# damaggu/StableKeypoints

Hardware: AMD Instinct MI355X
Metric: images/sec (token-opt step, 512², N=500 tokens) (higher is better)
Workload: dtype f32

## Files before the change

include/skp.h:

```cpp
#ifndef SKP_H
#define SKP_H

#ifdef __cplusplus
extern "C" {
#endif

#define SKP_OK 0
#define SKP_EBADARG (-1)
#define SKP_ELAUNCH (-2)
#define SKP_MAX_LAYERS 16

const char* skp_last_error(void);
int skp_version(void);

int skp_capture_fwd(const float* z_low, int BH, int s, int N, int R, float* attn, float* stats, void* stream);

int skp_capture_bwd(const float* z_low, int BH, int s, int N, int R, const float* dattn, int group, long long sb,
                    long long sp, long long sn, float gscale, const float* stats, float* dz_low, float* workspace,
                    void* stream);

int skp_capture_maps_fwd(const float* const* z_low, const int* sizes, int L, int B, int H, int N, int R, float* maps,
                         float* const* stats, void* stream);

int skp_capture_maps_bwd(const float* const* z_low, const int* sizes, int L, int B, int H, int N, int R,
                         const float* dmaps, float gscale, const float* const* stats, float* const* dz_low,
                         float* workspace, void* stream);

long long skp_capture_maps_bwd_sel_workspace(const int* sizes, int L, int B, int H, int N, int R, int K);
int skp_capture_maps_bwd_sel(const float* const* z_low, const int* sizes, int L, int B, int H, int N, int R,
                             const long long* sel_tok, int K, const float* gsel, float gscale,
                             const float* const* stats, float* const* dz_low, float* workspace, void* stream);
int skp_sel_bwd_timing(int enable);
int skp_sel_bwd_timing_read(double* ms, int* calls);

int skp_aggregate(const float* const* layers, int L, int BH, int RR, int N, const long long* indices,
                  int n_out, float* out, void* stream);

int skp_resize_bilinear(const float* in, int C, int R, int Ro, float* out, void* stream);
int skp_resize_bilinear_bwd(const float* gout, int C, int R, int Ro, float* gin, void* stream);

int skp_argmax2d(const float* maps, int T, int h, int w, const long long* rows, int n_rows, float* pos,
                 long long* idx, void* stream);

int skp_k_max_pixels(const float* maps, int T, int h, int w, int num, float radius2, float* pos,
                     float* masked, void* stream);

int skp_mask_radius(const float* maps, int T, int h, int w, const float* pos, float radius2, float* out,
                    void* stream);

int skp_weighted_avg(float* maps, int T, int h, int w, float distance, int mutate, float* pos, void* stream);

int skp_gaussian_target(const float* pos, int num, int T, int size, float sigma, float* out, void* stream);

int skp_topk_gaussian(const float* maps, int T, int h, int w, int top_k, float sigma, float epsilon,
                      int num_subjects, long long* out, double* kl, void* workspace, void* stream);

int skp_topk_gaussian_batch(const float* maps, int nb, int T, int h, int w, int top_k, float sigma,
                            float epsilon, int num_subjects, long long* out, double* kl, void* workspace,
                            void* stream);

int skp_topk_keys(const double* keys, int nb, int T, int top_k, long long* out, void* stream);

int skp_entropy_sort(const float* maps, int T, int h, int w, int top_k, long long* out, double* ent,
                     void* workspace, void* stream);

int skp_fps(const float* maps, int T, int h, int w, const long long* cand, int n_cand, int top_k,
            long long* out, int* n_out, void* workspace, void* stream);
int skp_fps_batch(const float* maps, int nb, int T, int h, int w, const long long* cand, int n_cand, int top_k,
                  long long* out, int* n_out, void* workspace, void* stream);
int skp_fps_keys_batch(const double* keys, const float* maps, int nb, int T, int h, int w, int n_cand, int top_k,
                       long long* cand, long long* out, int* n_out, void* workspace, void* stream);

int skp_sharpen_fwd(const float* A, int T, int h, int w, float sigma, int num_subjects, float* pos,
                     double* partial, float* loss, void* stream);
int skp_sharpen_bwd(const float* A, int T, int h, int w, float sigma, int num_subjects, const float* pos,
                     const float* gout, float* dA, void* stream);
int skp_sharpen_fwd_batch(const float* A, int nb, int T, int h, int w, float sigma, int num_subjects, float* pos,
                          double* partial, float* loss, void* stream);
int skp_sharpen_bwd_batch(const float* A, int nb, int T, int h, int w, float sigma, int num_subjects,
                          const float* pos, const float* gout, float* dA, void* stream);

int skp_affine_warp(const float* x, int B, int C, int H, int W, const float* theta, float* out, void* stream);
int skp_affine_warp_bwd(const float* gout, int B, int C, int H, int W, const float* theta, float* gin,
                        void* stream);

int skp_equiv_fwd(const float* A, const float* At, int T, int h, int w, const float* theta_inv,
                  double* partial, float* loss, void* stream);
int skp_equiv_bwd(const float* A, const float* At, int T, int h, int w, const float* theta_inv,
                  const float* gout, float* dA, float* dAt, void* stream);
int skp_equiv_fwd_batch(const float* A, const float* At, int nb, int T, int h, int w, const float* theta_inv,
                        double* partial, float* loss, void* stream);
int skp_equiv_bwd_batch(const float* A, const float* At, int nb, int T, int h, int w, const float* theta_inv,
                        const float* gout, float* dA, float* dAt, void* stream);

int skp_wino_in_transform(const float* x, int B, int C, int H, int W, float* V, void* stream);
int skp_wino_out_transform(const float* M, int B, int K, int H, int W, const float* bias, const float* residual,
                           float* y, void* stream);
int skp_wino_out_transform_kt(const float* M, int B, int K, int H, int W, const float* bias, const float* residual,
                              float* y, float* gn_part, void* stream);

int skp_bgemm_f32(const float* A, long long sAb, long long sAm, long long sAk, const float* B, long long sBb,
                  long long sBk, long long sBn, float* C, long long sCb, long long sCm, long long sCn, int batch,
                  int M, int N, int K, float alpha, int accumulate, void* stream);
int skp_bgemm_f32_2b(const float* A, long long sAo, long long sAb, long long sAm, long long sAk, const float* B,
                     long long sBo, long long sBb, long long sBk, long long sBn, float* C, long long sCo, long long sCb,
                     long long sCm, long long sCn, int batch, int hb, int M, int N, int K, float alpha, int accumulate,
                     void* stream);

int skp_groupnorm_workspace(int B, int C, long long HW, int G);
int skp_groupnorm_fwd(const float* x, const float* gamma, const float* beta, const float* shift, int B, int C,
                      long long HW, int G, float eps, int act, float* y, float* stats, double* partial,
                      void* stream);
int skp_groupnorm_bwd(const float* x, const float* dy, const float* gamma, const float* beta, const float* shift,
                      const float* stats, int B, int C, long long HW, int G, int act, float* dx, double* partial,
                      void* stream);
int skp_groupnorm_fwd_part(const float* x, const float* gamma, const float* beta, const float* shift, const float* part,
                           int nseg, int B, int C, long long HW, int G, float eps, int act, float* y, float* stats,
                           double* partial, void* stream);
int skp_groupnorm_stats(const float* x, const float* shift, int B, int C, long long HW, int G, float eps, float* stats,
                        double* partial, void* stream);
int skp_groupnorm_stats_part(const float* part, int nseg, const float* shift, int B, int C, long long HW, int G,
                             float eps, float* stats, double* partial, void* stream);
int skp_groupnorm_bwd_add(const float* x, const float* dy, const float* gamma, const float* beta, const float* shift,
                          const float* stats, int B, int C, long long HW, int G, int act, const float* dres, float* dx,
                          double* partial, void* stream);
int skp_softmax_bwd(const float* P, float* dP, long long rows, int cols, float alpha, void* stream);
int skp_softmax_fwd(float* S, long long rows, int cols, void* stream);
int skp_attn_dscore(const float* P, const float* dO, const float* V, const float* D, float* out, int BH, int S, int L,
                    int d, float alpha, void* stream);
int skp_attn_bwd_kv(const float* P, const float* dO, const float* Q, const float* V, const float* D, float* dS,
                    float* dV, float* dK, int BH, int S, int L, int d, float alpha, void* stream);
int skp_attn_fwd(const float* Q, const float* K, const float* V, float* O, float* stats, int BH, int S, int L, int d,
                 float scale, void* stream);
int skp_attn_bwd_flash(const float* Q, const float* K, const float* V, const float* dO, const float* stats,
                       const float* D, float* dS, float* dV, float* dK, int BH, int S, int L, int d, float scale,
                       void* stream);
int skp_attn_fwd_bshd(const float* Q, long long q_sb, int q_rs, const float* K, long long k_sb, int k_rs,
                      const float* V, long long v_sb, int v_rs, float* O, long long o_sb, int o_rs, float* stats, int B,
                      int H, int S, int L, int d, float scale, void* stream);
int skp_attn_bwd_flash_bshd(const float* Q, long long q_sb, int q_rs, const float* K, long long k_sb, int k_rs,
                            const float* V, long long v_sb, int v_rs, const float* dO, long long o_sb, int o_rs,
                            const float* stats, const float* D, float* dS, float* dV, long long dv_sb, int dv_rs,
                            float* dK, long long dk_sb, int dk_rs, int B, int H, int S, int L, int d, float scale,
                            void* stream);
int skp_layernorm_fwd(const float* x, const float* gamma, const float* beta, long long rows, int C, float eps, float* y,
                      float* stats, void* stream);
int skp_layernorm_bwd(const float* x, const float* dy, const float* gamma, const float* stats, long long rows, int C,
                      float* dx, void* stream);
int skp_layernorm_bwd_add(const float* x, const float* dy, const float* gamma, const float* stats, long long rows,
                          int C, const float* dres, float* dx, void* stream);
int skp_geglu_fwd(const float* h, long long rows, int I, float* out, void* stream);
int skp_geglu_bwd(const float* h, const float* dout, long long rows, int I, float* dh, void* stream);
int skp_residual_bias_add(const float* a, const float* h, const float* bias, int B, int C, long long HW,
                          float* out, void* stream);
int skp_wino_weights(const float* w, int K, int C, int flip, float* U, void* stream);
int skp_conv3x3_wino(const float* x, const float* U, const float* bias, const float* residual, float* y, int B, int C,
                     int K, int H, int W, int nsplit, float* ws, void* stream);
int skp_wino2_weights(const float* w, int K, int C, int flip, float* U, void* stream);
int skp_conv3x3_wino2(const float* x, const float* U, const float* bias, const float* residual, float* y, int B,
                      int C, int K, int H, int W, int nsplit, float* ws, void* stream);
int skp_conv3x3_wino2_gn(const float* x, const float* U, const float* bias, const float* residual, float* y, int B,
                         int C, int K, int H, int W, int nsplit, float* ws, float* gn_part, void* stream);
int skp_wino2_vtransform(const float* x, float* V, int B, int C, int H, int W, void* stream);
int skp_wino2_vtransform_gn(const float* x, const float* stats, const float* gamma, const float* beta,
                            const float* shift, int G, int act, float* V, int B, int C, int H, int W, void* stream);
int skp_conv3x3_wino2_v(const float* V, const float* U, const float* bias, const float* residual, float* y, int B,
                        int C, int K, int H, int W, int nsplit, float* ws, void* stream);
int skp_conv3x3_wino2_v_gn(const float* V, const float* U, const float* bias, const float* residual, float* y, int B,
                           int C, int K, int H, int W, int nsplit, float* ws, float* gn_part, void* stream);
int skp_wino2s2_weights(const float* w, int K, int C, float* U, void* stream);
int skp_conv3x3s2_f2(const float* x, const float* U, const float* bias, float* y, int B, int C, int K, int H, int W,
                     int nsplit, float* ws, void* stream);

int skp_map_range(const float* maps, int n, int h, int w, float* range, void* stream);
int skp_render_sheet(const float* images, int n, int H, int W, const float* maps, int h, int w, const float* range,
                     const float* lut, float alpha, const float* points, int K, float radius,
                     const unsigned char* colors, int rows, int cols, int f, int pad, unsigned char* out,
                     void* stream);

int skp_tta_reduce_workspace(int B, int n, int S);
int skp_tta_reduce(const float* maps, int B, int C, int n, int S, const float* theta_inv, float* pos, float* avg,
                   void* workspace, void* stream);

int skp_tta_reduce_scored_workspace(int B, int n, int S);
int skp_tta_reduce_scored(const float* maps, int B, int C, int n, int S, const float* theta_inv, float distance,
                          float* pos, float* refined, float* scores, float* avg, void* workspace, void* stream);

#ifdef __cplusplus
}
#endif
#endif
```

stablekeypoints_amd/_lib.py:

```python
import ctypes
import os

import torch

_HERE = os.path.dirname(os.path.abspath(__file__))
LIB_PATH = os.environ.get("SKP_LIB", os.path.join(_HERE, "libskp.so"))

_c_int, _c_float, _c_ll, _p = ctypes.c_int, ctypes.c_float, ctypes.c_longlong, ctypes.c_void_p

_SIGS = {
    "skp_capture_fwd": [_p, _c_int, _c_int, _c_int, _c_int, _p, _p, _p],
    "skp_capture_bwd": [_p, _c_int, _c_int, _c_int, _c_int, _p, _c_int, _c_ll, _c_ll, _c_ll, _c_float, _p, _p, _p,
                        _p],
    "skp_capture_maps_fwd": [ctypes.POINTER(_p), ctypes.POINTER(_c_int), _c_int, _c_int, _c_int, _c_int, _c_int, _p,
                             ctypes.POINTER(_p), _p],
    "skp_capture_maps_bwd": [ctypes.POINTER(_p), ctypes.POINTER(_c_int), _c_int, _c_int, _c_int, _c_int, _c_int, _p,
                             _c_float, ctypes.POINTER(_p), ctypes.POINTER(_p), _p, _p],
    "skp_capture_maps_bwd_sel": [ctypes.POINTER(_p), ctypes.POINTER(_c_int), _c_int, _c_int, _c_int, _c_int, _c_int,
                                 _p, _c_int, _p, _c_float, ctypes.POINTER(_p), ctypes.POINTER(_p), _p, _p],
    "skp_sel_bwd_timing": [_c_int],
    "skp_sel_bwd_timing_read": [_p, _p],
    "skp_capture_maps_bwd_sel_workspace": [ctypes.POINTER(_c_int), _c_int, _c_int, _c_int, _c_int, _c_int, _c_int],
    "skp_aggregate": [ctypes.POINTER(_p), _c_int, _c_int, _c_int, _c_int, _p, _c_int, _p, _p],
    "skp_resize_bilinear": [_p, _c_int, _c_int, _c_int, _p, _p],
    "skp_resize_bilinear_bwd": [_p, _c_int, _c_int, _c_int, _p, _p],
    "skp_argmax2d": [_p, _c_int, _c_int, _c_int, _p, _c_int, _p, _p, _p],
    "skp_k_max_pixels": [_p, _c_int, _c_int, _c_int, _c_int, _c_float, _p, _p, _p],
    "skp_mask_radius": [_p, _c_int, _c_int, _c_int, _p, _c_float, _p, _p],
    "skp_weighted_avg": [_p, _c_int, _c_int, _c_int, _c_float, _c_int, _p, _p],
    "skp_gaussian_target": [_p, _c_int, _c_int, _c_int, _c_float, _p, _p],
    "skp_topk_gaussian": [_p, _c_int, _c_int, _c_int, _c_int, _c_float, _c_float, _c_int, _p, _p, _p, _p],
    "skp_topk_gaussian_batch": [_p, _c_int, _c_int, _c_int, _c_int, _c_int, _c_float, _c_float, _c_int, _p, _p, _p,
                                _p],
    "skp_topk_keys": [_p, _c_int, _c_int, _c_int, _p, _p],
    "skp_entropy_sort": [_p, _c_int, _c_int, _c_int, _c_int, _p, _p, _p, _p],
    "skp_fps": [_p, _c_int, _c_int, _c_int, _p, _c_int, _c_int, _p, _p, _p, _p],
    "skp_fps_batch": [_p, _c_int, _c_int, _c_int, _c_int, _p, _c_int, _c_int, _p, _p, _p, _p],
    "skp_fps_keys_batch": [_p, _p, _c_int, _c_int, _c_int, _c_int, _c_int, _c_int, _p, _p, _p, _p, _p],
    "skp_sharpen_fwd": [_p, _c_int, _c_int, _c_int, _c_float, _c_int, _p, _p, _p, _p],
    "skp_sharpen_bwd": [_p, _c_int, _c_int, _c_int, _c_float, _c_int, _p, _p, _p, _p],
    "skp_wino_in_transform": [_p, _c_int, _c_int, _c_int, _c_int, _p, _p],
    "skp_wino_out_transform": [_p, _c_int, _c_int, _c_int, _c_int, _p, _p, _p, _p],
    "skp_wino_out_transform_kt": [_p, _c_int, _c_int, _c_int, _c_int, _p, _p, _p, _p, _p],
    "skp_sharpen_fwd_batch": [_p, _c_int, _c_int, _c_int, _c_int, _c_float, _c_int, _p, _p, _p, _p],
    "skp_sharpen_bwd_batch": [_p, _c_int, _c_int, _c_int, _c_int, _c_float, _c_int, _p, _p, _p, _p],
    "skp_affine_warp": [_p, _c_int, _c_int, _c_int, _c_int, _p, _p, _p],
    "skp_affine_warp_bwd": [_p, _c_int, _c_int, _c_int, _c_int, _p, _p, _p],
    "skp_equiv_fwd": [_p, _p, _c_int, _c_int, _c_int, _p, _p, _p, _p],
    "skp_equiv_bwd": [_p, _p, _c_int, _c_int, _c_int, _p, _p, _p, _p, _p],
    "skp_equiv_fwd_batch": [_p, _p, _c_int, _c_int, _c_int, _c_int, _p, _p, _p, _p],
    "skp_equiv_bwd_batch": [_p, _p, _c_int, _c_int, _c_int, _c_int, _p, _p, _p, _p, _p],
    "skp_bgemm_f32": [_p, _c_ll, _c_ll, _c_ll, _p, _c_ll, _c_ll, _c_ll, _p, _c_ll, _c_ll, _c_ll, _c_int, _c_int,
                      _c_int, _c_int, _c_float, _c_int, _p],
    "skp_bgemm_f32_2b": [_p, _c_ll, _c_ll, _c_ll, _c_ll, _p, _c_ll, _c_ll, _c_ll, _c_ll, _p, _c_ll, _c_ll, _c_ll,
                         _c_ll, _c_int, _c_int, _c_int, _c_int, _c_int, _c_float, _c_int, _p],
    "skp_groupnorm_workspace": [_c_int, _c_int, _c_ll, _c_int],
    "skp_groupnorm_fwd": [_p, _p, _p, _p, _c_int, _c_int, _c_ll, _c_int, _c_float, _c_int, _p, _p, _p, _p],
    "skp_groupnorm_bwd": [_p, _p, _p, _p, _p, _p, _c_int, _c_int, _c_ll, _c_int, _c_int, _p, _p, _p],
    "skp_groupnorm_bwd_add": [_p, _p, _p, _p, _p, _p, _c_int, _c_int, _c_ll, _c_int, _c_int, _p, _p, _p, _p],
    "skp_residual_bias_add": [_p, _p, _p, _c_int, _c_int, _c_ll, _p, _p],
    "skp_softmax_bwd": [_p, _p, _c_ll, _c_int, _c_float, _p],
    "skp_softmax_fwd": [_p, _c_ll, _c_int, _p],
    "skp_attn_dscore": [_p, _p, _p, _p, _p, _c_int, _c_int, _c_int, _c_int, _c_float, _p],
    "skp_attn_bwd_kv": [_p, _p, _p, _p, _p, _p, _p, _p, _c_int, _c_int, _c_int, _c_int, _c_float, _p],
    "skp_attn_fwd": [_p, _p, _p, _p, _p, _c_int, _c_int, _c_int, _c_int, _c_float, _p],
    "skp_attn_bwd_flash": [_p, _p, _p, _p, _p, _p, _p, _p, _p, _c_int, _c_int, _c_int, _c_int, _c_float, _p],
    "skp_attn_fwd_bshd": [_p, _c_ll, _c_int, _p, _c_ll, _c_int, _p, _c_ll, _c_int, _p, _c_ll, _c_int, _p, _c_int, _c_int,
                          _c_int, _c_int, _c_int, _c_float, _p],
    "skp_attn_bwd_flash_bshd": [_p, _c_ll, _c_int, _p, _c_ll, _c_int, _p, _c_ll, _c_int, _p, _c_ll, _c_int, _p, _p, _p,
                                _p, _c_ll, _c_int, _p, _c_ll, _c_int, _c_int, _c_int, _c_int, _c_int, _c_int, _c_float,
                                _p],
    "skp_layernorm_fwd": [_p, _p, _p, _c_ll, _c_int, _c_float, _p, _p, _p],
    "skp_layernorm_bwd": [_p, _p, _p, _p, _c_ll, _c_int, _p, _p],
    "skp_layernorm_bwd_add": [_p, _p, _p, _p, _c_ll, _c_int, _p, _p, _p],
    "skp_geglu_fwd": [_p, _c_ll, _c_int, _p, _p],
    "skp_geglu_bwd": [_p, _p, _c_ll, _c_int, _p, _p],
    "skp_wino_weights": [_p, _c_int, _c_int, _c_int, _p, _p],
    "skp_conv3x3_wino": [_p, _p, _p, _p, _p, _c_int, _c_int, _c_int, _c_int, _c_int, _c_int, _p, _p],
    "skp_wino2_weights": [_p, _c_int, _c_int, _c_int, _p, _p],
    "skp_conv3x3_wino2": [_p, _p, _p, _p, _p, _c_int, _c_int, _c_int, _c_int, _c_int, _c_int, _p, _p],
    "skp_conv3x3_wino2_gn": [_p, _p, _p, _p, _p, _c_int, _c_int, _c_int, _c_int, _c_int, _c_int, _p, _p, _p],
    "skp_groupnorm_fwd_part": [_p, _p, _p, _p, _p, _c_int, _c_int, _c_int, _c_ll, _c_int, _c_float, _c_int, _p, _p, _p,
                               _p],
    "skp_groupnorm_stats": [_p, _p, _c_int, _c_int, _c_ll, _c_int, _c_float, _p, _p, _p],
    "skp_groupnorm_stats_part": [_p, _c_int, _p, _c_int, _c_int, _c_ll, _c_int, _c_float, _p, _p, _p],
    "skp_wino2_vtransform": [_p, _p, _c_int, _c_int, _c_int, _c_int, _p],
    "skp_wino2_vtransform_gn": [_p, _p, _p, _p, _p, _c_int, _c_int, _p, _c_int, _c_int, _c_int, _c_int, _p],
    "skp_conv3x3_wino2_v": [_p, _p, _p, _p, _p, _c_int, _c_int, _c_int, _c_int, _c_int, _c_int, _p, _p],
    "skp_conv3x3_wino2_v_gn": [_p, _p, _p, _p, _p, _c_int, _c_int, _c_int, _c_int, _c_int, _c_int, _p, _p, _p],
    "skp_wino2s2_weights": [_p, _c_int, _c_int, _p, _p],
    "skp_conv3x3s2_f2":   [_p, _p, _p, _p, _c_int, _c_int, _c_int, _c_int, _c_int, _c_int, _p, _p],
    "skp_map_range": [_p, _c_int, _c_int, _c_int, _p, _p],
    "skp_render_sheet": [_p, _c_int, _c_int, _c_int, _p, _c_int, _c_int, _p, _p, _c_float, _p, _c_int, _c_float, _p,
                         _c_int, _c_int, _c_int, _c_int, _p, _p],
    "skp_tta_reduce_workspace": [_c_int, _c_int, _c_int],
    "skp_tta_reduce": [_p, _c_int, _c_int, _c_int, _c_int, _p, _p, _p, _p, _p],
    "skp_tta_reduce_scored_workspace": [_c_int, _c_int, _c_int],
    "skp_tta_reduce_scored": [_p, _c_int, _c_int, _c_int, _c_int, _p, _c_float, _p, _p, _p, _p, _p, _p],
    "skp_version": [],
}


_RESTYPE = {"skp_capture_maps_bwd_sel_workspace": _c_ll}
_MEASUREMENT_ONLY = {"skp_sel_bwd_timing", "skp_sel_bwd_timing_read"}


class SkpLibraryError(RuntimeError):
    pass


_lib = None


def lib():
    global _lib
    if _lib is None:
        if not os.path.exists(LIB_PATH):
            raise SkpLibraryError(f"libskp.so not found at {LIB_PATH}: build it with "
                                  "`python -c 'import __graft_entry__ as g; g.build()'` or `make -C stablekeypoints_amd/csrc`")
        try:
            L = ctypes.CDLL(LIB_PATH)
        except OSError as e:
            raise SkpLibraryError(f"cannot load {LIB_PATH}: {e}") from e
        for name, args in _SIGS.items():
            if name in _MEASUREMENT_ONLY and not hasattr(L, name):
                continue
            f = getattr(L, name)
            f.argtypes = args
            f.restype = _RESTYPE.get(name, _c_int)
        L.skp_last_error.argtypes = []
        L.skp_last_error.restype = ctypes.c_char_p
        _lib = L
    return _lib


def exported_symbols():
    return list(_SIGS) + ["skp_last_error"]


def call(name, *args):
    rc = getattr(lib(), name)(*args)
    if rc != 0:
        msg = lib().skp_last_error().decode(errors="replace")
        raise RuntimeError(f"{name} failed (rc={rc}): {msg}")


def ptr(t):
    return None if t is None else ctypes.c_void_p(t.data_ptr())


def stream(device=None):
    return ctypes.c_void_p(torch.cuda.current_stream(device).cuda_stream)


def require_device(*tensors):
    for t in tensors:
        if t is not None and not t.is_cuda:
            raise ValueError("stablekeypoints_amd ops run on the HIP device only; got a CPU tensor "
                             "(there is no CPU fallback: the CPU oracle lives under oracle/ and is test-only)")
```

stablekeypoints_amd/csrc/skp_groupnorm.hip:

```cpp
#include <algorithm>

#include "skp_common.h"
#include "skp_gn.h"

using namespace skp;

namespace {

constexpr int kThreads = 256;
constexpr int kChunk = 16384;

__device__ __forceinline__ float silu_grad(float z) {
  const float s = sigmoid_of(z);
  return s * (1.0f + z * (1.0f - s));
}

struct GNShape {
  int B, C, G, cpg, nsplit;
  long long HW, len;
};

__device__ __forceinline__ int chan_of(long long e, const GNShape& sh) {
#if SKP_GN_FAST
  return (int)((unsigned)e / (unsigned)sh.HW);
#else
  return (int)(e / sh.HW);
#endif
}

#ifndef SKP_GN_BATCH
#define SKP_GN_BATCH 4
#endif
template <typename Ld, typename Use>
__device__ __forceinline__ void for_f4(long long lo, long long hi, Ld ld, Use use) {
  constexpr int U = SKP_GN_BATCH;
  constexpr long long S = 4 * kThreads;
  long long e = lo + 4 * threadIdx.x;
  for (; e + (U - 1) * S < hi; e += U * S) {
    decltype(ld(e)) v[U];
#pragma unroll
    for (int u = 0; u < U; ++u) v[u] = ld(e + u * S);
#pragma unroll
    for (int u = 0; u < U; ++u) use(e + u * S, v[u]);
  }
  for (; e < hi; e += S) use(e, ld(e));
}

__device__ __forceinline__ float add_rn(float a, float b) {
#pragma clang fp contract(off)
  return a + b;
}

struct Pair4 {
  float4 a, b, r;
};
__device__ __forceinline__ Pair4 make_pair4(float4 a, float4 b) { return Pair4{a, b, make_float4(0.f, 0.f, 0.f, 0.f)}; }

__device__ __forceinline__ float shift_of(const float* __restrict__ shift, const GNShape& sh, int grp, int c) {
  return shift ? shift[(grp / sh.G) * sh.C + c] : 0.0f;
}

__device__ __forceinline__ void block_sum2(double& a, double& b, double* sd) {
  a = wave_sum(a);
  b = wave_sum(b);
  const int lane = threadIdx.x & 63, wid = threadIdx.x >> 6;
  if (lane == 0) { sd[2 * wid] = a; sd[2 * wid + 1] = b; }
  __syncthreads();
  if (threadIdx.x == 0) {
    double x = 0.0, y = 0.0;
    for (int w = 0; w < kThreads / 64; ++w) { x += sd[2 * w]; y += sd[2 * w + 1]; }
    sd[0] = x;
    sd[1] = y;
  }
  __syncthreads();
  a = sd[0];
  b = sd[1];
}

template <bool VEC>
__global__ __launch_bounds__(kThreads) void gn_stats_kernel(const float* __restrict__ x,
                                                            const float* __restrict__ shift, GNShape sh,
                                                            double* __restrict__ partial) {
  __shared__ double sd[2 * kThreads / 64];
  const int grp = blockIdx.x / sh.nsplit, sp = blockIdx.x % sh.nsplit;
  const int g = grp % sh.G;
  const float* base = x + (size_t)grp * sh.len;
  const long long lo = (long long)sp * kChunk, hi = min(sh.len, lo + kChunk);
  double s1 = 0.0, s2 = 0.0;
  if (VEC) {
    for_f4(lo, hi, [&](long long e) { return *reinterpret_cast<const float4*>(base + e); },
           [&](long long e, float4 v) {
             const float t = shift_of(shift, sh, grp, g * sh.cpg + chan_of(e, sh));
             v.x += t; v.y += t; v.z += t; v.w += t;
             s1 += (double)v.x + (double)v.y + (double)v.z + (double)v.w;
             s2 += (double)v.x * v.x + (double)v.y * v.y + (double)v.z * v.z + (double)v.w * v.w;
           });
  } else {
    for (long long e = lo + threadIdx.x; e < hi; e += kThreads) {
      const double v = base[e] + shift_of(shift, sh, grp, g * sh.cpg + chan_of(e, sh));
      s1 += v;
      s2 += v * v;
    }
  }
  block_sum2(s1, s2, sd);
  if (threadIdx.x == 0) {
    partial[2 * blockIdx.x] = s1;
    partial[2 * blockIdx.x + 1] = s2;
  }
}

__global__ __launch_bounds__(kThreads) void gn_part_combine_kernel(const float2* __restrict__ part, int nseg,
                                                                   const float* __restrict__ shift, GNShape sh,
                                                                   double* __restrict__ partial) {
  __shared__ double sd[2 * kThreads / 64];
  const int grp = blockIdx.x;
  const int b = grp / sh.G, g = grp - b * sh.G;
  const float2* pg = part + ((size_t)b * sh.C + (size_t)g * sh.cpg) * nseg;
  const double n = (double)(sh.HW / nseg);
  double s1 = 0.0, s2 = 0.0;
  for (int e = threadIdx.x; e < sh.cpg * nseg; e += kThreads) {
    const float2 v = pg[e];
    const double t = shift ? (double)shift[(size_t)b * sh.C + g * sh.cpg + e / nseg] : 0.0;
    const double mt = (double)v.x + t;
    s1 += n * mt;
    s2 += (double)v.y + n * mt * mt;
  }
  block_sum2(s1, s2, sd);
  if (threadIdx.x < sh.nsplit) {
    partial[2 * ((size_t)grp * sh.nsplit + threadIdx.x)] = threadIdx.x == 0 ? s1 : 0.0;
    partial[2 * ((size_t)grp * sh.nsplit + threadIdx.x) + 1] = threadIdx.x == 0 ? s2 : 0.0;
  }
  for (int k = kThreads + threadIdx.x; k < sh.nsplit; k += kThreads) {
    partial[2 * ((size_t)grp * sh.nsplit + k)] = 0.0;
    partial[2 * ((size_t)grp * sh.nsplit + k) + 1] = 0.0;
  }
}

__device__ __forceinline__ void group_moments(const double* __restrict__ partial, int grp, const GNShape& sh, float eps,
                                              float& mean, float& rstd) {
  double s1 = 0.0, s2 = 0.0;
  for (int k = 0; k < sh.nsplit; ++k) {
    s1 += partial[2 * (grp * sh.nsplit + k)];
    s2 += partial[2 * (grp * sh.nsplit + k) + 1];
  }
  const double n = (double)sh.len;
  const double m = s1 / n;
  double var = s2 / n - m * m;
  var = var < 0.0 ? 0.0 : var;
  mean = (float)m;
  rstd = (float)(1.0 / sqrt(var + (double)eps));
}

template <bool VEC, bool ACT>
__global__ __launch_bounds__(kThreads) void gn_apply_kernel(const float* __restrict__ x, const float* __restrict__ gamma,
                                                            const float* __restrict__ beta,
                                                            const float* __restrict__ shift, GNShape sh, float eps,
                                                            const double* __restrict__ partial, float* __restrict__ y,
                                                            float* __restrict__ stats) {
  __shared__ float sm[2];
  const int grp = blockIdx.x / sh.nsplit, sp = blockIdx.x % sh.nsplit;
  if (threadIdx.x == 0) {
    float mean, rstd;
    group_moments(partial, grp, sh, eps, mean, rstd);
    sm[0] = mean;
    sm[1] = rstd;
    if (sp == 0 && stats) { stats[2 * grp] = mean; stats[2 * grp + 1] = rstd; }
  }
  __syncthreads();
  const float mean = sm[0], rstd = sm[1];
  const int g = grp % sh.G;
  const float* base = x + (size_t)grp * sh.len;
  float* out = y + (size_t)grp * sh.len;
  const long long lo = (long long)sp * kChunk, hi = min(sh.len, lo + kChunk);
  if (VEC) {
    for_f4(lo, hi, [&](long long e) { return *reinterpret_cast<const float4*>(base + e); },
           [&](long long e, float4 v) {
             const int c = g * sh.cpg + chan_of(e, sh);
             const GNCoef k = gn_coef(gamma[c], beta[c], mean, rstd);
             const float t = shift_of(shift, sh, grp, c);
             v.x = gn_elem<ACT>(v.x, t, k); v.y = gn_elem<ACT>(v.y, t, k);
             v.z = gn_elem<ACT>(v.z, t, k); v.w = gn_elem<ACT>(v.w, t, k);
             *reinterpret_cast<float4*>(out + e) = v;
           });
  } else {
    for (long long e = lo + threadIdx.x; e < hi; e += kThreads) {
      const int c = g * sh.cpg + chan_of(e, sh);
      float v = ((base[e] + shift_of(shift, sh, grp, c)) - mean) * rstd * gamma[c] + beta[c];
      out[e] = ACT ? silu(v) : v;
    }
  }
}

template <bool VEC, bool ACT>
__global__ __launch_bounds__(kThreads) void gn_bwd_stats_kernel(const float* __restrict__ x,
                                                                const float* __restrict__ dy,
                                                                const float* __restrict__ gamma,
                                                                const float* __restrict__ beta,
                                                                const float* __restrict__ shift, GNShape sh,
                                                                const float* __restrict__ stats,
                                                                double* __restrict__ partial) {
  __shared__ double sd[2 * kThreads / 64];
  const int grp = blockIdx.x / sh.nsplit, sp = blockIdx.x % sh.nsplit;
  const int g = grp % sh.G;
  const float mean = stats[2 * grp], rstd = stats[2 * grp + 1];
  const float* xb = x + (size_t)grp * sh.len;
  const float* db = dy + (size_t)grp * sh.len;
  const long long lo = (long long)sp * kChunk, hi = min(sh.len, lo + kChunk);
  double s1 = 0.0, s2 = 0.0;
  auto body = [&](long long e0, const float* xv, const float* dv, int n) {
    const int c = g * sh.cpg + chan_of(e0, sh);
    const float ga = gamma[c], be = beta[c], t = shift_of(shift, sh, grp, c);
#pragma unroll
    for (int k = 0; k < 4; ++k) {
      if (k >= n) break;
      const float xh = ((xv[k] + t) - mean) * rstd;
      float gz = dv[k];
      if (ACT) gz *= silu_grad(xh * ga + be);
      const float gg = gz * ga;
      s1 += (double)gg;
      s2 += (double)gg * (double)xh;
    }
  };
  if (VEC) {
    for_f4(lo, hi,
           [&](long long e) {
             return make_pair4(*reinterpret_cast<const float4*>(xb + e), *reinterpret_cast<const float4*>(db + e));
           },
           [&](long long e, const Pair4& v) {
             const float xv[4] = {v.a.x, v.a.y, v.a.z, v.a.w}, dv[4] = {v.b.x, v.b.y, v.b.z, v.b.w};
             body(e, xv, dv, 4);
           });
  } else {
    for (long long e0 = lo + threadIdx.x; e0 < hi; e0 += kThreads) body(e0, xb + e0, db + e0, 1);
  }
  block_sum2(s1, s2, sd);
  if (threadIdx.x == 0) {
    partial[2 * blockIdx.x] = s1;
    partial[2 * blockIdx.x + 1] = s2;
  }
}

template <bool VEC, bool ACT>
__global__ __launch_bounds__(kThreads) void gn_bwd_apply_kernel(const float* __restrict__ x,
                                                                const float* __restrict__ dy,
                                                                const float* __restrict__ gamma,
                                                                const float* __restrict__ beta,
                                                                const float* __restrict__ shift, GNShape sh,
                                                                const float* __restrict__ stats,
                                                                const double* __restrict__ partial,
                                                                const float* __restrict__ dres,
                                                                float* __restrict__ dx) {
  __shared__ float sm[2];
  const int grp = blockIdx.x / sh.nsplit, sp = blockIdx.x % sh.nsplit;
  if (threadIdx.x == 0) {
    double s1 = 0.0, s2 = 0.0;
    for (int k = 0; k < sh.nsplit; ++k) {
      s1 += partial[2 * (grp * sh.nsplit + k)];
      s2 += partial[2 * (grp * sh.nsplit + k) + 1];
    }
    sm[0] = (float)(s1 / (double)sh.len);
    sm[1] = (float)(s2 / (double)sh.len);
  }
  __syncthreads();
  const float ma = sm[0], mb = sm[1];
  const int g = grp % sh.G;
  const float mean = stats[2 * grp], rstd = stats[2 * grp + 1];
  const float* xb = x + (size_t)grp * sh.len;
  const float* db = dy + (size_t)grp * sh.len;
  float* ob = dx + (size_t)grp * sh.len;
  const float* rb = dres ? dres + (size_t)grp * sh.len : nullptr;
  const long long lo = (long long)sp * kChunk, hi = min(sh.len, lo + kChunk);
  auto body = [&](long long e0, const float* xv, const float* dv, const float* av, float* r, int n) {
    const int c = g * sh.cpg + chan_of(e0, sh);
    const float ga = gamma[c], be = beta[c], t = shift_of(shift, sh, grp, c);
#pragma unroll
    for (int k = 0; k < 4; ++k) {
      if (k >= n) break;
      const float xh = ((xv[k] + t) - mean) * rstd;
      float gz = dv[k];
      if (ACT) gz *= silu_grad(xh * ga + be);
      r[k] = rstd * (gz * ga - ma - xh * mb);
      if (rb) r[k] = add_rn(r[k], av[k]);
    }
  };
  if (VEC) {
    for_f4(lo, hi,
           [&](long long e) {
             Pair4 v = make_pair4(*reinterpret_cast<const float4*>(xb + e), *reinterpret_cast<const float4*>(db + e));
             v.r = rb ? *reinterpret_cast<const float4*>(rb + e) : make_float4(0.f, 0.f, 0.f, 0.f);
             return v;
           },
           [&](long long e, const Pair4& v) {
             const float xv[4] = {v.a.x, v.a.y, v.a.z, v.a.w}, dv[4] = {v.b.x, v.b.y, v.b.z, v.b.w};
             const float av[4] = {v.r.x, v.r.y, v.r.z, v.r.w};
             float r[4];
             body(e, xv, dv, av, r, 4);
             *reinterpret_cast<float4*>(ob + e) = make_float4(r[0], r[1], r[2], r[3]);
           });
  } else {
    for (long long e0 = lo + threadIdx.x; e0 < hi; e0 += kThreads) {
      const float av = rb ? rb[e0] : 0.0f;
      float r;
      body(e0, xb + e0, db + e0, &av, &r, 1);
      ob[e0] = r;
    }
  }
}

template <bool VEC>
__global__ __launch_bounds__(kThreads) void residual_bias_kernel(const float* __restrict__ a,
                                                                 const float* __restrict__ h,
                                                                 const float* __restrict__ bias, int C, long long HW,
                                                                 long long total, float* __restrict__ out) {
  const long long step = (long long)gridDim.x * kThreads * (VEC ? 4 : 1);
  for (long long e = ((long long)blockIdx.x * kThreads + threadIdx.x) * (VEC ? 4 : 1); e < total; e += step) {
    const float b = bias[(e / HW) % C];
    if (VEC) {
      const float4 x = *reinterpret_cast<const float4*>(a + e), y = *reinterpret_cast<const float4*>(h + e);
      *reinterpret_cast<float4*>(out + e) = make_float4(x.x + (y.x + b), x.y + (y.y + b), x.z + (y.z + b),
                                                        x.w + (y.w + b));
    } else {
      out[e] = a[e] + (h[e] + b);
    }
  }
}

bool make_shape(int B, int C, long long HW, int G, GNShape& sh) {
  if (B <= 0 || C <= 0 || HW <= 0 || G <= 0 || C % G != 0) return false;
  sh.B = B; sh.C = C; sh.G = G; sh.cpg = C / G; sh.HW = HW;
  sh.len = (long long)sh.cpg * HW;
  sh.nsplit = (int)((sh.len + kChunk - 1) / kChunk);
  return sh.len < (1LL << 32);
}

}

extern "C" int skp_groupnorm_workspace(int B, int C, long long HW, int G) {
  GNShape sh;
  if (!make_shape(B, C, HW, G, sh)) return -1;
  return B * G * sh.nsplit * 2;
}

extern "C" int skp_groupnorm_fwd(const float* x, const float* gamma, const float* beta, const float* shift, int B,
                                 int C, long long HW, int G, float eps, int act, float* y, float* stats,
                                 double* partial, void* stream) {
  SKP_CHECK_ARG(x && gamma && beta && y && partial, "null pointer");
  GNShape sh;
  SKP_CHECK_ARG(make_shape(B, C, HW, G, sh), "bad shape (C must be divisible by G)");
  const bool vec = (HW % 4 == 0) && ((reinterpret_cast<uintptr_t>(x) & 15) == 0) &&
                   ((reinterpret_cast<uintptr_t>(y) & 15) == 0);
  hipStream_t st = as_stream(stream);
  const dim3 grid(B * G * sh.nsplit);
  if (vec) hipLaunchKernelGGL(gn_stats_kernel<true>, grid, dim3(kThreads), 0, st, x, shift, sh, partial);
  else hipLaunchKernelGGL(gn_stats_kernel<false>, grid, dim3(kThreads), 0, st, x, shift, sh, partial);
  SKP_LAUNCH_CHECK();
#define SKP_GN_APPLY(V, A) \
  hipLaunchKernelGGL((gn_apply_kernel<V, A>), grid, dim3(kThreads), 0, st, x, gamma, beta, shift, sh, eps, partial, y, \
                     stats)
  if (vec) { if (act) SKP_GN_APPLY(true, true); else SKP_GN_APPLY(true, false); }
  else { if (act) SKP_GN_APPLY(false, true); else SKP_GN_APPLY(false, false); }
#undef SKP_GN_APPLY
  SKP_LAUNCH_CHECK();
  return SKP_OK;
}

extern "C" int skp_groupnorm_fwd_part(const float* x, const float* gamma, const float* beta, const float* shift,
                                      const float* part, int nseg, int B, int C, long long HW, int G, float eps,
                                      int act, float* y, float* stats, double* partial, void* stream) {
  SKP_CHECK_ARG(x && gamma && beta && y && partial && part, "null pointer");
  SKP_CHECK_ARG(nseg > 0 && HW % nseg == 0, "nseg must divide H·W");
  GNShape sh;
  SKP_CHECK_ARG(make_shape(B, C, HW, G, sh), "bad shape (C must be divisible by G)");
  SKP_CHECK_ARG((reinterpret_cast<uintptr_t>(part) & 7) == 0, "part must be 8-byte aligned");
  const bool vec = (HW % 4 == 0) && ((reinterpret_cast<uintptr_t>(x) & 15) == 0) &&
                   ((reinterpret_cast<uintptr_t>(y) & 15) == 0);
  hipStream_t st = as_stream(stream);
  hipLaunchKernelGGL(gn_part_combine_kernel, dim3(B * G), dim3(kThreads), 0, st, reinterpret_cast<const float2*>(part),
                     nseg, shift, sh, partial);
  SKP_LAUNCH_CHECK();
  const dim3 grid(B * G * sh.nsplit);
#define SKP_GN_APPLY(V, A) \
  hipLaunchKernelGGL((gn_apply_kernel<V, A>), grid, dim3(kThreads), 0, st, x, gamma, beta, shift, sh, eps, partial, y, \
                     stats)
  if (vec) { if (act) SKP_GN_APPLY(true, true); else SKP_GN_APPLY(true, false); }
  else { if (act) SKP_GN_APPLY(false, true); else SKP_GN_APPLY(false, false); }
#undef SKP_GN_APPLY
  SKP_LAUNCH_CHECK();
  return SKP_OK;
}

namespace {
__global__ __launch_bounds__(kThreads) void gn_moments_kernel(const double* __restrict__ partial, GNShape sh, float eps,
                                                              float* __restrict__ stats) {
  const int grp = blockIdx.x * kThreads + threadIdx.x;
  if (grp >= sh.B * sh.G) return;
  float mean, rstd;
  group_moments(partial, grp, sh, eps, mean, rstd);
  stats[2 * grp] = mean;
  stats[2 * grp + 1] = rstd;
}
}

extern "C" int skp_groupnorm_stats(const float* x, const float* shift, int B, int C, long long HW, int G, float eps,
                                   float* stats, double* partial, void* stream) {
  SKP_CHECK_ARG(x && stats && partial, "null pointer");
  GNShape sh;
  SKP_CHECK_ARG(make_shape(B, C, HW, G, sh), "bad shape (C must be divisible by G)");
  const bool vec = (HW % 4 == 0) && ((reinterpret_cast<uintptr_t>(x) & 15) == 0);
  hipStream_t st = as_stream(stream);
  const dim3 grid(B * G * sh.nsplit);
  if (vec) hipLaunchKernelGGL(gn_stats_kernel<true>, grid, dim3(kThreads), 0, st, x, shift, sh, partial);
  else hipLaunchKernelGGL(gn_stats_kernel<false>, grid, dim3(kThreads), 0, st, x, shift, sh, partial);
  SKP_LAUNCH_CHECK();
  hipLaunchKernelGGL(gn_moments_kernel, dim3((B * G + kThreads - 1) / kThreads), dim3(kThreads), 0, st, partial, sh, eps,
                     stats);
  SKP_LAUNCH_CHECK();
  return SKP_OK;
}

extern "C" int skp_groupnorm_stats_part(const float* part, int nseg, const float* shift, int B, int C, long long HW,
                                        int G, float eps, float* stats, double* partial, void* stream) {
  SKP_CHECK_ARG(part && stats && partial, "null pointer");
  SKP_CHECK_ARG(nseg > 0 && HW % nseg == 0, "nseg must divide H·W");
  GNShape sh;
  SKP_CHECK_ARG(make_shape(B, C, HW, G, sh), "bad shape (C must be divisible by G)");
  SKP_CHECK_ARG((reinterpret_cast<uintptr_t>(part) & 7) == 0, "part must be 8-byte aligned");
  hipStream_t st = as_stream(stream);
  hipLaunchKernelGGL(gn_part_combine_kernel, dim3(B * G), dim3(kThreads), 0, st, reinterpret_cast<const float2*>(part),
                     nseg, shift, sh, partial);
  SKP_LAUNCH_CHECK();
  hipLaunchKernelGGL(gn_moments_kernel, dim3((B * G + kThreads - 1) / kThreads), dim3(kThreads), 0, st, partial, sh, eps,
                     stats);
  SKP_LAUNCH_CHECK();
  return SKP_OK;
}

extern "C" int skp_groupnorm_bwd_add(const float* x, const float* dy, const float* gamma, const float* beta,
                                     const float* shift, const float* stats, int B, int C, long long HW, int G, int act,
                                     const float* dres, float* dx, double* partial, void* stream) {
  SKP_CHECK_ARG(x && dy && gamma && beta && stats && dx && partial, "null pointer");
  GNShape sh;
  SKP_CHECK_ARG(make_shape(B, C, HW, G, sh), "bad shape (C must be divisible by G)");
  const bool vec = (HW % 4 == 0) && ((reinterpret_cast<uintptr_t>(x) & 15) == 0) &&
                   ((reinterpret_cast<uintptr_t>(dy) & 15) == 0) && ((reinterpret_cast<uintptr_t>(dx) & 15) == 0) &&
                   ((reinterpret_cast<uintptr_t>(dres) & 15) == 0);
  hipStream_t st = as_stream(stream);
  const dim3 grid(B * G * sh.nsplit);
#define SKP_GN_B(K, V, A, ...) hipLaunchKernelGGL((K<V, A>), grid, dim3(kThreads), 0, st, __VA_ARGS__)
  if (vec) {
    if (act) SKP_GN_B(gn_bwd_stats_kernel, true, true, x, dy, gamma, beta, shift, sh, stats, partial);
    else SKP_GN_B(gn_bwd_stats_kernel, true, false, x, dy, gamma, beta, shift, sh, stats, partial);
  } else {
    if (act) SKP_GN_B(gn_bwd_stats_kernel, false, true, x, dy, gamma, beta, shift, sh, stats, partial);
    else SKP_GN_B(gn_bwd_stats_kernel, false, false, x, dy, gamma, beta, shift, sh, stats, partial);
  }
  SKP_LAUNCH_CHECK();
  if (vec) {
    if (act) SKP_GN_B(gn_bwd_apply_kernel, true, true, x, dy, gamma, beta, shift, sh, stats, partial, dres, dx);
    else SKP_GN_B(gn_bwd_apply_kernel, true, false, x, dy, gamma, beta, shift, sh, stats, partial, dres, dx);
  } else {
    if (act) SKP_GN_B(gn_bwd_apply_kernel, false, true, x, dy, gamma, beta, shift, sh, stats, partial, dres, dx);
    else SKP_GN_B(gn_bwd_apply_kernel, false, false, x, dy, gamma, beta, shift, sh, stats, partial, dres, dx);
  }
#undef SKP_GN_B
  SKP_LAUNCH_CHECK();
  return SKP_OK;
}

extern "C" int skp_groupnorm_bwd(const float* x, const float* dy, const float* gamma, const float* beta,
                                 const float* shift, const float* stats, int B, int C, long long HW, int G, int act,
                                 float* dx, double* partial, void* stream) {
  return skp_groupnorm_bwd_add(x, dy, gamma, beta, shift, stats, B, C, HW, G, act, nullptr, dx, partial, stream);
}

extern "C" int skp_residual_bias_add(const float* a, const float* h, const float* bias, int B, int C, long long HW,
                                     float* out, void* stream) {
  SKP_CHECK_ARG(a && h && bias && out, "null pointer");
  SKP_CHECK_ARG(B > 0 && C > 0 && HW > 0, "non-positive shape");
  const long long total = (long long)B * C * HW;
  const bool vec = (HW % 4 == 0) && ((reinterpret_cast<uintptr_t>(a) & 15) == 0) &&
                   ((reinterpret_cast<uintptr_t>(h) & 15) == 0) && ((reinterpret_cast<uintptr_t>(out) & 15) == 0);
  const long long units = vec ? total / 4 : total;
  const int blocks = (int)std::min<long long>((units + kThreads - 1) / kThreads, 256LL * 16);
  hipStream_t st = as_stream(stream);
  if (vec) hipLaunchKernelGGL(residual_bias_kernel<true>, dim3(blocks), dim3(kThreads), 0, st, a, h, bias, C, HW, total, out);
  else hipLaunchKernelGGL(residual_bias_kernel<false>, dim3(blocks), dim3(kThreads), 0, st, a, h, bias, C, HW, total, out);
  SKP_LAUNCH_CHECK();
  return SKP_OK;
}
```

stablekeypoints_amd/csrc/skp_softmax.hip:

```cpp
#include "skp_common.h"

using namespace skp;

namespace {

template <int TPR, int EPT, bool VEC>
__global__ __launch_bounds__(TPR) void softmax_bwd_kernel(const float* __restrict__ P, float* __restrict__ G,
                                                          long long rows, int cols, float alpha) {
  __shared__ float sred[TPR / WAVE];
  const long long row = blockIdx.x;
  if (row >= rows) return;
  const float* p = P + row * cols;
  float* g = G + row * cols;
  static_assert(!VEC || EPT % 4 == 0, "float4 path needs EPT % 4 == 0");
  float pv[EPT], gv[EPT];
  float dot = 0.0f;
  if (VEC) {
#pragma unroll
    for (int q = 0; q < EPT / 4; ++q) {
      const int e = 4 * (threadIdx.x + q * TPR);
      float4 a = make_float4(0.f, 0.f, 0.f, 0.f), b = a;
      if (e < cols) {
        a = *reinterpret_cast<const float4*>(p + e);
        b = *reinterpret_cast<const float4*>(g + e);
// ... 233 lines not shown
template <int KS, int DB>
__global__ __launch_bounds__(256) void attn_fwd_kernel(const float* __restrict__ Q, const float* __restrict__ K,
                                                       const float* __restrict__ V, float* __restrict__ O,
                                                       float2* __restrict__ ST, int S, int L, float scale, int H,
                                                       AttnLay lq, AttnLay lk, AttnLay lv, AttnLay lo) {
  constexpr int d = 4 * KS, dp = d + 1;
  __shared__ float sK[64 * dp], sV[64 * 16 * DB];
  const int b = blockIdx.y;
  const int r0 = blockIdx.x * 64;
  const int t = threadIdx.x, lane = t & 63, w = t >> 6;
  const int row = r0 + 16 * w + (lane & 15);
  const float* Qb = lq.at(Q, b, H, d);
  const float* Kb = lk.at(K, b, H, d);
  const float* Vb = lv.at(V, b, H, d);
  float qv[KS];
  {
    const float* q = Qb + (size_t)row * lq.rs + (lane >> 4);
#pragma unroll
    for (int ks = 0; ks < KS; ++ks) qv[ks] = q[4 * ks] * scale;
  }
  f32x4a o[DB];
#pragma unroll
  for (int db = 0; db < DB; ++db) o[db] = f32x4a{0.f, 0.f, 0.f, 0.f};
  float m = -INFINITY, l = 0.0f;
  for (int k0 = 0; k0 < L; k0 += 64) {
    __syncthreads();
    {
      for (int e = t; e < 64 * KS; e += 256) {
        const int key = e / KS, c = 4 * (e - key * KS);
        float4 kk = make_float4(0.f, 0.f, 0.f, 0.f), vv = kk;
        if (k0 + key < L) {
          kk = *reinterpret_cast<const float4*>(Kb + (size_t)(k0 + key) * lk.rs + c);
          vv = *reinterpret_cast<const float4*>(Vb + (size_t)(k0 + key) * lv.rs + c);
        }
        float* pk = sK + key * dp + c;
        pk[0] = kk.x; pk[1] = kk.y; pk[2] = kk.z; pk[3] = kk.w;
        *reinterpret_cast<float4*>(sV + key * 16 * DB + c) = vv;
      }
      if constexpr (16 * DB > d)
        for (int e = t; e < 64 * (16 * DB - d); e += 256) {
          const int key = e / (16 * DB - d), c = d + (e - key * (16 * DB - d));
          sV[key * 16 * DB + c] = 0.0f;
        }
    }
    __syncthreads();
    f32x4a s4[4];
#pragma unroll
    for (int c = 0; c < 4; ++c) {
      s4[c] = f32x4a{0.f, 0.f, 0.f, 0.f};
      const float* kr = sK + (16 * c + (lane & 15)) * dp + (lane >> 4);
#pragma unroll
      for (int ks = 0; ks < KS; ++ks) s4[c] = __builtin_amdgcn_mfma_f32_16x16x4f32(kr[4 * ks], qv[ks], s4[c], 0, 0, 0);
    }
    if (k0 + 64 > L) {
#pragma unroll
      for (int c = 0; c < 4; ++c)
#pragma unroll
        for (int r = 0; r < 4; ++r)
          if (k0 + 16 * c + 4 * (lane >> 4) + r >= L) s4[c][r] = -INFINITY;
    }
    float bm = -INFINITY;
#pragma unroll
    for (int c = 0; c < 4; ++c) bm = fmaxf(bm, fmaxf(fmaxf(s4[c][0], s4[c][1]), fmaxf(s4[c][2], s4[c][3])));
    bm = fmaxf(bm, __shfl_xor(bm, 16, 64));
    bm = fmaxf(bm, __shfl_xor(bm, 32, 64));
    const float mn = fmaxf(m, bm);
    const float corr = __expf(m - mn);
    float bs = 0.0f;
#pragma unroll
    for (int c = 0; c < 4; ++c)
#pragma unroll
      for (int r = 0; r < 4; ++r) {
        s4[c][r] = __expf(s4[c][r] - mn);
        bs += s4[c][r];
      }
    bs += __shfl_xor(bs, 16, 64);
    bs += __shfl_xor(bs, 32, 64);
    l = l * corr + bs;
    m = mn;
#pragma unroll
    for (int db = 0; db < DB; ++db) o[db] *= corr;
#pragma unroll
    for (int c = 0; c < 4; ++c)
#pragma unroll
      for (int r = 0; r < 4; ++r) {
        const float* vr = sV + (16 * c + 4 * (lane >> 4) + r) * 16 * DB + (lane & 15);
#pragma unroll
        for (int db = 0; db < DB; ++db)
          o[db] = __builtin_amdgcn_mfma_f32_16x16x4f32(vr[16 * db], s4[c][r], o[db], 0, 0, 0);
      }
  }
  const float inv = 1.0f / l;
  float* orow = lo.at(O, b, H, d) + (size_t)row * lo.rs;
#pragma unroll
  for (int db = 0; db < DB; ++db) {
    const int dd = 16 * db + 4 * (lane >> 4);
    if (dd < d) *reinterpret_cast<float4*>(orow + dd) = make_float4(o[db][0] * inv, o[db][1] * inv, o[db][2] * inv, o[db][3] * inv);
  }
  if (ST != nullptr && lane < 16) ST[(size_t)b * S + row] = make_float2(m, inv);
}

}

namespace {
int attn_fwd_launch(const float* Q, AttnLay lq, const float* K, AttnLay lk, const float* V, AttnLay lv, float* O,
                    AttnLay lo, float* stats, int BH, int H, int S, int L, int d, float scale, void* stream) {
  SKP_CHECK_ARG(Q && K && V && O, "null pointer");
  SKP_CHECK_ARG(BH > 0 && H > 0 && BH % H == 0 && S > 0 && L > 0, "non-positive shape");
  SKP_CHECK_ARG(S % 64 == 0, "S must be a multiple of 64");
  SKP_CHECK_ARG(BH <= 65535, "grid too large");
  SKP_CHECK_ARG(((reinterpret_cast<uintptr_t>(K) | reinterpret_cast<uintptr_t>(V) | reinterpret_cast<uintptr_t>(O)) &
                 15) == 0,
                "tensors must be 16-byte aligned");
  SKP_CHECK_ARG(((lk.rs | lv.rs | lo.rs | lk.sb | lv.sb | lo.sb) & 3) == 0, "K, V, O strides must be multiples of 4");
  SKP_CHECK_ARG((reinterpret_cast<uintptr_t>(stats) & 7) == 0, "stats must be 8-byte aligned");
  const dim3 grid((unsigned)(S / 64), (unsigned)BH);
  hipStream_t st = as_stream(stream);
  float2* ST = reinterpret_cast<float2*>(stats);
#define SKP_AF(KS_, DB_)                                                                                        \
  hipLaunchKernelGGL((attn_fwd_kernel<KS_, DB_>), grid, dim3(256), 0, st, Q, K, V, O, ST, S, L, scale, H, lq, lk, lv, \
                     lo)
  switch (d) {
    case 40: SKP_AF(10, 3); break;
    case 64: SKP_AF(16, 4); break;
    case 80: SKP_AF(20, 5); break;
    default: SKP_CHECK_ARG(false, "head dim must be 40, 64 or 80");
  }
#undef SKP_AF
  SKP_LAUNCH_CHECK();
  return SKP_OK;
}
AttnLay contig(int rows, int d) { return AttnLay{(long long)rows * d, d}; }
}

extern "C" int skp_attn_fwd(const float* Q, const float* K, const float* V, float* O, float* stats, int BH, int S,
                            int L, int d, float scale, void* stream) {
  return attn_fwd_launch(Q, contig(S, d), K, contig(L, d), V, contig(L, d), O, contig(S, d), stats, BH, 1, S, L, d,
                         scale, stream);
}

extern "C" int skp_attn_fwd_bshd(const float* Q, long long q_sb, int q_rs, const float* K, long long k_sb, int k_rs,
                                 const float* V, long long v_sb, int v_rs, float* O, long long o_sb, int o_rs,
                                 float* stats, int B, int H, int S, int L, int d, float scale, void* stream) {
  SKP_CHECK_ARG(B > 0 && H > 0 && (long long)B * H <= 65535, "bad B, H");
  return attn_fwd_launch(Q, AttnLay{q_sb, q_rs}, K, AttnLay{k_sb, k_rs}, V, AttnLay{v_sb, v_rs}, O, AttnLay{o_sb, o_rs},
                         stats, B * H, H, S, L, d, scale, stream);
}

namespace {

template <int KS, int DB, int WPE, bool RC>
__global__ __launch_bounds__(256) __attribute__((amdgpu_waves_per_eu(WPE, WPE))) void attn_bwd_kv_kernel(
    const float* __restrict__ P, const float* __restrict__ dO, const float* __restrict__ Q, const float* __restrict__ V,
    const float* __restrict__ D, float* __restrict__ dS, float* __restrict__ dV, float* __restrict__ dK, int S, int L,
    float alpha, const float* __restrict__ Kt, const float2* __restrict__ ST, float scale, int H, AttnLay lo, AttnLay lq,
    AttnLay lk, AttnLay lv, AttnLay ldv, AttnLay ldk) {
  constexpr int d = 4 * KS, dp = d + 1, dq = 16 * DB + 1;
  __shared__ float sV[64 * dp];
  __shared__ float sK[RC ? 64 * dp : 1];
  __shared__ float2 sST[2][RC ? 64 : 1];
  __shared__ float sO[2][64 * dq], sQ[2][64 * dq];
  __shared__ float sD[2][64];
  const int b = blockIdx.y, k0 = blockIdx.x * 64;
  const int t = threadIdx.x, lane = t & 63, w = t >> 6;
  const float* Vb = lv.at(V, b, H, d);
  const float* dOb = lo.at(dO, b, H, d);
  const float* Qb = lq.at(Q, b, H, d);
  {
    for (int e = t; e < 64 * KS; e += 256) {
      const int key = e / KS, c = 4 * (e - key * KS);
      const bool in = k0 + key < L;
      const float4 v = in ? *reinterpret_cast<const float4*>(Vb + (size_t)(k0 + key) * lv.rs + c)
                          : make_float4(0.f, 0.f, 0.f, 0.f);
      float* p = sV + key * dp + c;
      p[0] = v.x; p[1] = v.y; p[2] = v.z; p[3] = v.w;
      if constexpr (RC) {
        const float4 kk = in ? *reinterpret_cast<const float4*>(lk.at(Kt, b, H, d) + (size_t)(k0 + key) * lk.rs + c)
                             : make_float4(0.f, 0.f, 0.f, 0.f);
        float* pk = sK + key * dp + c;
        pk[0] = kk.x; pk[1] = kk.y; pk[2] = kk.z; pk[3] = kk.w;
      }
    }
    for (int e = t; e < 64 * (dq - d); e += 256) {
      const int row = e / (dq - d), c = d + (e - row * (dq - d));
      sO[0][row * dq + c] = 0.0f; sO[1][row * dq + c] = 0.0f;
      sQ[0][row * dq + c] = 0.0f; sQ[1][row * dq + c] = 0.0f;
    }
  }
  constexpr int NPF = (64 * KS + 255) / 256;
  float4 fo[NPF], fq[NPF];
  float fd = 0.0f;
  float2 fst = make_float2(0.0f, 0.0f);
  const int rl = 16 * w + 4 * (lane >> 4);
  auto fetch = [&](int r0) {
#pragma unroll
    for (int j = 0; j < NPF; ++j) {
      const int e = t + 256 * j;
      if (e < 64 * KS) {
        const int row = e / KS, c = 4 * (e - row * KS);
        fo[j] = *reinterpret_cast<const float4*>(dOb + (size_t)(r0 + row) * lo.rs + c);
        fq[j] = *reinterpret_cast<const float4*>(Qb + (size_t)(r0 + row) * lq.rs + c);
      }
    }
    if (t < 64) {
      fd = D[(size_t)b * S + r0 + t];
      if constexpr (RC) fst = ST[(size_t)b * S + r0 + t];
    }
  };
  auto stash = [&](int buf) {
#pragma unroll
    for (int j = 0; j < NPF; ++j) {
      const int e = t + 256 * j;
      if (e < 64 * KS) {
        const int row = e / KS, c = 4 * (e - row * KS);
        float* po = sO[buf] + row * dq + c;
        float* pq = sQ[buf] + row * dq + c;
        po[0] = fo[j].x; po[1] = fo[j].y; po[2] = fo[j].z; po[3] = fo[j].w;
        pq[0] = fq[j].x; pq[1] = fq[j].y; pq[2] = fq[j].z; pq[3] = fq[j].w;
      }
    }
    if (t < 64) {
      sD[buf][t] = fd;
      if constexpr (RC) sST[buf][t] = fst;
    }
  };
  const float* Pl = P + ((size_t)b * S + rl) * L + k0 + (lane & 15);
  float* dSl = dS + ((size_t)b * S + rl) * L + k0 + (lane & 15);
  f32x4a pc[4];
  if constexpr (!RC) {
#pragma unroll
    for (int bj = 0; bj < 4; ++bj)
#pragma unroll
      for (int r = 0; r < 4; ++r) pc[bj][r] = Pl[(size_t)r * L + 16 * bj];
  }
  fetch(0);
  stash(0);
  f32x4a dv[DB][4], dk[DB][4];
#pragma unroll
  for (int db = 0; db < DB; ++db)
#pragma unroll
    for (int bj = 0; bj < 4; ++bj) {
      dv[db][bj] = f32x4a{0.f, 0.f, 0.f, 0.f};
      dk[db][bj] = f32x4a{0.f, 0.f, 0.f, 0.f};
    }
  for (int r0 = 0, buf = 0; r0 < S; r0 += 64, buf ^= 1) {
    __syncthreads();
    const bool more = r0 + 64 < S;
    f32x4a pn[4];
    if (more) {
      fetch(r0 + 64);
      if constexpr (!RC) {
        const float* Pn = Pl + (size_t)(r0 + 64) * L;
#pragma unroll
        for (int bj = 0; bj < 4; ++bj)
#pragma unroll
          for (int r = 0; r < 4; ++r) pn[bj][r] = Pn[(size_t)r * L + 16 * bj];
      }
    }
    const float* tO = sO[buf];
    const float* tQ = sQ[buf];
    f32x4a dp4[4];
    {
      const float* oa = tO + (16 * w + (lane & 15)) * dq + (lane >> 4);
      const float* vb = sV + (lane & 15) * dp + (lane >> 4);
#pragma unroll
      for (int bj = 0; bj < 4; ++bj) dp4[bj] = f32x4a{0.f, 0.f, 0.f, 0.f};
#pragma unroll
      for (int ks = 0; ks < KS; ++ks) {
        const float a = oa[4 * ks];
#pragma unroll
        for (int bj = 0; bj < 4; ++bj)
          dp4[bj] = __builtin_amdgcn_mfma_f32_16x16x4f32(a, vb[16 * bj * dp + 4 * ks], dp4[bj], 0, 0, 0);
      }
    }
    if constexpr (RC) {
      f32x4a sc[4];
      const float* qa = tQ + (16 * w + (lane & 15)) * dq + (lane >> 4);
      const float* kb = sK + (lane & 15) * dp + (lane >> 4);
#pragma unroll
      for (int bj = 0; bj < 4; ++bj) sc[bj] = f32x4a{0.f, 0.f, 0.f, 0.f};
#pragma unroll
      for (int ks = 0; ks < KS; ++ks) {
        const float a = qa[4 * ks];
#pragma unroll
        for (int bj = 0; bj < 4; ++bj)
          sc[bj] = __builtin_amdgcn_mfma_f32_16x16x4f32(a, kb[16 * bj * dp + 4 * ks], sc[bj], 0, 0, 0);
      }
#pragma unroll
      for (int r = 0; r < 4; ++r) {
        const float2 st = sST[buf][rl + r];
#pragma unroll
        for (int bj = 0; bj < 4; ++bj)
          pc[bj][r] = k0 + 16 * bj + (lane & 15) < L ? __expf(sc[bj][r] * scale - st.x) * st.y : 0.0f;
      }
    }
    f32x4a s4[4];
    float* dSr = dSl + (size_t)r0 * L;
#pragma unroll
    for (int r = 0; r < 4; ++r) {
      const float Dr = sD[buf][rl + r];
#pragma unroll
      for (int bj = 0; bj < 4; ++bj) {
        const float sv = alpha * (pc[bj][r] * (dp4[bj][r] - Dr));
        if (!RC || k0 + 16 * bj + (lane & 15) < L) dSr[(size_t)r * L + 16 * bj] = sv;
        s4[bj][r] = sv;
      }
    }
#pragma unroll
    for (int r = 0; r < 4; ++r) {
      const float* orow = tO + (rl + r) * dq + (lane & 15);
      const float* qrow = tQ + (rl + r) * dq + (lane & 15);
#pragma unroll
      for (int db = 0; db < DB; ++db) {
        const float ao = orow[16 * db], aq = qrow[16 * db];
#pragma unroll
        for (int bj = 0; bj < 4; ++bj) {
          dv[db][bj] = __builtin_amdgcn_mfma_f32_16x16x4f32(ao, pc[bj][r], dv[db][bj], 0, 0, 0);
          dk[db][bj] = __builtin_amdgcn_mfma_f32_16x16x4f32(aq, s4[bj][r], dk[db][bj], 0, 0, 0);
        }
      }
    }
    if (more) {
      stash(buf ^ 1);
      if constexpr (!RC) {
#pragma unroll
        for (int bj = 0; bj < 4; ++bj) pc[bj] = pn[bj];
      }
    }
  }
  __syncthreads();
  float* red = sO[0];
  for (int m = 0; m < 2; ++m) {
#pragma unroll
    for (int db = 0; db < DB; ++db)
#pragma unroll
      for (int bj = 0; bj < 4; ++bj) {
        const f32x4a val = m == 0 ? dv[db][bj] : dk[db][bj];
        *reinterpret_cast<float4*>(red + (w * 64 + lane) * 4) = make_float4(val[0], val[1], val[2], val[3]);
        __syncthreads();
        if (w == 0) {
          float4 acc = *reinterpret_cast<const float4*>(red + lane * 4);
#pragma unroll
          for (int ww = 1; ww < 4; ++ww) {
            const float4 x = *reinterpret_cast<const float4*>(red + (ww * 64 + lane) * 4);
            acc.x += x.x; acc.y += x.y; acc.z += x.z; acc.w += x.w;
          }
          const int dd = 16 * db + 4 * (lane >> 4);
          const int key = k0 + 16 * bj + (lane & 15);
          if (dd < d && key < L) {
            float* dst = m == 0 ? ldv.at(dV, b, H, d) + (size_t)key * ldv.rs : ldk.at(dK, b, H, d) + (size_t)key * ldk.rs;
            *reinterpret_cast<float4*>(dst + dd) = acc;
          }
        }
        __syncthreads();
      }
  }
}

}

extern "C" int skp_attn_bwd_kv(const float* P, const float* dO, const float* Q, const float* V, const float* D,
                               float* dS, float* dV, float* dK, int BH, int S, int L, int d, float alpha,
                               void* stream) {
  SKP_CHECK_ARG(P && dO && Q && V && D && dS && dV && dK, "null pointer");
  SKP_CHECK_ARG(BH > 0 && S > 0 && L > 0, "non-positive shape");
  SKP_CHECK_ARG(S % 64 == 0 && L % 64 == 0, "S and L must be multiples of 64");
  SKP_CHECK_ARG(BH <= 65535, "grid too large");
  SKP_CHECK_ARG(((reinterpret_cast<uintptr_t>(dO) | reinterpret_cast<uintptr_t>(Q) | reinterpret_cast<uintptr_t>(V) |
                  reinterpret_cast<uintptr_t>(dV) | reinterpret_cast<uintptr_t>(dK)) & 15) == 0,
                "tensors must be 16-byte aligned");
  const dim3 grid((unsigned)(L / 64), (unsigned)BH);
  hipStream_t st = as_stream(stream);
  const AttnLay ls = contig(S, d), ll = contig(L, d);
  switch (d) {
#define SKP_BKV(KS_, DB_, W_) \
  hipLaunchKernelGGL((attn_bwd_kv_kernel<KS_, DB_, W_, false>), grid, dim3(256), 0, st, P, dO, Q, V, D, dS, dV, dK, S, L, \
                     alpha, nullptr, nullptr, 0.0f, 1, ls, ls, ll, ll, ll, ll)
    case 40: SKP_BKV(10, 3, 2); break;
    case 64: SKP_BKV(16, 4, 1); break;
    case 80: SKP_BKV(20, 5, 1); break;
#undef SKP_BKV
    default: SKP_CHECK_ARG(false, "head dim must be 40, 64 or 80");
  }
  SKP_LAUNCH_CHECK();
  return SKP_OK;
}

namespace {
int attn_bwd_flash_launch(const float* Q, AttnLay lq, const float* K, AttnLay lk, const float* V, AttnLay lv,
                          const float* dO, AttnLay lo, const float* stats, const float* D, float* dS, float* dV,
                          AttnLay ldv, float* dK, AttnLay ldk, int BH, int H, int S, int L, int d, float scale,
                          void* stream) {
  SKP_CHECK_ARG(Q && K && V && dO && stats && D && dS && dV && dK, "null pointer");
  SKP_CHECK_ARG(BH > 0 && H > 0 && BH % H == 0 && S > 0 && L > 0, "non-positive shape");
  SKP_CHECK_ARG(S % 64 == 0, "S must be a multiple of 64");
  SKP_CHECK_ARG(BH <= 65535, "grid too large");
  SKP_CHECK_ARG(((reinterpret_cast<uintptr_t>(dO) | reinterpret_cast<uintptr_t>(Q) | reinterpret_cast<uintptr_t>(K) |
                  reinterpret_cast<uintptr_t>(V) | reinterpret_cast<uintptr_t>(dV) | reinterpret_cast<uintptr_t>(dK)) &
                 15) == 0 && (reinterpret_cast<uintptr_t>(stats) & 7) == 0,
                "tensors must be 16-byte aligned (stats 8-byte)");
  SKP_CHECK_ARG(((lq.rs | lk.rs | lv.rs | lo.rs | ldv.rs | ldk.rs | lq.sb | lk.sb | lv.sb | lo.sb | ldv.sb | ldk.sb) & 3) == 0,
                "strides must be multiples of 4");
  const dim3 grid((unsigned)((L + 63) / 64), (unsigned)BH);
  hipStream_t st = as_stream(stream);
  const float2* ST = reinterpret_cast<const float2*>(stats);
  switch (d) {
#define SKP_BFL(KS_, DB_, W_) \
  hipLaunchKernelGGL((attn_bwd_kv_kernel<KS_, DB_, W_, true>), grid, dim3(256), 0, st, nullptr, dO, Q, V, D, dS, dV, dK, \
                     S, L, scale, K, ST, scale, H, lo, lq, lk, lv, ldv, ldk)
    case 40: SKP_BFL(10, 3, 2); break;
    case 64: SKP_BFL(16, 4, 1); break;
    case 80: SKP_BFL(20, 5, 1); break;
#undef SKP_BFL
    default: SKP_CHECK_ARG(false, "head dim must be 40, 64 or 80");
  }
  SKP_LAUNCH_CHECK();
  return SKP_OK;
}
}

extern "C" int skp_attn_bwd_flash(const float* Q, const float* K, const float* V, const float* dO, const float* stats,
                                  const float* D, float* dS, float* dV, float* dK, int BH, int S, int L, int d, float scale,
                                  void* stream) {
  const AttnLay ls = contig(S, d), ll = contig(L, d);
  return attn_bwd_flash_launch(Q, ls, K, ll, V, ll, dO, ls, stats, D, dS, dV, ll, dK, ll, BH, 1, S, L, d, scale, stream);
}

extern "C" int skp_attn_bwd_flash_bshd(const float* Q, long long q_sb, int q_rs, const float* K, long long k_sb,
                                       int k_rs, const float* V, long long v_sb, int v_rs, const float* dO,
                                       long long o_sb, int o_rs, const float* stats, const float* D, float* dS,
                                       float* dV, long long dv_sb, int dv_rs, float* dK, long long dk_sb, int dk_rs,
                                       int B, int H, int S, int L, int d, float scale, void* stream) {
  SKP_CHECK_ARG(B > 0 && H > 0 && (long long)B * H <= 65535, "bad B, H");
  return attn_bwd_flash_launch(Q, AttnLay{q_sb, q_rs}, K, AttnLay{k_sb, k_rs}, V, AttnLay{v_sb, v_rs}, dO,
                               AttnLay{o_sb, o_rs}, stats, D, dS, dV, AttnLay{dv_sb, dv_rs}, dK, AttnLay{dk_sb, dk_rs},
                               B * H, H, S, L, d, scale, stream);
}
```

stablekeypoints_amd/csrc/skp_wino_gemm.hip:

```cpp
#include "skp_common.h"

using namespace skp;

namespace {

__device__ constexpr float kBt[6][6] = {{1.f, -1.5f, -2.f, 1.5f, 1.f, 0.f},  {0.f, -1.f, 0.5f, 2.5f, 1.f, 0.f},
                                        {0.f, 1.f, -2.5f, 0.5f, 1.f, 0.f},  {0.f, -2.f, -1.f, 2.f, 1.f, 0.f},
                                        {0.f, 0.5f, -1.f, -0.5f, 1.f, 0.f}, {0.f, 1.f, -1.5f, -2.f, 1.5f, 1.f}};
__device__ constexpr float kAt[4][6] = {{1.f, 1.f, 1.f, 1.f, 1.f, 0.f},
                                        {0.f, 1.f, -1.f, 0.5f, -2.f, 0.f},
                                        {0.f, 1.f, 1.f, 0.25f, 4.f, 0.f},
                                        {0.f, 1.f, -1.f, 0.125f, -8.f, 1.f}};

__global__ __launch_bounds__(256) void wino_in_kernel(const float* __restrict__ x, int B, int C, int H, int W,
                                                      float* __restrict__ V) {
  const int tw = W >> 2, th = H >> 2, T = B * th * tw;
  const int t = blockIdx.x * blockDim.x + threadIdx.x;
  const int c = blockIdx.y;
  if (t >= T) return;
  const int b = t / (th * tw), r = t - b * th * tw;
  const int ty = r / tw, tx = r - ty * tw;
  const float* xc = x + ((size_t)b * C + c) * H * W;
  float d[6][6];
#pragma unroll
  for (int a = 0; a < 6; ++a) {
    const int yy = 4 * ty - 1 + a;
#pragma unroll
    for (int e = 0; e < 6; ++e) {
      const int xx = 4 * tx - 1 + e;
      d[a][e] = (yy >= 0 && yy < H && xx >= 0 && xx < W) ? xc[(size_t)yy * W + xx] : 0.0f;
    }
  }
  float tmp[6][6];
#pragma unroll
  for (int i = 0; i < 6; ++i)
#pragma unroll
    for (int e = 0; e < 6; ++e) {
      float s = 0.0f;
#pragma unroll
      for (int a = 0; a < 6; ++a)
        if (kBt[i][a] != 0.0f) s = fmaf(kBt[i][a], d[a][e], s);
      tmp[i][e] = s;
    }
  const size_t ps = (size_t)C * T;
  float* out = V + (size_t)c * T + t;
#pragma unroll
  for (int i = 0; i < 6; ++i)
#pragma unroll
    for (int j = 0; j < 6; ++j) {
      float s = 0.0f;
#pragma unroll
      for (int e = 0; e < 6; ++e)
        if (kBt[j][e] != 0.0f) s = fmaf(tmp[i][e], kBt[j][e], s);
      out[(size_t)(6 * i + j) * ps] = s;
    }
}

__global__ __launch_bounds__(256) void wino_out_kernel(const float* __restrict__ M, int B, int K, int H, int W,
                                                       const float* __restrict__ bias, const float* __restrict__ res,
                                                       float* __restrict__ y) {
  const int tw = W >> 2, th = H >> 2, T = B * th * tw;
  const int k = blockIdx.x * blockDim.x + threadIdx.x;
  const int t = blockIdx.y;
  if (k >= K) return;
  const int b = t / (th * tw), r = t - b * th * tw;
  const int ty = r / tw, tx = r - ty * tw;
  const size_t ps = (size_t)T * K;
  const float* m = M + (size_t)t * K + k;
  float mv[6][6];
#pragma unroll
  for (int i = 0; i < 6; ++i)
#pragma unroll
    for (int j = 0; j < 6; ++j) mv[i][j] = m[(size_t)(6 * i + j) * ps];
  float tmp[4][6];
#pragma unroll
  for (int q = 0; q < 4; ++q)
#pragma unroll
    for (int j = 0; j < 6; ++j) {
      float s = 0.0f;
#pragma unroll
      for (int i = 0; i < 6; ++i)
        if (kAt[q][i] != 0.0f) s = fmaf(kAt[q][i], mv[i][j], s);
      tmp[q][j] = s;
    }
  const float bk = bias ? bias[k] : 0.0f;
  const size_t base = ((size_t)b * K + k) * H * W + (size_t)(4 * ty) * W + 4 * tx;
#pragma unroll
  for (int q = 0; q < 4; ++q) {
    float o[4];
#pragma unroll
    for (int s2 = 0; s2 < 4; ++s2) {
      float s = 0.0f;
#pragma unroll
      for (int j = 0; j < 6; ++j)
        if (kAt[s2][j] != 0.0f) s = fmaf(tmp[q][j], kAt[s2][j], s);
      o[s2] = s;
    }
    const size_t off = base + (size_t)q * W;
    float4 v = make_float4(o[0], o[1], o[2], o[3]);
    if (bias) {
      v.x += bk; v.y += bk; v.z += bk; v.w += bk;
    }
    if (res) {
      const float4 rv = *reinterpret_cast<const float4*>(res + off);
      v.x += rv.x; v.y += rv.y; v.z += rv.z; v.w += rv.w;
    }
    *reinterpret_cast<float4*>(y + off) = v;
  }
}

__global__ __launch_bounds__(256) void wino_out_kt_kernel(const float* __restrict__ M, int B, int K, int H, int W,
                                                          const float* __restrict__ bias,
                                                          const float* __restrict__ res, float* __restrict__ y,
                                                          float2* __restrict__ gnp) {
  const int tw = W >> 2, th = H >> 2, P = th * tw, T = B * P;
  const long long e = (long long)blockIdx.x * blockDim.x + threadIdx.x;
  const bool live = e < (long long)K * T;
  const long long ee = live ? e : (long long)K * T - 1;
  const int k = (int)(ee / T);
  const int tt = (int)(ee - (long long)k * T);
  const int b = tt / P, r = tt - b * P;
  const int ty = r / tw, tx = r - ty * tw;
  const size_t ps = (size_t)K * T;
  const float* m = M + (size_t)k * T + tt;
  float mv[6][6];
#pragma unroll
  for (int i = 0; i < 6; ++i)
#pragma unroll
    for (int j = 0; j < 6; ++j) mv[i][j] = m[(size_t)(6 * i + j) * ps];
  float tmp[4][6];
#pragma unroll
  for (int q = 0; q < 4; ++q)
#pragma unroll
    for (int j = 0; j < 6; ++j) {
      float s = 0.0f;
#pragma unroll
      for (int i = 0; i < 6; ++i)
        if (kAt[q][i] != 0.0f) s = fmaf(kAt[q][i], mv[i][j], s);
      tmp[q][j] = s;
    }
  const float bk = bias ? bias[k] : 0.0f;
  const size_t base = ((size_t)b * K + k) * H * W + (size_t)(4 * ty) * W + 4 * tx;
  const int seg = P < 64 ? P : 64;
  float s1 = 0.0f, s2 = 0.0f, piv = 0.0f;
#pragma unroll
  for (int q = 0; q < 4; ++q) {
    float o[4];
#pragma unroll
    for (int s2i = 0; s2i < 4; ++s2i) {
      float s = 0.0f;
#pragma unroll
      for (int j = 0; j < 6; ++j)
        if (kAt[s2i][j] != 0.0f) s = fmaf(tmp[q][j], kAt[s2i][j], s);
      o[s2i] = s;
    }
    const size_t off = base + (size_t)q * W;
    float4 v = make_float4(o[0], o[1], o[2], o[3]);
    if (bias) {
      v.x += bk; v.y += bk; v.z += bk; v.w += bk;
    }
    if (res) {
      const float4 rv = *reinterpret_cast<const float4*>(res + off);
      v.x += rv.x; v.y += rv.y; v.z += rv.z; v.w += rv.w;
    }
    if (live) *reinterpret_cast<float4*>(y + off) = v;
    if (gnp) {
      if (q == 0) piv = __shfl(v.x, (int)(threadIdx.x & 63) & ~(seg - 1), 64);
      const float dx = v.x - piv, dy = v.y - piv, dz = v.z - piv, dw = v.w - piv;
      s1 += (dx + dy) + (dz + dw);
      s2 += (dx * dx + dy * dy) + (dz * dz + dw * dw);
    }
  }
  if (gnp) {
    if (!live) s1 = s2 = 0.0f;
    s1 += dpp_read<0xB1>(s1); s2 += dpp_read<0xB1>(s2);
    s1 += dpp_read<0x4E>(s1); s2 += dpp_read<0x4E>(s2);
    s1 += dpp_read<0x141>(s1); s2 += dpp_read<0x141>(s2);
    s1 += dpp_read<0x140>(s1); s2 += dpp_read<0x140>(s2);
    if (seg >= 32) { s1 += __shfl_xor(s1, 16, 64); s2 += __shfl_xor(s2, 16, 64); }
    if (seg >= 64) { s1 += __shfl_xor(s1, 32, 64); s2 += __shfl_xor(s2, 32, 64); }
    if (live && (threadIdx.x & (seg - 1)) == 0) {
      const int nseg = P / seg;
      const float inv_n = 1.0f / (float)(16 * seg);
      gnp[((size_t)b * K + k) * nseg + r / seg] = make_float2(piv + s1 * inv_n, fmaxf(s2 - s1 * (s1 * inv_n), 0.0f));
    }
  }
}

}

extern "C" int skp_wino_in_transform(const float* x, int B, int C, int H, int W, float* V, void* stream) {
  SKP_CHECK_ARG(x && V, "null pointer");
  SKP_CHECK_ARG(B > 0 && C > 0 && H > 0 && W > 0, "non-positive shape");
  SKP_CHECK_ARG(H % 4 == 0 && W % 4 == 0, "H and W must be multiples of 4");
  SKP_CHECK_ARG(C <= 65535, "C > 65535");
  const long long T = (long long)B * (H / 4) * (W / 4);
  SKP_CHECK_ARG(T * C * 36 < (1LL << 40), "too large");
  hipLaunchKernelGGL(wino_in_kernel, dim3((unsigned)((T + 255) / 256), C), dim3(256), 0, as_stream(stream), x, B, C, H, W,
                     V);
  SKP_LAUNCH_CHECK();
  return SKP_OK;
}

extern "C" int skp_wino_out_transform(const float* M, int B, int K, int H, int W, const float* bias,
                                      const float* residual, float* y, void* stream) {
  SKP_CHECK_ARG(M && y, "null pointer");
  SKP_CHECK_ARG(B > 0 && K > 0 && H > 0 && W > 0, "non-positive shape");
  SKP_CHECK_ARG(H % 4 == 0 && W % 4 == 0, "H and W must be multiples of 4");
  SKP_CHECK_ARG((reinterpret_cast<uintptr_t>(y) & 15) == 0 &&
                    (!residual || (reinterpret_cast<uintptr_t>(residual) & 15) == 0),
                "y and residual must be 16-B aligned");
  const long long T = (long long)B * (H / 4) * (W / 4);
  SKP_CHECK_ARG(T <= 65535, "more than 65535 tiles (grid y)");
  hipLaunchKernelGGL(wino_out_kernel, dim3((K + 255) / 256, (unsigned)T), dim3(256), 0, as_stream(stream), M, B, K, H,
                     W, bias, residual, y);
  SKP_LAUNCH_CHECK();
  return SKP_OK;
}

extern "C" int skp_wino_out_transform_kt(const float* M, int B, int K, int H, int W, const float* bias,
                                         const float* residual, float* y, float* gn_part, void* stream) {
  SKP_CHECK_ARG(M && y, "null pointer");
  SKP_CHECK_ARG(B > 0 && K > 0 && H > 0 && W > 0, "non-positive shape");
  SKP_CHECK_ARG(H % 4 == 0 && W % 4 == 0, "H and W must be multiples of 4");
  SKP_CHECK_ARG(K <= 65535, "more than 65535 output channels (grid y)");
  SKP_CHECK_ARG((reinterpret_cast<uintptr_t>(y) & 15) == 0 &&
                    (!residual || (reinterpret_cast<uintptr_t>(residual) & 15) == 0),
                "y and residual must be 16-B aligned");
  const long long P = (long long)(H / 4) * (W / 4), T = B * P;
  SKP_CHECK_ARG(T < (1LL << 31), "too many tiles");
  SKP_CHECK_ARG(!gn_part || ((P == 16 || P == 32 || P % 64 == 0) && (reinterpret_cast<uintptr_t>(gn_part) & 7) == 0),
                "gn_part: tiles per plane must be 16, 32 or a multiple of 64; 8-B aligned");
  SKP_CHECK_ARG(T * K < (1LL << 40), "too large");
  hipLaunchKernelGGL(wino_out_kt_kernel, dim3((unsigned)((T * K + 255) / 256)), dim3(256), 0, as_stream(stream), M, B,
                     K, H, W, bias, residual, y, reinterpret_cast<float2*>(gn_part));
  SKP_LAUNCH_CHECK();
  return SKP_OK;
}
```

stablekeypoints_amd/ops.py:

```python
import ctypes
import os

import torch

from . import _lib
from ._lib import call, ptr, stream

F32 = torch.float32

_TIMER = None


def set_kernel_timer(timer):
    global _TIMER
    _TIMER = timer


class _NoTimer:
    def __enter__(self):
        return self

    def __exit__(self, *a):
        return False

# ... 541 lines not shown
    call("skp_gaussian_target", ptr(pos), num, T, int(size), float(sigma), ptr(out), stream(pos.device))
    return out


def find_top_k_gaussian(maps, top_k, sigma=3, epsilon=1e-5, num_subjects=1, return_kl=False):
    _lib.require_device(maps)
    maps = _c(maps)
    T, h, w = maps.shape
    top_k = min(int(top_k), T)
    out = torch.empty(top_k, device=maps.device, dtype=torch.int64)
    kl = torch.empty(T, device=maps.device, dtype=torch.float64)
    call("skp_topk_gaussian", ptr(maps), T, h, w, int(top_k), float(sigma), float(epsilon), int(num_subjects),
         ptr(out), ptr(kl), ptr(kl), stream(maps.device))
    return (out, kl) if return_kl else out


def find_top_k_gaussian_batch(maps, top_k, sigma=3, epsilon=1e-5, num_subjects=1):
    _lib.require_device(maps)
    maps = _c(maps)
    nb, T, h, w = maps.shape
    top_k = min(int(top_k), T)
    out = torch.empty(nb, top_k, device=maps.device, dtype=torch.int64)
    kl = torch.empty(nb, T, device=maps.device, dtype=torch.float64)
    with _timed("skp_topk_gaussian_batch", maps.numel() * 4 + nb * T * 8):
        call("skp_topk_gaussian_batch", ptr(maps), nb, T, h, w, int(top_k), float(sigma), float(epsilon),
             int(num_subjects), ptr(out), ptr(kl), ptr(kl), stream(maps.device))
    return out


def furthest_point_sampling_batch(maps, top_k, candidates):
    _lib.require_device(maps)
    maps = _c(maps)
    nb, T, h, w = maps.shape
    cand = candidates.to(device=maps.device, dtype=torch.int64).contiguous()
    if cand.dim() != 2 or cand.shape[0] != nb:
        raise ValueError(f"candidates {tuple(cand.shape)} for {nb} images")
    out = torch.empty(nb, top_k, device=maps.device, dtype=torch.int64)
    n_out = torch.empty(nb, device=maps.device, dtype=torch.int32)
    ws = torch.empty(2 * cand.numel() + 2, device=maps.device, dtype=F32)
    call("skp_fps_batch", ptr(maps), nb, T, h, w, ptr(cand), cand.shape[1], int(top_k), ptr(out), ptr(n_out),
         ptr(ws), stream(maps.device))
    return out, n_out


def fps_from_keys_batch(keys, maps, n_cand, top_k):
    _lib.require_device(maps)
    maps = _c(maps)
    nb, T, h, w = maps.shape
    keys = keys.to(device=maps.device, dtype=torch.float64).contiguous()
    if tuple(keys.shape) != (nb, T):
        raise ValueError(f"keys {tuple(keys.shape)} for maps {tuple(maps.shape)}")
    n_cand = min(int(n_cand), T)
    dev = maps.device
    cand = torch.empty(nb, n_cand, device=dev, dtype=torch.int64)
    out = torch.empty(nb, top_k, device=dev, dtype=torch.int64)
    n_out = torch.empty(nb, device=dev, dtype=torch.int32)
    ws = torch.empty(2 * nb * n_cand + 2, device=dev, dtype=F32)
    call("skp_fps_keys_batch", ptr(keys), ptr(maps), nb, T, h, w, n_cand, int(top_k), ptr(cand), ptr(out), ptr(n_out),
         ptr(ws), stream(dev))
    return out, n_out, cand


def gaussian_fps_batch(maps, maps_t, n_cand, top_k, sigma=3, epsilon=1e-5, num_subjects=1):
    _lib.require_device(maps)
    maps = _c(maps)
    nb, T, h, w = maps.shape
    if tuple(maps_t.shape) != (nb, T, h, w):
        raise ValueError(f"maps_t {tuple(maps_t.shape)} for maps {tuple(maps.shape)}")
    kl = torch.empty(nb, T, device=maps.device, dtype=torch.float64)
    with _timed("skp_selection", maps.numel() * 4 + nb * T * 8 + nb * min(int(n_cand), T) * h * w * 4):
        with _timed("skp_topk_gaussian_batch", maps.numel() * 4 + nb * T * 8):
            call("skp_topk_gaussian_batch", ptr(maps), nb, T, h, w, 0, float(sigma), float(epsilon),
                 int(num_subjects), ptr(kl), ptr(kl), ptr(kl), stream(maps.device))
        return fps_from_keys_batch(kl, maps_t, n_cand, top_k)


def entropy_keys_batch(maps):
    _lib.require_device(maps)
    maps = _c(maps)
    nb, T, h, w = maps.shape
    ent = torch.empty(nb, T, device=maps.device, dtype=torch.float64)
    call("skp_entropy_sort", ptr(maps), nb * T, h, w, 0, ptr(ent), ptr(ent), ptr(ent), stream(maps.device))
    return ent


def entropy_sort_batch(maps, top_k):
    _lib.require_device(maps)
    maps = _c(maps)
    nb, T, h, w = maps.shape
    top_k = min(int(top_k), T)
    out = torch.empty(nb, top_k, device=maps.device, dtype=torch.int64)
    ent = torch.empty(nb, T, device=maps.device, dtype=torch.float64)
    call("skp_entropy_sort", ptr(maps), nb * T, h, w, 0, ptr(out), ptr(ent), ptr(ent), stream(maps.device))
    if top_k > 0:
        call("skp_topk_keys", ptr(ent), nb, T, int(top_k), ptr(out), stream(maps.device))
    return out


def entropy_sort(maps, top_k, return_entropy=False):
    _lib.require_device(maps)
    maps = _c(maps)
    T, h, w = maps.shape
    top_k = min(int(top_k), T)
    out = torch.empty(top_k, device=maps.device, dtype=torch.int64)
    ent = torch.empty(T, device=maps.device, dtype=torch.float64)
    call("skp_entropy_sort", ptr(maps), T, h, w, int(top_k), ptr(out), ptr(ent), ptr(ent), stream(maps.device))
    return (out, ent) if return_entropy else out


def furthest_point_sampling(maps, top_k, candidates):
    _lib.require_device(maps)
    maps = _c(maps)
    T, h, w = maps.shape
    cand = candidates.to(device=maps.device, dtype=torch.int64).contiguous()
    out = torch.empty(top_k, device=maps.device, dtype=torch.int64)
    n_out = torch.empty(1, device=maps.device, dtype=torch.int32)
    ws = torch.empty(2 * cand.numel() + 2, device=maps.device, dtype=F32)
    call("skp_fps", ptr(maps), T, h, w, ptr(cand), cand.numel(), int(top_k), ptr(out), ptr(n_out), ptr(ws),
         stream(maps.device))
    return out, n_out


class SharpeningLoss(torch.autograd.Function):
    @staticmethod
    def forward(ctx, A, sigma, num_subjects):
        A = _c(A)
        T, h, w = A.shape
        pos = torch.empty(num_subjects, T, 2, device=A.device, dtype=F32)
        part = torch.empty(T, device=A.device, dtype=torch.float64)
        loss = torch.empty((), device=A.device, dtype=F32)
        call("skp_sharpen_fwd", ptr(A), T, h, w, float(sigma), int(num_subjects), ptr(pos), ptr(part), ptr(loss),
             stream(A.device))
        ctx.save_for_backward(A, pos)
        ctx.sigma, ctx.num = sigma, num_subjects
        return loss

    @staticmethod
    def backward(ctx, g):
        A, pos = ctx.saved_tensors
        T, h, w = A.shape
        dA = torch.empty_like(A)
        call("skp_sharpen_bwd", ptr(A), T, h, w, float(ctx.sigma), int(ctx.num), ptr(pos), ptr(_c(g.reshape(1))),
             ptr(dA), stream(A.device))
        return dA, None, None


def sharpening_loss(A, sigma=1.0, num_subjects=1):
    _lib.require_device(A)
    return SharpeningLoss.apply(A, float(sigma), int(num_subjects))


class SharpeningLossBatch(torch.autograd.Function):

    @staticmethod
    def forward(ctx, A, nb, sigma, num_subjects):
        A = _c(A)
        R, h, w = A.shape
        T = R // nb
        pos = torch.empty(num_subjects, R, 2, device=A.device, dtype=F32)
        part = torch.empty(R, device=A.device, dtype=torch.float64)
        loss = torch.empty(nb, device=A.device, dtype=F32)
        call("skp_sharpen_fwd_batch", ptr(A), nb, T, h, w, float(sigma), int(num_subjects), ptr(pos), ptr(part),
             ptr(loss), stream(A.device))
        ctx.save_for_backward(A, pos)
        ctx.meta = (nb, T, sigma, num_subjects)
        return loss

    @staticmethod
    def backward(ctx, g):
        A, pos = ctx.saved_tensors
        nb, T, sigma, num = ctx.meta
        _, h, w = A.shape
        dA = torch.empty_like(A)
        call("skp_sharpen_bwd_batch", ptr(A), nb, T, h, w, float(sigma), int(num), ptr(pos), ptr(_c(g.reshape(nb))),
             ptr(dA), stream(A.device))
        return dA, None, None, None


def sharpening_loss_batch(A, nb, sigma=1.0, num_subjects=1):
    _lib.require_device(A)
    if A.shape[0] % nb:
        raise ValueError(f"{A.shape[0]} rows for {nb} images")
    return SharpeningLossBatch.apply(A, int(nb), float(sigma), int(num_subjects))


class AffineWarp(torch.autograd.Function):
    @staticmethod
    def forward(ctx, x, theta):
        x = _c(x)
        B, C, H, W = x.shape
        th = _c(theta.to(x.device))
        out = torch.empty_like(x)
        call("skp_affine_warp", ptr(x), B, C, H, W, ptr(th), ptr(out), stream(x.device))
        ctx.save_for_backward(th)
        ctx.shape = (B, C, H, W)
        return out

    @staticmethod
    def backward(ctx, g):
        (th,) = ctx.saved_tensors
        B, C, H, W = ctx.shape
        gin = torch.empty(B, C, H, W, device=g.device, dtype=F32)
        call("skp_affine_warp_bwd", ptr(_c(g)), B, C, H, W, ptr(th), ptr(gin), stream(g.device))
        return gin, None


def affine_warp(x, theta):
    _lib.require_device(x)
    return AffineWarp.apply(x, theta)


class EquivarianceLoss(torch.autograd.Function):
    @staticmethod
    def forward(ctx, A, At, theta_inv):
        A, At = _c(A), _c(At)
        T, h, w = A.shape
        th = _c(theta_inv.to(A.device)).reshape(6)
        part = torch.empty(T, device=A.device, dtype=torch.float64)
        loss = torch.empty((), device=A.device, dtype=F32)
        call("skp_equiv_fwd", ptr(A), ptr(At), T, h, w, ptr(th), ptr(part), ptr(loss), stream(A.device))
        ctx.save_for_backward(A, At, th)
        return loss

    @staticmethod
    def backward(ctx, g):
        A, At, th = ctx.saved_tensors
        T, h, w = A.shape
        dA = torch.empty_like(A) if ctx.needs_input_grad[0] else None
        dAt = torch.empty_like(At)
        call("skp_equiv_bwd", ptr(A), ptr(At), T, h, w, ptr(th), ptr(_c(g.reshape(1))), ptr(dA), ptr(dAt),
             stream(A.device))
        return dA, (dAt if ctx.needs_input_grad[1] else None), None


def equivariance_loss_single(A, At, theta_inv):
    _lib.require_device(A, At)
    return EquivarianceLoss.apply(A, At, theta_inv)


class EquivarianceLossBatch(torch.autograd.Function):

    @staticmethod
    def forward(ctx, A, At, theta_inv, nb):
        A, At = _c(A), _c(At)
        R, h, w = A.shape
        T = R // nb
        th = _c(theta_inv.to(A.device)).reshape(nb * 6)
        part = torch.empty(R, device=A.device, dtype=torch.float64)
        loss = torch.empty(nb, device=A.device, dtype=F32)
        call("skp_equiv_fwd_batch", ptr(A), ptr(At), nb, T, h, w, ptr(th), ptr(part), ptr(loss), stream(A.device))
        ctx.save_for_backward(A, At, th)
        ctx.meta = (nb, T)
        return loss

    @staticmethod
    def backward(ctx, g):
        A, At, th = ctx.saved_tensors
        nb, T = ctx.meta
        _, h, w = A.shape
        dA = torch.empty_like(A) if ctx.needs_input_grad[0] else None
        dAt = torch.empty_like(At)
        call("skp_equiv_bwd_batch", ptr(A), ptr(At), nb, T, h, w, ptr(th), ptr(_c(g.reshape(nb))), ptr(dA), ptr(dAt),
             stream(A.device))
        return dA, (dAt if ctx.needs_input_grad[1] else None), None, None


def equivariance_loss_batch(A, At, theta_inv, nb):
    _lib.require_device(A, At)
    if A.shape[0] % nb or theta_inv.numel() != 6 * nb:
        raise ValueError(f"{A.shape[0]} rows / theta_inv {tuple(theta_inv.shape)} for {nb} images")
    return EquivarianceLossBatch.apply(A, At, theta_inv, int(nb))


GN_EPI = True


def _gn_parts_of(x):
    ent = getattr(x, "_skp_gn", None)
    if ent is None or ent[0] != x._version:
        return None
    return ent[1], ent[2]


def _gn_fwd(x, gamma, beta, shift, groups, eps, act):
    B, C = x.shape[:2]
    HW = x[0, 0].numel()
    nws = _lib.lib().skp_groupnorm_workspace(B, C, HW, groups)
    if nws < 0:
        raise ValueError(f"groupnorm: bad shape {tuple(x.shape)} groups={groups}")
    part = torch.empty(nws, device=x.device, dtype=torch.float64)
    stats = torch.empty(B * groups * 2, device=x.device, dtype=F32)
    y = torch.empty_like(x)
    g, b = _c(gamma.detach()), _c(beta.detach())
    pre = _gn_parts_of(x) if GN_EPI else None
    if pre is not None:
        call("skp_groupnorm_fwd_part", ptr(x), ptr(g), ptr(b), ptr(shift), ptr(pre[0]), pre[1], B, C, HW,
             int(groups), float(eps), int(act), ptr(y), ptr(stats), ptr(part), stream(x.device))
    else:
        call("skp_groupnorm_fwd", ptr(x), ptr(g), ptr(b), ptr(shift), B, C, HW, int(groups), float(eps), int(act),
             ptr(y), ptr(stats), ptr(part), stream(x.device))
    return y, stats, g, b, nws


class GroupNormAct(torch.autograd.Function):

    @staticmethod
    def forward(ctx, x, gamma, beta, groups, eps, act, shift):
        x = _c(x)
        B, C = x.shape[:2]
        HW = x[0, 0].numel()
        if shift is not None:
            shift = _c(shift.detach().expand(B, C))
        y, stats, g, b, nws = _gn_fwd(x, gamma, beta, shift, groups, eps, act)
        ctx.save_for_backward(x, g, b, stats, shift)
        ctx.meta = (B, C, HW, int(groups), int(act), nws)
        return y

    @staticmethod
    def backward(ctx, dy):
        x, g, b, stats, shift = ctx.saved_tensors
        B, C, HW, G, act, nws = ctx.meta
        dy = _c(dy)
        dx = torch.empty_like(x)
        part = torch.empty(nws, device=x.device, dtype=torch.float64)
        call("skp_groupnorm_bwd", ptr(x), ptr(dy), ptr(g), ptr(b), ptr(shift), ptr(stats), B, C, HW, G, act, ptr(dx),
             ptr(part), stream(x.device))
        return dx, None, None, None, None, None, None


class GroupNormActRes(torch.autograd.Function):

    @staticmethod
    def forward(ctx, x, gamma, beta, groups, eps, act, shift):
        xc = _c(x)
        B, C = xc.shape[:2]
        HW = xc[0, 0].numel()
        if shift is not None:
            shift = _c(shift.detach().expand(B, C))
        y, stats, g, b, nws = _gn_fwd(xc, gamma, beta, shift, groups, eps, act)
        ctx.save_for_backward(xc, g, b, stats, shift)
        ctx.meta = (B, C, HW, int(groups), int(act), nws)
        return y, x.view_as(x)

    @staticmethod
    def backward(ctx, dy, dpass):
        x, g, b, stats, shift = ctx.saved_tensors
        B, C, HW, G, act, nws = ctx.meta
        dy = _c(dy)
        dres = None if dpass is None else _c16(dpass)
        dx = torch.empty_like(x)
        part = torch.empty(nws, device=x.device, dtype=torch.float64)
        call("skp_groupnorm_bwd_add", ptr(x), ptr(dy), ptr(g), ptr(b), ptr(shift), ptr(stats), B, C, HW, G, act,
             ptr(dres), ptr(dx), ptr(part), stream(x.device))
        return dx, None, None, None, None, None, None


def group_norm_act_res(x, gamma, beta, groups, eps, act):
    _lib.require_device(x)
    return GroupNormActRes.apply(x, gamma, beta, int(groups), float(eps), bool(act), None)


def group_norm_act(x, gamma, beta, groups, eps, act, shift=None):
    _lib.require_device(x)
    if shift is not None:
        shift = shift.reshape(-1, x.shape[1]).to(x.device, F32)
    return GroupNormAct.apply(x, gamma, beta, int(groups), float(eps), bool(act), shift)


class ResidualBiasAdd(torch.autograd.Function):

    @staticmethod
    def forward(ctx, a, h, bias):
        a, h = _c(a), _c(h)
        B, C = a.shape[:2]
        out = torch.empty_like(a)
        call("skp_residual_bias_add", ptr(a), ptr(h), ptr(_c(bias.detach())), B, C, a[0, 0].numel(), ptr(out),
             stream(a.device))
        return out

    @staticmethod
    def backward(ctx, g):
        return g, g, None


def residual_bias_add(a, h, bias):
    _lib.require_device(a, h)
    if a.shape != h.shape:
        raise ValueError(f"residual_bias_add: shapes {tuple(a.shape)} and {tuple(h.shape)} differ")
    return ResidualBiasAdd.apply(a, h, bias)


def softmax_(s):
    if s.dtype != F32 or not s.is_contiguous() or s.shape[-1] % 4 or s.shape[-1] > 16384 or \
            s.data_ptr() % 16:
        return s.copy_(s.softmax(dim=-1))
    call("skp_softmax_fwd", ptr(s), s.numel() // s.shape[-1], s.shape[-1], stream(s.device))
    return s


def attention_probs(q, k, scale):
    sim = torch.baddbmm(torch.empty(q.shape[0], q.shape[1], k.shape[1], dtype=q.dtype, device=q.device),
                        q, k.transpose(1, 2), beta=0, alpha=scale)
    return softmax_(sim)


def attention_nograd(q, k, v, scale):
    BH, S, d = q.shape
    L = k.shape[1]
    if (q.dtype == F32 and S % 64 == 0 and d in (40, 64, 80) and q.is_contiguous()
            and k.is_contiguous() and v.is_contiguous()):
        out = torch.empty_like(q)
        call("skp_attn_fwd", ptr(q), ptr(k), ptr(v), ptr(out), None, BH, S, L, d, float(scale), stream(q.device))
        return out
    return torch.bmm(attention_probs(q, k, scale), v)


ATTN_FUSED_KV = (40,)


class MathAttention(torch.autograd.Function):

    @staticmethod
    def forward(ctx, q, k, v, scale):
        p = attention_probs(q, k, scale)
        out = torch.bmm(p, v)
        ctx.save_for_backward(q, k, v, p, out)
        ctx.scale = scale
        return out

    @staticmethod
    def backward(ctx, dout):
        q, k, v, p, out = ctx.saved_tensors
        dout = dout.contiguous()
        BH, S, L = p.shape
        d = q.shape[2]
        if (d in ATTN_FUSED_KV and S % 64 == 0 and L % 64 == 0 and ctx.needs_input_grad[1]
                and all(t.is_contiguous() and t.data_ptr() % 16 == 0 for t in (q, v, dout))):
            D = (dout * out).sum(-1)
            ds, dv, dk = torch.empty_like(p), torch.empty_like(v), torch.empty_like(k)
            call("skp_attn_bwd_kv", ptr(p), ptr(dout), ptr(q), ptr(v), ptr(D), ptr(ds), ptr(dv), ptr(dk),
                 BH, S, L, d, float(ctx.scale), stream(p.device))
            dq = torch.bmm(ds, k) if ctx.needs_input_grad[0] else None
            return dq, dk, dv if ctx.needs_input_grad[2] else None, None
        dv = torch.bmm(p.transpose(1, 2), dout) if ctx.needs_input_grad[2] else None
        dq = dk = None
        if ctx.needs_input_grad[0] or ctx.needs_input_grad[1]:
            if S % 64 == 0 and L % 64 == 0 and d in (40, 64, 80, 160) and v.is_contiguous():
                D = (dout * out).sum(-1)
                ds = torch.empty_like(p)
                call("skp_attn_dscore", ptr(p), ptr(dout), ptr(v), ptr(D), ptr(ds), BH, S, L, d,
                     float(ctx.scale), stream(p.device))
            else:
                ds = torch.bmm(dout, v.transpose(1, 2))
                call("skp_softmax_bwd", ptr(p), ptr(ds), p.shape[0] * p.shape[1], p.shape[2], float(ctx.scale),
                     stream(p.device))
            dq = torch.bmm(ds, k) if ctx.needs_input_grad[0] else None
            dk = torch.bmm(ds.transpose(1, 2), q) if ctx.needs_input_grad[1] else None
        return dq, dk, dv, None


class LayerNormFn(torch.autograd.Function):

    @staticmethod
    def forward(ctx, x, weight, bias, eps):
        x = _c(x)
        C = x.shape[-1]
        rows = x.numel() // C
        y = torch.empty_like(x)
        stats = torch.empty(rows, 2, device=x.device, dtype=F32)
        w, b = _c(weight.detach()), _c(bias.detach())
        call("skp_layernorm_fwd", ptr(x), ptr(w), ptr(b), rows, C, float(eps), ptr(y), ptr(stats), stream(x.device))
        ctx.save_for_backward(x, w, stats)
        return y

    @staticmethod
    def backward(ctx, dy):
        x, w, stats = ctx.saved_tensors
        dy = _c(dy)
        C = x.shape[-1]
        dx = torch.empty_like(x)
        call("skp_layernorm_bwd", ptr(x), ptr(dy), ptr(w), ptr(stats), x.numel() // C, C, ptr(dx), stream(x.device))
        return dx, None, None, None


class LayerNormRes(torch.autograd.Function):

    @staticmethod
    def forward(ctx, x, weight, bias, eps):
        xc = _c(x)
        C = xc.shape[-1]
        rows = xc.numel() // C
        y = torch.empty_like(xc)
        stats = torch.empty(rows, 2, device=xc.device, dtype=F32)
        w, b = _c(weight.detach()), _c(bias.detach())
        call("skp_layernorm_fwd", ptr(xc), ptr(w), ptr(b), rows, C, float(eps), ptr(y), ptr(stats), stream(xc.device))
        ctx.save_for_backward(xc, w, stats)
        return y, x.view_as(x)

    @staticmethod
    def backward(ctx, dy, dpass):
        x, w, stats = ctx.saved_tensors
        dy = _c(dy)
        dres = None if dpass is None else _c16(dpass)
        C = x.shape[-1]
        dx = torch.empty_like(x)
        call("skp_layernorm_bwd_add", ptr(x), ptr(dy), ptr(w), ptr(stats), x.numel() // C, C, ptr(dres), ptr(dx),
             stream(x.device))
        return dx, None, None, None


def layer_norm_res(x, weight, bias, eps):
    _lib.require_device(x)
    C = x.shape[-1]
    if (x.dtype != F32 or C % 4 or C > 2048 or weight is None or bias is None or weight.requires_grad
            or bias.requires_grad or x.numel() == 0 or x.numel() // C < LN_MIN_ROWS):
        return torch.nn.functional.layer_norm(x, (C,), weight, bias, eps), x
    return LayerNormRes.apply(x, weight, bias, float(eps))


LN_MIN_ROWS = 2048


def layer_norm(x, weight, bias, eps):
    _lib.require_device(x)
    C = x.shape[-1]
    if (x.dtype != F32 or C % 4 or C > 2048 or weight is None or bias is None or weight.requires_grad
            or bias.requires_grad or x.numel() == 0 or x.numel() // C < LN_MIN_ROWS):
        return torch.nn.functional.layer_norm(x, (C,), weight, bias, eps)
    return LayerNormFn.apply(x, weight, bias, float(eps))


class Geglu(torch.autograd.Function):

    @staticmethod
    def forward(ctx, h):
        h = _c(h)
        I = h.shape[-1] // 2
        out = torch.empty(*h.shape[:-1], I, device=h.device, dtype=F32)
        call("skp_geglu_fwd", ptr(h), h.numel() // h.shape[-1], I, ptr(out), stream(h.device))
        ctx.save_for_backward(h)
        return out

    @staticmethod
    def backward(ctx, dout):
        (h,) = ctx.saved_tensors
        dout = _c(dout)
        dh = torch.empty_like(h)
        call("skp_geglu_bwd", ptr(h), ptr(dout), h.numel() // h.shape[-1], h.shape[-1] // 2, ptr(dh),
             stream(h.device))
        return dh


def geglu(h):
    _lib.require_device(h)
    if h.dtype != F32 or h.shape[-1] % 8:
        x, gate = h.chunk(2, dim=-1)
        return x * torch.nn.functional.gelu(gate)
    return Geglu.apply(h)


ATTN_FLASH = (40, 64)


class FlashAttention(torch.autograd.Function):

    @staticmethod
    def forward(ctx, q, k, v, scale):
        BH, S, d = q.shape
        L = k.shape[1]
        out = torch.empty_like(q)
        stats = torch.empty(BH, S, 2, device=q.device, dtype=F32)
        call("skp_attn_fwd", ptr(q), ptr(k), ptr(v), ptr(out), ptr(stats), BH, S, L, d, float(scale),
             stream(q.device))
        ctx.save_for_backward(q, k, v, out, stats)
        ctx.scale = scale
        return out

    @staticmethod
    def backward(ctx, dout):
        q, k, v, out, stats = ctx.saved_tensors
        dout = dout.contiguous()
        BH, S, d = q.shape
        L = k.shape[1]
        D = (dout * out).sum(-1)
        ds = torch.empty(BH, S, L, device=q.device, dtype=F32)
        dv, dk = torch.empty_like(v), torch.empty_like(k)
        call("skp_attn_bwd_flash", ptr(q), ptr(k), ptr(v), ptr(dout), ptr(stats), ptr(D), ptr(ds), ptr(dv), ptr(dk),
             BH, S, L, d, float(ctx.scale), stream(q.device))
        dq = torch.bmm(ds, k) if ctx.needs_input_grad[0] else None
        return dq, dk if ctx.needs_input_grad[1] else None, dv if ctx.needs_input_grad[2] else None, None


def math_attention(q, k, v, scale):
    _lib.require_device(q, k, v)
    BH, S, d = q.shape
    L = k.shape[1]
    if (d in ATTN_FLASH and S % 64 == 0 and q.dtype == F32
            and all(t.dtype == F32 and t.is_contiguous() and t.data_ptr() % 16 == 0 for t in (q, k, v))):
        return FlashAttention.apply(q, k, v, float(scale))
    return MathAttention.apply(q, k, v, float(scale))


ATTN_BSHD = True


def _lay(t):
    return int(t.stride(0)), int(t.stride(1))


def _bshd_ok(q, k, v, H):
    B, S, C = q.shape
    if not ATTN_BSHD or C % H or S % 64 or k.shape[-1] != C or v.shape[-1] != C:
        return False
    return all(t.is_cuda and t.dtype == F32 and t.dim() == 3 and t.stride(2) == 1 and t.stride(1) % 4 == 0
               and t.stride(0) % 4 == 0 and t.data_ptr() % 16 == 0 for t in (q, k, v))


class FlashAttentionBSHD(torch.autograd.Function):

    @staticmethod
    def forward(ctx, q, k, v, H, scale):
        B, S, C = q.shape
        L = k.shape[1]
        d = C // H
        out = torch.empty(B, S, C, device=q.device, dtype=F32)
        stats = torch.empty(B * H, S, 2, device=q.device, dtype=F32)
        call("skp_attn_fwd_bshd", ptr(q), *_lay(q), ptr(k), *_lay(k), ptr(v), *_lay(v), ptr(out), S * C, C, ptr(stats),
             B, H, S, L, d, float(scale), stream(q.device))
        ctx.save_for_backward(q, k, v, out, stats)
        ctx.H, ctx.scale = H, scale
        return out

    @staticmethod
    def backward(ctx, dout):
        q, k, v, out, stats = ctx.saved_tensors
        H, scale = ctx.H, ctx.scale
        dout = _c16(dout)
        B, S, C = q.shape
        L = k.shape[1]
        d = C // H
        D = (dout.view(B, S, H, d) * out.view(B, S, H, d)).sum(-1).transpose(1, 2).contiguous()
        ds = torch.empty(B * H, S, L, device=q.device, dtype=F32)
        dv = torch.empty(B, L, C, device=q.device, dtype=F32)
        dk = torch.empty(B, L, C, device=q.device, dtype=F32)
        call("skp_attn_bwd_flash_bshd", ptr(q), *_lay(q), ptr(k), *_lay(k), ptr(v), *_lay(v), ptr(dout), S * C, C,
             ptr(stats), ptr(D), ptr(ds), ptr(dv), L * C, C, ptr(dk), L * C, C, B, H, S, L, d, float(scale),
             stream(q.device))
        dq = None
        if ctx.needs_input_grad[0]:
            k4 = k.view(k.shape[0], L, H, d).transpose(1, 2).expand(B, H, L, d)
            dq = torch.matmul(ds.view(B, H, S, L), k4).transpose(1, 2).reshape(B, S, C)
        return (dq, dk if ctx.needs_input_grad[1] else None, dv if ctx.needs_input_grad[2] else None, None, None)


def attention_heads(q, k, v, H, scale):
    if not _bshd_ok(q, k, v, H):
        return None
    B, S, C = q.shape
    d = C // H
    if torch.is_grad_enabled() and (q.requires_grad or k.requires_grad or v.requires_grad):
        if d not in ATTN_FLASH or k.stride(0) != 0:
            return None
        return FlashAttentionBSHD.apply(q, k, v, int(H), float(scale))
    if d not in (40, 64, 80):
        return None
    out = torch.empty(B, S, C, device=q.device, dtype=F32)
    call("skp_attn_fwd_bshd", ptr(q), *_lay(q), ptr(k), *_lay(k), ptr(v), *_lay(v), ptr(out), S * C, C, None,
         B, H, S, k.shape[1], d, float(scale), stream(q.device))
    return out


_QKV_W = {}


def _qkv_weight(*ws):
    key = tuple(id(w) for w in ws)
    sig = tuple((w._version, w.data_ptr()) for w in ws)
    ent = _QKV_W.get(key)
    if ent is not None and ent[0] == sig and all(r() is w for r, w in zip(ent[1], ws)):
        return ent[2]
    w3 = torch.cat([w.detach() for w in ws], 0).contiguous()
    drop = lambda _r, key=key: _QKV_W.pop(key, None)
    _QKV_W[key] = (sig, tuple(_weakref.ref(w, drop) for w in ws), w3)
    return w3


class QKVProjection(torch.autograd.Function):

    @staticmethod
    def forward(ctx, x, w3, C):
        out = torch.matmul(x, w3.t())
        ctx.save_for_backward(w3)
        ctx.C = C
        ctx.x_shape = x.shape
        ctx.set_materialize_grads(False)
        return tuple(out[..., i * C:(i + 1) * C] for i in range(w3.shape[0] // C))

    @staticmethod
    def backward(ctx, *grads):
        (w3,) = ctx.saved_tensors
        C = ctx.C
        dx = None
        for i, g in enumerate(grads):
            if g is None:
                continue
            g2 = g.reshape(-1, C)
            wi = w3[i * C:(i + 1) * C]
            if dx is None:
                dx = torch.mm(g2, wi)
            else:
                dx.addmm_(g2, wi)
        if dx is None:
            return None, None, None
        return dx.view(ctx.x_shape), None, None


QKV_FUSED = True


def qkv_projection(x, *ws):
    _lib.require_device(x)
    return QKVProjection.apply(x, _qkv_weight(*ws), int(ws[0].shape[0]))


class TokensProjIn(torch.autograd.Function):

    @staticmethod
    def forward(ctx, x, w, bias):
        B, C, HW = x.shape
        h = torch.bmm(x.transpose(1, 2), w.t().expand(B, C, w.shape[0]))
        if bias is not None:
            h.add_(bias)
        ctx.save_for_backward(w)
        return h

    @staticmethod
    def backward(ctx, dh):
        (w,) = ctx.saved_tensors
        B = dh.shape[0]
        dx = torch.bmm(w.t().expand(B, w.shape[1], w.shape[0]), dh.transpose(1, 2))
        return dx, None, None


class TokensProjOut(torch.autograd.Function):

    @staticmethod
    def forward(ctx, h, w):
        B = h.shape[0]
        ctx.save_for_backward(w)
        return torch.bmm(w.expand(B, *w.shape), h.transpose(1, 2))

    @staticmethod
    def backward(ctx, dy):
        (w,) = ctx.saved_tensors
        B = dy.shape[0]
        return torch.bmm(dy.transpose(1, 2), w.expand(B, *w.shape)), None


def tokens_proj_in(x, weight, bias):
    B, C = x.shape[:2]
    return TokensProjIn.apply(x.reshape(B, C, -1), weight.detach().reshape(weight.shape[0], C),
                              None if bias is None else bias.detach())


def tokens_proj_out(h, weight, bias, residual):
    B, C = residual.shape[:2]
    y = TokensProjOut.apply(h, weight.detach().reshape(C, h.shape[-1]))
    return residual_bias_add(residual, y.view(residual.shape), bias)


import weakref as _weakref

_WINO_U = {}
WINO_MIN_WORKGROUPS = 128
WINO_KERNEL = "auto"
WINO_SPLIT = True
WINO_NSPLIT_FORCE = 0


def _wino_v2(H, W, B=None):
    if WINO_KERNEL == "v1":
        return False
    return (H % 32 == 0 and W % 32 == 0) or (H == 16 and W == 16 and B is not None and B % 4 == 0)


def _wino_u_cached(weight, flip, form, build):
    key = id(weight)
    ent = _WINO_U.get(key)
    if ent is None or ent[0]() is not weight:
        ent = _WINO_U[key] = (_weakref.ref(weight, lambda _r: _WINO_U.pop(key, None)), {})
    hit = ent[1].get((flip, form))
    if hit is None or hit[0] != weight._version:
        hit = ent[1][(flip, form)] = (weight._version, build())
    return hit[1]


def _wino_u(weight, flip, v2=False):
    def build():
        w = _c(weight.detach())
        K, C = (w.shape[0], w.shape[1]) if not flip else (w.shape[1], w.shape[0])
        if v2 == "s2":
            U = torch.empty(K * C * 28, device=w.device, dtype=F32)
            call("skp_wino2s2_weights", ptr(w), K, C, ptr(U), stream(w.device))
        else:
            U = torch.empty(K * C * (40 if v2 else 36), device=w.device, dtype=F32)
            call("skp_wino2_weights" if v2 else "skp_wino_weights", ptr(w), K, C, int(flip), ptr(U), stream(w.device))
        return U
    return _wino_u_cached(weight, flip, v2, build)


def _batch_chunks(B, per_img_bytes):
    bmax = max(1, (2 ** 31 - 1) // per_img_bytes)
    for b0 in range(0, B, bmax):
        yield b0, min(B, b0 + bmax)


def _wino_plan_uncached(B, C, K, H, W, force):
    v2 = _wino_v2(H, W, B)
    if v2:
        wgs = (B // 4 if H == 16 else B * (H // 32) * (W // 32)) * (K // 32)
    elif B * (H // 4) * (W // 4) <= 32 and K % 64 == 0:
        wgs = K // 64
    else:
        wgs = -(-(B * (H // 4) * (W // 4)) // 64) * (K // 32)
    out_bytes = B * K * H * W * 4

    def cost(s):
        if v2:
            k = -(-2 * wgs * s // 256)
            st = C // s // 4
            return (k // 2) * st * 1.72e-6 + (k % 2) * st * 1.48e-6 + (s > 1) * (s + 1) * out_bytes / 2e12
        rounds = -(-wgs * s // 256)
        return rounds * ((C // s // 4) * 2.4e-6 + 5e-6) + (s > 1) * (s + 1) * out_bytes / 5e12

    nsplit = 1
    if WINO_SPLIT:
        cands = [s for s in range(1, 33) if C % (4 * s) == 0 and (s == 1 or C // s >= 32)]
        nsplit = min(cands, key=cost)
        if force and C % (4 * force) == 0:
            nsplit = force
    return v2, nsplit, wgs * nsplit


_WINO_PLANS = {}


def _wino_plan(B, C, K, H, W):
    force = int(WINO_NSPLIT_FORCE)
    key = (B, C, K, H, W, force, WINO_KERNEL, WINO_SPLIT)
    plan = _WINO_PLANS.get(key)
    if plan is None:
        plan = _WINO_PLANS[key] = _wino_plan_uncached(B, C, K, H, W, force)
    return plan


def wino_eligible(B, C, K, H, W, min_workgroups=None):
    if C % 4 or K % 32 or H % 4 or W % 4:
        return False
    wgs = _wino_plan(B, C, K, H, W)[2]
    return wgs >= (WINO_MIN_WORKGROUPS if min_workgroups is None else min_workgroups)


WINO_GEMM_MAX_HW = 1024
WINO_GEMM_MIN_CH = 256
_WINO_G = ((1.0, 0.0, 0.0), (1 / 3, 1 / 3, 1 / 3), (-1 / 3, 1 / 3, -1 / 3), (-16 / 15, -8 / 15, -4 / 15),
           (1 / 15, -2 / 15, 4 / 15), (0.0, 0.0, 1.0))


def _wino_gemm_ok(B, C, K, H, W):
    return (0 < H * W <= WINO_GEMM_MAX_HW and C >= WINO_GEMM_MIN_CH and K >= WINO_GEMM_MIN_CH
            and H % 4 == 0 and W % 4 == 0 and B * (H // 4) * (W // 4) <= 65535)


def _wino_u_gemm(weight, flip):
    def build():
        w = weight.detach().double()
        g = w.flip(2, 3).transpose(0, 1) if flip else w
        G = torch.tensor(_WINO_G, dtype=torch.float64, device=w.device)
        return torch.einsum("iu,kcuv,jv->ijck", G, g, G).reshape(36, g.shape[1], g.shape[0]).float().contiguous()
    return _wino_u_cached(weight, flip, "gemm", build)


def _wino_gemm_conv(x, weight, flip, bias, residual, K, gn=False):
    B, C, H, W = x.shape
    T = B * (H // 4) * (W // 4)
    U = _wino_u_gemm(weight, flip)
    V = torch.empty(36, C, T, device=x.device, dtype=F32)
    call("skp_wino_in_transform", ptr(x), B, C, H, W, ptr(V), stream(x.device))
    y = torch.empty(B, K, H, W, device=x.device, dtype=F32)
    bp, rp = ptr(bias) if bias is not None else None, ptr(residual) if residual is not None else None
    M = torch.bmm(U.transpose(1, 2), V)
    P = (H // 4) * (W // 4)
    gnp = None
    if gn and GN_EPI and (P in (16, 32) or P % 64 == 0):
        nseg = P // min(P, 64)
        gnp = torch.empty(B, K, nseg, 2, device=x.device, dtype=F32)
    call("skp_wino_out_transform_kt", ptr(M), B, K, H, W, bp, rp, ptr(y), ptr(gnp), stream(x.device))
    if gnp is not None:
        y._skp_gn = (y._version, gnp, gnp.shape[2])
    return y


def _wino_conv(x, weight, flip, bias, residual, K, gn=False):
    B, C, H, W = x.shape
    if _wino_gemm_ok(B, C, K, H, W):
        return _wino_gemm_conv(x, weight, flip, bias, residual, K, gn)
    y = torch.empty(B, K, H, W, device=x.device, dtype=F32)
    chunks = list(_batch_chunks(B, C * H * W * 4))
    gnp = None
    if gn and GN_EPI and H % 32 == 0 and W % 32 == 0 and all(
            _wino_plan(b1 - b0, C, K, H, W)[:2] == (True, 1) for b0, b1 in chunks):
        nseg = (H // 16) * (W // 32)
        gnp = torch.empty(B, K, nseg, 2, device=x.device, dtype=F32)
    for b0, b1 in chunks:
        _wino_launch(x[b0:b1], weight, flip, bias, None if residual is None else residual[b0:b1], y[b0:b1], K,
                     None if gnp is None else gnp[b0:b1])
    if gnp is not None:
        y._skp_gn = (y._version, gnp, gnp.shape[2])
    return y


def _wino_launch(x, weight, flip, bias, residual, y, K, gnp=None):
    B, C, H, W = x.shape
    v2, nsplit, _ = _wino_plan(B, C, K, H, W)
    U = _wino_u(weight, flip, v2)
    ws = torch.empty(nsplit, B, K, H, W, device=x.device, dtype=F32) if nsplit > 1 else None
    name = "skp_conv3x3_wino2" if v2 else "skp_conv3x3_wino"
    args = (ptr(x), ptr(U), ptr(bias) if bias is not None else None,
            ptr(residual) if residual is not None else None, ptr(y), B, C, K, H, W, nsplit,
            ptr(ws) if ws is not None else None)
    with _timed(name, 0):
        if gnp is not None:
            call("skp_conv3x3_wino2_gn", *args, ptr(gnp), stream(x.device))
        else:
            call(name, *args, stream(x.device))


class Conv3x3(torch.autograd.Function):

    @staticmethod
    def forward(ctx, x, weight, bias, residual):
        x = _c(x)
        K = weight.shape[0]
        y = _wino_conv(x, weight, False, None if bias is None else _c(bias.detach()),
                       None if residual is None else _c(residual), K, gn=True)
        ctx.weight = weight
        ctx.xshape = x.shape
        ctx.has_res = residual is not None
        return y

    @staticmethod
    def backward(ctx, dy):
        w = ctx.weight
        B, C, H, W = ctx.xshape
        K = w.shape[0]
        dx = None
        if ctx.needs_input_grad[0]:
            dy = _c(dy)
            if wino_eligible(B, K, C, H, W):
                dx = _wino_conv(dy, w, True, None, None, C)
            else:
                dx = torch.nn.grad.conv2d_input(ctx.xshape, w.detach(), dy, padding=1)
        return dx, None, None, (dy if ctx.has_res else None)


class Conv1x1(torch.autograd.Function):

    @staticmethod
    def forward(ctx, x, w):
        B, C, H, W = x.shape
        K = w.shape[0]
        y = torch.bmm(w.expand(B, K, C), x.reshape(B, C, H * W))
        ctx.save_for_backward(w)
        ctx.shape = (B, C, H, W)
        return y.view(B, K, H, W)

    @staticmethod
    def backward(ctx, dy):
        (w,) = ctx.saved_tensors
        B, C, H, W = ctx.shape
        K = w.shape[0]
        dx = torch.bmm(w.t().expand(B, C, K), dy.reshape(B, K, H * W)) if ctx.needs_input_grad[0] else None
        return (None if dx is None else dx.view(B, C, H, W)), None


CONV1X1_GEMM = False


def conv1x1(x, weight):
    _lib.require_device(x)
    if weight.requires_grad:
        raise ValueError("conv1x1: the weight must be frozen (requires_grad=False)")
    if not CONV1X1_GEMM or x.dtype != F32:
        return torch.nn.functional.conv2d(x, weight)
    return Conv1x1.apply(_c(x), weight.detach().reshape(weight.shape[0], weight.shape[1]))


WINO_S2 = True
WINO_S2_MIN_PIXELS = 128 * 128


def conv3x3_s2_eligible(x, weight):
    B, C, H, W = x.shape
    K = weight.shape[0]
    return (WINO_S2 and x.is_cuda and x.dtype == F32 and tuple(weight.shape[1:]) == (C, 3, 3) and C % 4 == 0
            and K % 32 == 0 and H % 32 == 0 and W % 32 == 0 and H * W >= WINO_S2_MIN_PIXELS
            and not weight.requires_grad and not (torch.is_grad_enabled() and x.requires_grad))


def conv3x3_s2(x, weight, bias=None):
    _lib.require_device(x)
    if not conv3x3_s2_eligible(x, weight):
        raise ValueError(f"conv3x3_s2: unsupported x {tuple(x.shape)} / weight {tuple(weight.shape)}")
    x = _c16(x)
    B, C, H, W = x.shape
    K = weight.shape[0]
    y = torch.empty(B, K, H // 2, W // 2, device=x.device, dtype=F32)
    U = _wino_u(weight, False, "s2")
    b = None if bias is None else _c(bias.detach())
    for b0, b1 in _batch_chunks(B, C * H * W * 4):
        _, nsplit, _ = _wino_plan(b1 - b0, C, K, H, W)
        ws = torch.empty(nsplit, b1 - b0, K, H // 2, W // 2, device=x.device, dtype=F32) if nsplit > 1 else None
        with _timed("skp_conv3x3s2_f2", 0):
            call("skp_conv3x3s2_f2", ptr(x[b0:b1]), ptr(U), ptr(b), ptr(y[b0:b1]), b1 - b0, C, K, H, W, nsplit,
                 ptr(ws), stream(x.device))
    return y


def conv3x3(x, weight, bias=None, residual=None):
    _lib.require_device(x)
    if weight.requires_grad:
        raise ValueError("conv3x3: the weight must be frozen (requires_grad=False)")
    B, C, H, W = x.shape
    K = weight.shape[0]
    if tuple(weight.shape[1:]) != (C, 3, 3):
        raise ValueError(f"conv3x3: weight {tuple(weight.shape)} does not fit input {tuple(x.shape)}")
    if residual is not None and tuple(residual.shape) != (B, K, H, W):
        raise ValueError(f"conv3x3: residual {tuple(residual.shape)} is not ({B}, {K}, {H}, {W})")
    if C % 4 and C < 16 and x.dtype == F32 and wino_eligible(B, C + 4 - C % 4, K, H, W):
        pad = 4 - C % 4
        xp = torch.nn.functional.pad(x, (0, 0, 0, 0, 0, pad))
        wp = torch.nn.functional.pad(weight.detach(), (0, 0, 0, 0, 0, pad))
        return Conv3x3.apply(xp, wp, bias, residual)
    if x.dtype != F32 or not wino_eligible(B, C, K, H, W):
        y = torch.nn.functional.conv2d(x, weight, bias, 1, 1)
        return y if residual is None else residual + y
    return Conv3x3.apply(x, weight, bias, residual)


WINO_V_SHAPES = {(512, 512, 64, 64), (256, 512, 128, 128), (512, 512, 128, 128), (128, 256, 256, 256),
                 (256, 256, 256, 256)}
WINO_V_MIN_BATCH = 4


def gn_conv3x3_wins(B, C, K, H, W):
    return ((C, K, H, W) in WINO_V_SHAPES and B >= WINO_V_MIN_BATCH and C % 4 == 0 and K % 32 == 0
            and H % 32 == 0 and W % 32 == 0 and WINO_KERNEL == "auto" and not _wino_gemm_ok(B, C, K, H, W))


def gn_conv3x3(x, gamma, beta, groups, eps, act, shift, weight, bias=None, residual=None):
    _lib.require_device(x)
    if torch.is_grad_enabled() and (x.requires_grad or (residual is not None and residual.requires_grad)):
        raise ValueError("gn_conv3x3: forward only (no gradient reaches the normalised activation)")
    if weight.requires_grad or gamma.requires_grad or beta.requires_grad:
        raise ValueError("gn_conv3x3: the parameters must be frozen")
    pre = _gn_parts_of(x) if GN_EPI else None
    x = _c16(x.detach())
    B, C, H, W = x.shape
    K = weight.shape[0]
    if tuple(weight.shape[1:]) != (C, 3, 3):
        raise ValueError(f"gn_conv3x3: weight {tuple(weight.shape)} does not fit input {tuple(x.shape)}")
    if residual is not None:
        if tuple(residual.shape) != (B, K, H, W):
            raise ValueError(f"gn_conv3x3: residual {tuple(residual.shape)} is not ({B}, {K}, {H}, {W})")
        residual = _c16(residual.detach())
    if shift is not None:
        shift = _c(shift.detach().reshape(-1, C).to(x.device, F32).expand(B, C))
    dev = x.device
    nws = _lib.lib().skp_groupnorm_workspace(B, C, H * W, int(groups))
    if nws < 0:
        raise ValueError(f"gn_conv3x3: bad shape {tuple(x.shape)} groups={groups}")
    part = torch.empty(nws, device=dev, dtype=torch.float64)
    stats = torch.empty(B * groups * 2, device=dev, dtype=F32)
    g, b = _c(gamma.detach()), _c(beta.detach())
    if pre is not None:
        call("skp_groupnorm_stats_part", ptr(pre[0]), pre[1], ptr(shift), B, C, H * W, int(groups), float(eps),
             ptr(stats), ptr(part), stream(dev))
    else:
        call("skp_groupnorm_stats", ptr(x), ptr(shift), B, C, H * W, int(groups), float(eps), ptr(stats), ptr(part),
             stream(dev))
    V = torch.empty(B * C * (H // 4) * (W // 4) * 36, device=dev, dtype=F32)
    with _timed("skp_wino2_vtransform_gn", 0):
        call("skp_wino2_vtransform_gn", ptr(x), ptr(stats), ptr(g), ptr(b), ptr(shift), int(groups), int(bool(act)),
             ptr(V), B, C, H, W, stream(dev))
    _, nsplit, _ = _wino_plan(B, C, K, H, W)
    U = _wino_u(weight, False, True)
    y = torch.empty(B, K, H, W, device=dev, dtype=F32)
    ws = torch.empty(nsplit, B, K, H, W, device=dev, dtype=F32) if nsplit > 1 else None
    gnp = torch.empty(B, K, (H // 16) * (W // 32), 2, device=dev, dtype=F32) if GN_EPI and nsplit == 1 else None
    bias = None if bias is None else _c(bias.detach())
    with _timed("skp_conv3x3_wino2_v", 0):
        call("skp_conv3x3_wino2_v_gn", ptr(V), ptr(U), ptr(bias), ptr(residual), ptr(y), B, C, K, H, W, nsplit,
             ptr(ws), ptr(gnp), stream(dev))
    if gnp is not None:
        y._skp_gn = (y._version, gnp, gnp.shape[2])
    return y


TAB10 = ((31, 119, 180), (255, 127, 14), (44, 160, 44), (214, 39, 40), (148, 103, 189), (140, 86, 75),
         (227, 119, 194), (127, 127, 127), (188, 189, 34), (23, 190, 207))
_VIRIDIS_ANCHORS = ((0, (0.267004, 0.004874, 0.329415)), (32, (0.278826, 0.175490, 0.483397)),
                    (64, (0.229739, 0.322361, 0.545706)), (96, (0.172719, 0.448791, 0.557885)),
                    (128, (0.127568, 0.566949, 0.550556)), (160, (0.157851, 0.683765, 0.501686)),
                    (192, (0.369214, 0.788888, 0.382914)), (224, (0.678489, 0.863742, 0.189503)),
                    (255, (0.993248, 0.906157, 0.143936)))
_LUT_CACHE = {}


def default_colors(K):
    if K <= 10:
        rows = TAB10[:K]
    else:
        import colorsys
        rows = [tuple(int(round(255 * c)) for c in colorsys.hsv_to_rgb(j / K, 0.9, 1.0)) for j in range(K)]
    return torch.tensor(rows, dtype=torch.uint8).reshape(K, 3)


def fallback_lut():
    lut = torch.empty(256, 3, dtype=F32)
    for (i0, c0), (i1, c1) in zip(_VIRIDIS_ANCHORS[:-1], _VIRIDIS_ANCHORS[1:]):
        t = torch.arange(i0, i1 + 1, dtype=torch.float64).sub(i0).div(i1 - i0)[:, None]
        lut[i0:i1 + 1] = (torch.tensor(c0, dtype=torch.float64) * (1 - t) + torch.tensor(c1, dtype=torch.float64) * t).float()
    return lut.clamp_(0.0, 1.0)


def default_lut():
    try:
        import matplotlib
        import numpy as np
        cm = matplotlib.colormaps["viridis"]
        return torch.tensor(np.asarray(cm(np.linspace(0.0, 1.0, 256)))[:, :3], dtype=F32).contiguous()
    except ImportError:
        return fallback_lut()


def map_range(maps):
    _lib.require_device(maps)
    maps = _c(maps)
    n, h, w = maps.shape
    out = torch.empty(n, 2, device=maps.device, dtype=F32)
    call("skp_map_range", ptr(maps), n, h, w, ptr(out), stream(maps.device))
    return out


def sheet_shape(H, W, rows, cols, downscale=1, pad=2):
    return rows * (H // downscale + pad) + pad, cols * (W // downscale + pad) + pad


def render_sheet(images, maps=None, points=None, *, rows, cols, downscale=1, pad=2, alpha=0.7, radius=None,
                 colors=None, lut=None, overlay=None):
    _lib.require_device(images, maps, points)
    images = _c(images)
    n, C, H, W = images.shape
    if C != 3:
        raise ValueError(f"render_sheet: images must be (n, 3, H, W), got {tuple(images.shape)}")
    dev = images.device
    f = int(downscale)
    h = w = 0
    rng = None
    if maps is not None:
        maps = _c(maps)
        if maps.dim() != 3 or maps.shape[0] != n:
            raise ValueError(f"render_sheet: maps must be ({n}, h, w), got {tuple(maps.shape)}")
        h, w = maps.shape[1:]
        rng = map_range(maps)
        if overlay is not None:
            keep = torch.as_tensor(overlay, dtype=torch.bool).to(dev)
            if keep.shape != (n,):
                raise ValueError(f"render_sheet: overlay must be ({n},), got {tuple(keep.shape)}")
            rng[~keep] = float("nan")
        if lut is None:
            if dev not in _LUT_CACHE:
                _LUT_CACHE[dev] = default_lut().to(dev)
            lut = _LUT_CACHE[dev]
        lut = _c(lut.to(dev))
        if tuple(lut.shape) != (256, 3):
            raise ValueError(f"render_sheet: lut must be (256, 3), got {tuple(lut.shape)}")
    K = 0
    if points is not None:
        points = _c(points)
        if points.dim() != 3 or points.shape[0] != n or points.shape[2] != 2:
            raise ValueError(f"render_sheet: points must be ({n}, K, 2), got {tuple(points.shape)}")
        K = points.shape[1]
    if K:
        colors = default_colors(K) if colors is None else torch.as_tensor(colors)
        if colors.dtype != torch.uint8 or tuple(colors.shape) != (K, 3):
            raise ValueError(f"render_sheet: colors must be ({K}, 3) uint8")
        colors = colors.to(dev).contiguous()
        if radius is None:
            radius = max(2.0, (H // max(f, 1)) / 32.0)
    else:
        points = colors = None
    Hs, Ws = sheet_shape(H, W, rows, cols, max(f, 1), pad)
    out = torch.empty(Hs, Ws, 3, device=dev, dtype=torch.uint8)
    call("skp_render_sheet", ptr(images), n, H, W, ptr(maps), h, w, ptr(rng), ptr(lut) if maps is not None else None,
         float(alpha), ptr(points), K, float(radius or 0.0), ptr(colors), int(rows), int(cols), f, int(pad), ptr(out),
         stream(dev))
    return out


_TTA_WS = {}


def tta_reduce_bytes(B, C, n, S, avg=False):
    return 4 * B * C * n * S * S + (4 * B * n * S * S if avg else 0)


def tta_reduce(maps, theta_inv, return_avg=False):
    _lib.require_device(maps, theta_inv)
    if maps.dim() != 5 or maps.shape[-1] != maps.shape[-2]:
        raise ValueError(f"tta_reduce: maps must be (B, C, n, S, S), got {tuple(maps.shape)}")
    maps = _c(maps)
    B, C, n, S, _ = maps.shape
    if tuple(theta_inv.shape) != (B, C, 2, 3):
        raise ValueError(f"tta_reduce: theta_inv must be ({B}, {C}, 2, 3), got {tuple(theta_inv.shape)}")
    dev = maps.device
    th = _c(theta_inv.to(dev))
    key = (dev, B, n, S)
    ws = _TTA_WS.get(key)
    if ws is None:
        nbytes = _lib.lib().skp_tta_reduce_workspace(B, n, S)
        if nbytes <= 0:
            raise ValueError(f"tta_reduce: bad shape B={B}, n={n}, S={S}")
        ws = _TTA_WS[key] = torch.empty((nbytes + 7) // 8, device=dev, dtype=torch.int64)
    pos = torch.empty(B, n, 2, device=dev, dtype=F32)
    avg = torch.empty(B, n, S, S, device=dev, dtype=F32) if return_avg else None
    with _timed("skp_tta_reduce", tta_reduce_bytes(B, C, n, S, return_avg)):
        call("skp_tta_reduce", ptr(maps), B, C, n, S, ptr(th), ptr(pos), ptr(avg), ptr(ws), stream(dev))
    return pos, avg


_TTA_SCORED_WS = {}


def tta_reduce_scored_bytes(B, C, n, S, distance=5, avg=False):
    side = 2 * int(distance) + 1
    return tta_reduce_bytes(B, C, n, S, avg) + 16 * B * n * C * side * side


def tta_reduce_scored(maps, theta_inv, distance=5, return_avg=False):
    _lib.require_device(maps, theta_inv)
    if maps.dim() != 5 or maps.shape[-1] != maps.shape[-2]:
        raise ValueError(f"tta_reduce_scored: maps must be (B, C, n, S, S), got {tuple(maps.shape)}")
    maps = _c(maps)
    B, C, n, S, _ = maps.shape
    if tuple(theta_inv.shape) != (B, C, 2, 3):
        raise ValueError(f"tta_reduce_scored: theta_inv must be ({B}, {C}, 2, 3), got {tuple(theta_inv.shape)}")
    distance = float(distance)
    if not 0.0 < distance <= 16.0:
        raise ValueError(f"tta_reduce_scored: distance must be in (0, 16], got {distance}")
    dev = maps.device
    th = _c(theta_inv.to(dev))
    key = (dev, B, n, S)
    ws = _TTA_SCORED_WS.get(key)
    if ws is None:
        nbytes = _lib.lib().skp_tta_reduce_scored_workspace(B, n, S)
        if nbytes <= 0:
            raise ValueError(f"tta_reduce_scored: bad shape B={B}, n={n}, S={S}")
        ws = _TTA_SCORED_WS[key] = torch.empty((nbytes + 7) // 8, device=dev, dtype=torch.int64)
    pos = torch.empty(B, n, 2, device=dev, dtype=F32)
    refined = torch.empty(B, n, 2, device=dev, dtype=F32)
    scores = torch.empty(B, n, 3, device=dev, dtype=F32)
    avg = torch.empty(B, n, S, S, device=dev, dtype=F32) if return_avg else None
    with _timed("skp_tta_reduce_scored", tta_reduce_scored_bytes(B, C, n, S, distance, return_avg)):
        call("skp_tta_reduce_scored", ptr(maps), B, C, n, S, ptr(th), distance, ptr(pos), ptr(refined), ptr(scores),
             ptr(avg), ptr(ws), stream(dev))
    return pos, refined, scores, avg
```

stablekeypoints_amd/sd/unet.py:

```python
import math

import os

import torch
import torch.nn as nn
import torch.nn.functional as F


class CaptureComplete(Exception):
    """Raised by a patched attention when its controller has every map it needs.

    The reference discards the UNet output of a capture pass
    (``ptp_utils.py:246-252``), and nothing after the 4th captured layer feeds the
    loss, so the forward may stop there (SURVEY.md §7 "UNet early exit").
    """


USE_FUSED_GROUPNORM = True
USE_SKP_LAYERNORM = True


def _fused(x, *modules):
    return USE_FUSED_GROUPNORM and x.is_cuda and not any(p.requires_grad for m in modules for p in m.parameters())


def _conv_in(conv, x):
    if _fused(x, conv):
        from .. import ops
        return ops.conv3x3(x, conv.weight, conv.bias)
    return conv(x)


def _ln(norm, x):
    if USE_SKP_LAYERNORM and _fused(x, norm):
        from .. import ops
        return ops.layer_norm(x, norm.weight, norm.bias, norm.eps)
    return norm(x)


NORM_RES = True


def _ln_res(norm, x):
    if NORM_RES and USE_SKP_LAYERNORM and _fused(x, norm) and torch.is_grad_enabled() and x.requires_grad:
        from .. import ops
        return ops.layer_norm_res(x, norm.weight, norm.bias, norm.eps)
    return _ln(norm, x), x


def gn_act_res(norm, x, act):
    if NORM_RES and _fused(x, norm) and torch.is_grad_enabled() and x.requires_grad:
        from .. import ops
        return ops.group_norm_act_res(x, norm.weight, norm.bias, norm.num_groups, norm.eps, act)
    return gn_act(norm, x, act), x


def gn_act(norm, x, act, shift=None):
    if _fused(x, norm):
        from .. import ops
        return ops.group_norm_act(x, norm.weight, norm.bias, norm.num_groups, norm.eps, act, shift)
    if shift is not None:
        x = x + shift.reshape(-1, x.shape[1], 1, 1)
    y = norm(x)
    return F.silu(y) if act else y


class CrossAttention(nn.Module):

    backend = "math"

    def __init__(self, query_dim, cross_attention_dim=None, heads=8, dim_head=64, dropout=0.0, bias=False):
        super().__init__()
        inner_dim = dim_head * heads
        cross_attention_dim = cross_attention_dim if cross_attention_dim is not None else query_dim
        self.scale = dim_head ** -0.5
        self.heads = heads
        self.to_q = nn.Linear(query_dim, inner_dim, bias=bias)
        self.to_k = nn.Linear(cross_attention_dim, inner_dim, bias=bias)
        self.to_v = nn.Linear(cross_attention_dim, inner_dim, bias=bias)
        self.to_out = nn.ModuleList([nn.Linear(inner_dim, query_dim), nn.Dropout(dropout)])

    def reshape_heads_to_batch_dim(self, tensor):
        b, s, dim = tensor.shape
        h = self.heads
        return tensor.reshape(b, s, h, dim // h).permute(0, 2, 1, 3).reshape(b * h, s, dim // h)

    def reshape_batch_dim_to_heads(self, tensor):
        bh, s, d = tensor.shape
        h = self.heads
        return tensor.reshape(bh // h, h, s, d).permute(0, 2, 1, 3).reshape(bh // h, s, d * h)

    def forward(self, x, context=None, mask=None):
        context = x if context is None else context
        if mask is None and USE_FUSED_GROUPNORM and x.is_cuda and CrossAttention.backend == "math":
            from .. import ops
            one = None
            if context is x and ops.QKV_FUSED and _fused(x, self.to_q, self.to_k, self.to_v) and \
                    self.to_q.bias is None and self.to_k.bias is None and self.to_v.bias is None:
                qf, kf, vf = ops.qkv_projection(x, self.to_q.weight, self.to_k.weight, self.to_v.weight)
            else:
                qf = self.to_q(x)
                one = _shared_context(context)
                if one is not None:
                    k1, v1 = shared_kv(self, one)
                    kf, vf = k1.expand(x.shape[0], -1, -1), v1.expand(x.shape[0], -1, -1)
                else:
                    kf, vf = kv_projection(self, context)
            out = ops.attention_heads(qf, kf, vf, self.heads, self.scale)
            if out is None and one is not None and SHARED_HEAD_MAJOR and torch.is_grad_enabled():
                out = shared_context_attention(qf, k1, v1, self.heads, self.scale)
            if out is not None:
                return self.to_out[1](self.to_out[0](out))
            q = self.reshape_heads_to_batch_dim(qf)
            k, v = kf, vf
        else:
            q = self.reshape_heads_to_batch_dim(self.to_q(x))
            k, v = kv_projection(self, context)
        k = self.reshape_heads_to_batch_dim(k)
        v = self.reshape_heads_to_batch_dim(v)
        out = attention_core(q, k, v, self.scale, mask, self.heads)
        out = self.reshape_batch_dim_to_heads(out)
        return self.to_out[1](self.to_out[0](out))


SHARED_KV = True
SHARED_HEAD_MAJOR = True


def _shared_context(context):
    if SHARED_KV and context.dim() == 3 and context.shape[0] > 1 and context.stride(0) == 0:
        base = context._base
        if (base is not None and base.dim() == 3 and base.shape[0] == 1 and base.shape[1:] == context.shape[1:]
                and base.stride()[1:] == context.stride()[1:] and base.data_ptr() == context.data_ptr()):
            return base
        return context[:1]
    return None


def shared_kv(attn, one):
    from .. import ops
    if ops.QKV_FUSED and _fused(one, attn.to_k, attn.to_v) and attn.to_k.bias is None and attn.to_v.bias is None:
        return ops.qkv_projection(one, attn.to_k.weight, attn.to_v.weight)
    return attn.to_k(one), attn.to_v(one)


def shared_context_attention(qf, k1, v1, H, scale):
    B, S, C = qf.shape
    L, d = k1.shape[1], C // H
    q = qf.reshape(B, S, H, d).permute(2, 0, 1, 3).reshape(H, B * S, d)
    k = k1.reshape(L, H, d).transpose(0, 1).contiguous()
    v = v1.reshape(L, H, d).transpose(0, 1).contiguous()
    o = attention_core(q, k, v, scale)
    return o.reshape(H, B, S, d).permute(1, 2, 0, 3).reshape(B, S, C)


def kv_projection(attn, context):
    one = _shared_context(context)
    if one is not None:
        B = context.shape[0]
        k1, v1 = shared_kv(attn, one)
        return k1.expand(B, -1, -1), v1.expand(B, -1, -1)
    return attn.to_k(context), attn.to_v(context)


def attention_core(q, k, v, scale, mask=None, heads=1):
    if mask is None and CrossAttention.backend == "sdpa":
        return F.scaled_dot_product_attention(q.unsqueeze(0), k.unsqueeze(0), v.unsqueeze(0), scale=scale)[0]
    if mask is None and USE_FUSED_GROUPNORM and q.is_cuda and torch.is_grad_enabled() and \
            (q.requires_grad or k.requires_grad or v.requires_grad):
        from .. import ops
        return ops.math_attention(q, k, v, scale)
    if mask is None and USE_FUSED_GROUPNORM and q.is_cuda:
        from .. import ops
        return ops.attention_nograd(q, k, v, scale)
    sim = torch.baddbmm(torch.empty(q.shape[0], q.shape[1], k.shape[1], dtype=q.dtype, device=q.device),
                        q, k.transpose(1, 2), beta=0, alpha=scale)
    if mask is not None:
        b = mask.shape[0]
        m = mask.reshape(b, -1)[:, None, :].repeat(heads, 1, 1)
        sim = sim.masked_fill(~m, -torch.finfo(sim.dtype).max)
    return torch.bmm(sim.softmax(dim=-1), v)


class GEGLU(nn.Module):
    def __init__(self, dim_in, dim_out):
        super().__init__()
        self.proj = nn.Linear(dim_in, dim_out * 2)

    def forward(self, x):
        h = self.proj(x)
        if USE_FUSED_GROUPNORM and h.is_cuda:
            from .. import ops
            return ops.geglu(h)
        x, gate = h.chunk(2, dim=-1)
        return x * F.gelu(gate)


class FeedForward(nn.Module):
    def __init__(self, dim, mult=4, dropout=0.0):
        super().__init__()
        inner = dim * mult
        self.net = nn.ModuleList([GEGLU(dim, inner), nn.Dropout(dropout), nn.Linear(inner, dim)])

    def forward(self, x):
        for m in self.net:
            x = m(x)
        return x


class BasicTransformerBlock(nn.Module):
    def __init__(self, dim, n_heads, d_head, cross_attention_dim):
        super().__init__()
        self.attn1 = CrossAttention(dim, heads=n_heads, dim_head=d_head)
        self.ff = FeedForward(dim)
        self.attn2 = CrossAttention(dim, cross_attention_dim=cross_attention_dim, heads=n_heads, dim_head=d_head)
        self.norm1 = nn.LayerNorm(dim)
        self.norm2 = nn.LayerNorm(dim)
        self.norm3 = nn.LayerNorm(dim)

    def forward(self, h, context=None):
        y, h = _ln_res(self.norm1, h)
        h = self.attn1(y) + h
        y, h = _ln_res(self.norm2, h)
        h = self.attn2(y, context=context) + h
        y, h = _ln_res(self.norm3, h)
        return self.ff(y) + h


class Transformer2DModel(nn.Module):

    def __init__(self, num_attention_heads, attention_head_dim, in_channels, cross_attention_dim, norm_num_groups=32,
                 depth=1, linear_proj=False):
        super().__init__()
        inner = num_attention_heads * attention_head_dim
        self.linear_proj = linear_proj
        self.norm = nn.GroupNorm(norm_num_groups, in_channels, eps=1e-6, affine=True)
        self.proj_in = nn.Linear(in_channels, inner) if linear_proj else nn.Conv2d(in_channels, inner, 1)
        self.transformer_blocks = nn.ModuleList(
            [BasicTransformerBlock(inner, num_attention_heads, attention_head_dim, cross_attention_dim)
             for _ in range(depth)])
        self.proj_out = nn.Linear(inner, in_channels) if linear_proj else nn.Conv2d(inner, in_channels, 1)

    def forward(self, x, encoder_hidden_states=None):
        b, c, hh, ww = x.shape
        x, res = gn_act_res(self.norm, x, False)
        if not self.linear_proj and _fused(x, self.proj_in, self.proj_out):
            from .. import ops
            x = ops.tokens_proj_in(x, self.proj_in.weight, self.proj_in.bias)
            for blk in self.transformer_blocks:
                x = blk(x, context=encoder_hidden_states)
            return ops.tokens_proj_out(x, self.proj_out.weight, self.proj_out.bias, res)
        if self.linear_proj:
            x = self.proj_in(x.permute(0, 2, 3, 1).reshape(b, hh * ww, c))
        else:
            x = self.proj_in(x)
            x = x.permute(0, 2, 3, 1).reshape(b, hh * ww, x.shape[1])
        inner = x.shape[-1]
        for blk in self.transformer_blocks:
            x = blk(x, context=encoder_hidden_states)
        if self.linear_proj:
            return self.proj_out(x).reshape(b, hh, ww, c).permute(0, 3, 1, 2) + res
        x = x.reshape(b, hh, ww, inner).permute(0, 3, 1, 2)
        return self.proj_out(x) + res


class ResnetBlock2D(nn.Module):
    def __init__(self, in_channels, out_channels=None, temb_channels=1280, groups=32, eps=1e-5):
        super().__init__()
        out_channels = in_channels if out_channels is None else out_channels
        self.norm1 = nn.GroupNorm(groups, in_channels, eps=eps, affine=True)
        self.conv1 = nn.Conv2d(in_channels, out_channels, 3, 1, 1)
        self.time_emb_proj = nn.Linear(temb_channels, out_channels) if temb_channels is not None else None
        self.norm2 = nn.GroupNorm(groups, out_channels, eps=eps, affine=True)
        self.dropout = nn.Dropout(0.0)
        self.conv2 = nn.Conv2d(out_channels, out_channels, 3, 1, 1)
        self.conv_shortcut = nn.Conv2d(in_channels, out_channels, 1) if in_channels != out_channels else None

    def forward(self, x, temb=None):
        if _fused(x, self.conv1, self.conv2, self.norm2):
            from .. import ops
            vst = (not torch.is_grad_enabled() and x.dtype == torch.float32 and _fused(x, self.norm1)
                   and (self.dropout.p == 0 or not self.training))
            K = self.conv1.out_channels
            if vst and ops.gn_conv3x3_wins(x.shape[0], x.shape[1], K, x.shape[2], x.shape[3]):
                n1 = self.norm1
                h = ops.gn_conv3x3(x, n1.weight, n1.bias, n1.num_groups, n1.eps, True, None, self.conv1.weight)
            else:
                y, x = gn_act_res(self.norm1, x, True)
                h = ops.conv3x3(y, self.conv1.weight)
            shift = self.conv1.bias[None]
            if temb is not None and self.time_emb_proj is not None:
                shift = shift + self.time_emb_proj(F.silu(temb))
            bias = self.conv2.bias
            if self.conv_shortcut is not None:
                if _fused(x, self.conv_shortcut):
                    x = ops.conv1x1(x, self.conv_shortcut.weight)
                    bias = bias + self.conv_shortcut.bias
                else:
                    x = self.conv_shortcut(x)
            if vst and ops.gn_conv3x3_wins(h.shape[0], K, K, h.shape[2], h.shape[3]):
                n2 = self.norm2
                return ops.gn_conv3x3(h, n2.weight, n2.bias, n2.num_groups, n2.eps, True, shift, self.conv2.weight,
                                      bias, x)
            return ops.conv3x3(self.dropout(gn_act(self.norm2, h, True, shift)), self.conv2.weight, bias, x)
        h = self.conv1(gn_act(self.norm1, x, True))
        if temb is not None and self.time_emb_proj is not None:
            h = h + self.time_emb_proj(F.silu(temb))[:, :, None, None]
        h = self.conv2(self.dropout(gn_act(self.norm2, h, True)))
        if self.conv_shortcut is not None:
            x = self.conv_shortcut(x)
        return x + h


class Downsample2D(nn.Module):
    def __init__(self, channels, padding=1):
        super().__init__()
        self.padding = padding
        self.conv = nn.Conv2d(channels, channels, 3, stride=2, padding=padding)

    def forward(self, x):
        if self.padding == 0 and _fused(x, self.conv):
            from .. import ops
            if ops.conv3x3_s2_eligible(x, self.conv.weight):
                return ops.conv3x3_s2(x, self.conv.weight, self.conv.bias)
        if self.padding == 0:
            B, C, H, W = x.shape
            xp = x.new_empty(B, C, H + 1, W + 1)
            xp[:, :, :H, :W] = x
            xp[:, :, H, :].zero_()
            xp[:, :, :H, W].zero_()
            x = xp
        return self.conv(x)


class Upsample2D(nn.Module):
    def __init__(self, channels):
        super().__init__()
        self.conv = nn.Conv2d(channels, channels, 3, padding=1)

    def forward(self, x, output_size=None):
        if output_size is None:
            x = F.interpolate(x, scale_factor=2.0, mode="nearest")
        else:
            x = F.interpolate(x, size=output_size, mode="nearest")
        if _fused(x, self.conv):
            from .. import ops
            return ops.conv3x3(x, self.conv.weight, self.conv.bias)
        return self.conv(x)


class CrossAttnDownBlock2D(nn.Module):
    def __init__(self, in_ch, out_ch, temb, heads, ctx_dim, add_downsample, groups=32, depth=1, linear_proj=False):
        super().__init__()
        self.resnets = nn.ModuleList([ResnetBlock2D(in_ch if i == 0 else out_ch, out_ch, temb, groups) for i in range(2)])
        self.attentions = nn.ModuleList([Transformer2DModel(heads, out_ch // heads, out_ch, ctx_dim, groups, depth,
                                                            linear_proj) for _ in range(2)])
        self.downsamplers = nn.ModuleList([Downsample2D(out_ch)]) if add_downsample else None

    def forward(self, h, temb, context):
        outs = ()
        for resnet, attn in zip(self.resnets, self.attentions):
            h = attn(resnet(h, temb), encoder_hidden_states=context)
            outs += (h,)
        if self.downsamplers is not None:
            h = self.downsamplers[0](h)
            outs += (h,)
        return h, outs


class DownBlock2D(nn.Module):
    def __init__(self, in_ch, out_ch, temb, add_downsample, groups=32):
        super().__init__()
        self.resnets = nn.ModuleList([ResnetBlock2D(in_ch if i == 0 else out_ch, out_ch, temb, groups) for i in range(2)])
        self.downsamplers = nn.ModuleList([Downsample2D(out_ch)]) if add_downsample else None

    def forward(self, h, temb, context=None):
        outs = ()
        for resnet in self.resnets:
            h = resnet(h, temb)
            outs += (h,)
        if self.downsamplers is not None:
            h = self.downsamplers[0](h)
            outs += (h,)
        return h, outs


class _UpBase(nn.Module):
    def _make_resnets(self, in_ch, out_ch, prev_ch, temb, groups=32):
        res = []
        for i in range(3):
            skip = in_ch if i == 2 else out_ch
            rin = prev_ch if i == 0 else out_ch
            res.append(ResnetBlock2D(rin + skip, out_ch, temb, groups))
        return nn.ModuleList(res)


class CrossAttnUpBlock2D(_UpBase):
    def __init__(self, in_ch, out_ch, prev_ch, temb, heads, ctx_dim, add_upsample, groups=32, depth=1,
                 linear_proj=False):
        super().__init__()
        self.resnets = self._make_resnets(in_ch, out_ch, prev_ch, temb, groups)
        self.attentions = nn.ModuleList([Transformer2DModel(heads, out_ch // heads, out_ch, ctx_dim, groups, depth,
                                                            linear_proj) for _ in range(3)])
        self.upsamplers = nn.ModuleList([Upsample2D(out_ch)]) if add_upsample else None

    def forward(self, h, res_tuple, temb, context, upsample_size=None):
        for resnet, attn in zip(self.resnets, self.attentions):
            skip = res_tuple[-1]
            res_tuple = res_tuple[:-1]
            h = torch.cat([h, skip], dim=1)
            h = attn(resnet(h, temb), encoder_hidden_states=context)
        if self.upsamplers is not None:
            h = self.upsamplers[0](h, upsample_size)
        return h


class UpBlock2D(_UpBase):
    def __init__(self, in_ch, out_ch, prev_ch, temb, add_upsample, groups=32):
        super().__init__()
        self.resnets = self._make_resnets(in_ch, out_ch, prev_ch, temb, groups)
        self.upsamplers = nn.ModuleList([Upsample2D(out_ch)]) if add_upsample else None

    def forward(self, h, res_tuple, temb, context=None, upsample_size=None):
        for resnet in self.resnets:
            skip = res_tuple[-1]
            res_tuple = res_tuple[:-1]
            h = resnet(torch.cat([h, skip], dim=1), temb)
        if self.upsamplers is not None:
            h = self.upsamplers[0](h, upsample_size)
        return h


class UNetMidBlock2DCrossAttn(nn.Module):
    def __init__(self, ch, temb, heads, ctx_dim, groups=32, depth=1, linear_proj=False):
        super().__init__()
        self.resnets = nn.ModuleList([ResnetBlock2D(ch, ch, temb, groups) for _ in range(2)])
        self.attentions = nn.ModuleList([Transformer2DModel(heads, ch // heads, ch, ctx_dim, groups, depth,
                                                            linear_proj)])

    def forward(self, h, temb, context):
        h = self.resnets[0](h, temb)
        h = self.attentions[0](h, encoder_hidden_states=context)
        return self.resnets[1](h, temb)


class TimestepEmbedding(nn.Module):
    def __init__(self, ch, dim):
        super().__init__()
        self.linear_1 = nn.Linear(ch, dim)
        self.linear_2 = nn.Linear(dim, dim)

    def forward(self, x):
        return self.linear_2(F.silu(self.linear_1(x)))


def timestep_embedding(timesteps, dim, flip_sin_to_cos=True, downscale_freq_shift=0.0, max_period=10000):
    half = dim // 2
    exponent = -math.log(max_period) * torch.arange(half, dtype=torch.float32, device=timesteps.device)
    exponent = exponent / (half - downscale_freq_shift)
    emb = timesteps[:, None].float() * torch.exp(exponent)[None, :]
    emb = torch.cat([torch.sin(emb), torch.cos(emb)], dim=-1)
    if flip_sin_to_cos:
        emb = torch.cat([emb[:, half:], emb[:, :half]], dim=-1)
    return emb


class UNet2DConditionModel(nn.Module):

    def __init__(self, in_channels=4, out_channels=4, block_out_channels=(320, 640, 1280, 1280),
                 cross_attention_dim=768, attention_head_dim=8, norm_num_groups=32):
        super().__init__()
        self.cross_attention_dim = cross_attention_dim
        ch0 = block_out_channels[0]
        temb = ch0 * 4
        heads = attention_head_dim
        self.conv_in = nn.Conv2d(in_channels, ch0, 3, padding=1)
        self.time_embedding = TimestepEmbedding(ch0, temb)
        self.down_blocks = nn.ModuleList()
        out_ch = ch0
        for i in range(4):
            in_ch, out_ch = out_ch, block_out_channels[i]
            last = i == 3
            if i < 3:
                self.down_blocks.append(CrossAttnDownBlock2D(in_ch, out_ch, temb, heads, cross_attention_dim, not last,
                                                             norm_num_groups))
            else:
                self.down_blocks.append(DownBlock2D(in_ch, out_ch, temb, not last, norm_num_groups))
        self.mid_block = UNetMidBlock2DCrossAttn(block_out_channels[-1], temb, heads, cross_attention_dim,
                                                 norm_num_groups)
        self.up_blocks = nn.ModuleList()
        rev = list(reversed(block_out_channels))
        out_ch = rev[0]
        for i in range(4):
            prev_ch, out_ch = out_ch, rev[i]
            in_ch = rev[min(i + 1, 3)]
            last = i == 3
            if i == 0:
                self.up_blocks.append(UpBlock2D(in_ch, out_ch, prev_ch, temb, not last, norm_num_groups))
            else:
                self.up_blocks.append(CrossAttnUpBlock2D(in_ch, out_ch, prev_ch, temb, heads, cross_attention_dim,
                                                         not last, norm_num_groups))
        self.conv_norm_out = nn.GroupNorm(norm_num_groups, ch0, eps=1e-5)
        self.conv_act = nn.SiLU()
        self.conv_out = nn.Conv2d(ch0, out_channels, 3, padding=1)
        self.time_proj_dim = ch0

    def forward(self, sample, timestep, encoder_hidden_states, return_dict=True):
        if not torch.is_tensor(timestep):
            timestep = torch.tensor([timestep], dtype=torch.long, device=sample.device)
        timesteps = timestep.reshape(-1).to(sample.device).expand(sample.shape[0])
        emb = self.time_embedding(timestep_embedding(timesteps, self.time_proj_dim).to(sample.dtype))
        h = _conv_in(self.conv_in, sample)
        res = (h,)
        for blk in self.down_blocks:
            h, r = blk(h, emb, encoder_hidden_states)
            res += r
        h = self.mid_block(h, emb, encoder_hidden_states)
        for i, blk in enumerate(self.up_blocks):
            n = len(blk.resnets)
            r, res = res[-n:], res[:-n]
            size = res[-1].shape[2:] if (i < 3) else None
            h = blk(h, r, emb, encoder_hidden_states, upsample_size=size)
        h = self.conv_out(gn_act(self.conv_norm_out, h, True))
        return {"sample": h} if return_dict else (h,)
```

Baseline: 45.25.

## Fuse GroupNorm into Winograd GEMM input transform and trim GN launches

Adds a GroupNorm+SiLU-aware Winograd input transform so ResnetBlock convolutions on the GEMM Winograd path normalize on the fly instead of materializing a normalized tensor. This now also covers the grad-enabled token-optimization step, with a custom autograd backward. GroupNorm stats kernels now write mean/rstd directly when possible, and the part-combine is folded into the apply kernel, removing extra launches. Attention backward skips allocating and writing dS when the query gradient is not needed. The cost is a more complex backward path, and the fused transform recomputes the normalization for each element read.

```diff
diff --git a/include/skp.h b/include/skp.h
--- a/include/skp.h
+++ b/include/skp.h
@@ -94,6 +94,8 @@
                         const float* gout, float* dA, float* dAt, void* stream);
 
 int skp_wino_in_transform(const float* x, int B, int C, int H, int W, float* V, void* stream);
+int skp_wino_in_transform_gn(const float* x, const float* stats, const float* gamma, const float* beta,
+                             const float* shift, int G, int act, float* V, int B, int C, int H, int W, void* stream);
 int skp_wino_out_transform(const float* M, int B, int K, int H, int W, const float* bias, const float* residual,
                            float* y, void* stream);
 int skp_wino_out_transform_kt(const float* M, int B, int K, int H, int W, const float* bias, const float* residual,
@@ -124,6 +126,9 @@
 int skp_groupnorm_bwd_add(const float* x, const float* dy, const float* gamma, const float* beta, const float* shift,
                           const float* stats, int B, int C, long long HW, int G, int act, const float* dres, float* dx,
                           double* partial, void* stream);
+int skp_groupnorm_apply(const float* x, const float* gamma, const float* beta, const float* shift, int B, int C,
+                        long long HW, int G, float eps, int act, const double* partial, float* y, float* stats,
+                        void* stream);
 int skp_softmax_bwd(const float* P, float* dP, long long rows, int cols, float alpha, void* stream);
 int skp_softmax_fwd(float* S, long long rows, int cols, void* stream);
 int skp_attn_dscore(const float* P, const float* dO, const float* V, const float* D, float* out, int BH, int S, int L,
diff --git a/stablekeypoints_amd/_lib.py b/stablekeypoints_amd/_lib.py
--- a/stablekeypoints_amd/_lib.py
+++ b/stablekeypoints_amd/_lib.py
@@ -84,6 +84,8 @@
                                _p],
     "skp_groupnorm_stats": [_p, _p, _c_int, _c_int, _c_ll, _c_int, _c_float, _p, _p, _p],
     "skp_groupnorm_stats_part": [_p, _c_int, _p, _c_int, _c_int, _c_ll, _c_int, _c_float, _p, _p, _p],
+    "skp_groupnorm_apply": [_p, _p, _p, _p, _c_int, _c_int, _c_ll, _c_int, _c_float, _c_int, _p, _p, _p, _p],
+    "skp_wino_in_transform_gn": [_p, _p, _p, _p, _p, _c_int, _c_int, _p, _c_int, _c_int, _c_int, _c_int, _p],
     "skp_wino2_vtransform": [_p, _p, _c_int, _c_int, _c_int, _c_int, _p],
     "skp_wino2_vtransform_gn": [_p, _p, _p, _p, _p, _c_int, _c_int, _p, _c_int, _c_int, _c_int, _c_int, _p],
     "skp_conv3x3_wino2_v": [_p, _p, _p, _p, _p, _c_int, _c_int, _c_int, _c_int, _c_int, _c_int, _p, _p],
diff --git a/stablekeypoints_amd/csrc/skp_groupnorm.hip b/stablekeypoints_amd/csrc/skp_groupnorm.hip
--- a/stablekeypoints_amd/csrc/skp_groupnorm.hip
+++ b/stablekeypoints_amd/csrc/skp_groupnorm.hip
@@ -77,10 +77,21 @@
   b = sd[1];
 }
 
+__device__ __forceinline__ void moments_of(double s1, double s2, const GNShape& sh, float eps, float& mean,
+                                           float& rstd) {
+  const double n = (double)sh.len;
+  const double m = s1 / n;
+  double var = s2 / n - m * m;
+  var = var < 0.0 ? 0.0 : var;
+  mean = (float)m;
+  rstd = (float)(1.0 / sqrt(var + (double)eps));
+}
+
 template <bool VEC>
 __global__ __launch_bounds__(kThreads) void gn_stats_kernel(const float* __restrict__ x,
                                                             const float* __restrict__ shift, GNShape sh,
-                                                            double* __restrict__ partial) {
+                                                            double* __restrict__ partial, float eps,
+                                                            float* __restrict__ stats) {
   __shared__ double sd[2 * kThreads / 64];
   const int grp = blockIdx.x / sh.nsplit, sp = blockIdx.x % sh.nsplit;
   const int g = grp % sh.G;
@@ -106,18 +117,22 @@
   if (threadIdx.x == 0) {
     partial[2 * blockIdx.x] = s1;
     partial[2 * blockIdx.x + 1] = s2;
-  }
-}
-
-__global__ __launch_bounds__(kThreads) void gn_part_combine_kernel(const float2* __restrict__ part, int nseg,
-                                                                   const float* __restrict__ shift, GNShape sh,
-                                                                   double* __restrict__ partial) {
-  __shared__ double sd[2 * kThreads / 64];
-  const int grp = blockIdx.x;
+    if (stats) {
+      float mean, rstd;
+      moments_of(0.0 + s1, 0.0 + s2, sh, eps, mean, rstd);
+      stats[2 * grp] = mean;
+      stats[2 * grp + 1] = rstd;
+    }
+  }
+}
+
+__device__ __forceinline__ void part_sums(const float2* __restrict__ part, int nseg, const float* __restrict__ shift,
+                                          const GNShape& sh, int grp, double& s1, double& s2) {
   const int b = grp / sh.G, g = grp - b * sh.G;
   const float2* pg = part + ((size_t)b * sh.C + (size_t)g * sh.cpg) * nseg;
   const double n = (double)(sh.HW / nseg);
-  double s1 = 0.0, s2 = 0.0;
+  s1 = 0.0;
+  s2 = 0.0;
   for (int e = threadIdx.x; e < sh.cpg * nseg; e += kThreads) {
     const float2 v = pg[e];
     const double t = shift ? (double)shift[(size_t)b * sh.C + g * sh.cpg + e / nseg] : 0.0;
@@ -125,7 +140,23 @@
     s1 += n * mt;
     s2 += (double)v.y + n * mt * mt;
   }
+}
+
+__global__ __launch_bounds__(kThreads) void gn_part_combine_kernel(const float2* __restrict__ part, int nseg,
+                                                                   const float* __restrict__ shift, GNShape sh,
+                                                                   double* __restrict__ partial, float eps,
+                                                                   float* __restrict__ stats) {
+  __shared__ double sd[2 * kThreads / 64];
+  const int grp = blockIdx.x;
+  double s1, s2;
+  part_sums(part, nseg, shift, sh, grp, s1, s2);
   block_sum2(s1, s2, sd);
+  if (threadIdx.x == 0) {
+    float mean, rstd;
+    moments_of(0.0 + s1, 0.0 + s2, sh, eps, mean, rstd);
+    stats[2 * grp] = mean;
+    stats[2 * grp + 1] = rstd;
+  }
   if (threadIdx.x < sh.nsplit) {
     partial[2 * ((size_t)grp * sh.nsplit + threadIdx.x)] = threadIdx.x == 0 ? s1 : 0.0;
     partial[2 * ((size_t)grp * sh.nsplit + threadIdx.x) + 1] = threadIdx.x == 0 ? s2 : 0.0;
@@ -143,23 +174,31 @@
     s1 += partial[2 * (grp * sh.nsplit + k)];
     s2 += partial[2 * (grp * sh.nsplit + k) + 1];
   }
-  const double n = (double)sh.len;
-  const double m = s1 / n;
-  double var = s2 / n - m * m;
-  var = var < 0.0 ? 0.0 : var;
-  mean = (float)m;
-  rstd = (float)(1.0 / sqrt(var + (double)eps));
+  moments_of(s1, s2, sh, eps, mean, rstd);
 }
 
 template <bool VEC, bool ACT>
 __global__ __launch_bounds__(kThreads) void gn_apply_kernel(const float* __restrict__ x, const float* __restrict__ gamma,
                                                             const float* __restrict__ beta,
                                                             const float* __restrict__ shift, GNShape sh, float eps,
-                                                            const double* __restrict__ partial, float* __restrict__ y,
-                                                            float* __restrict__ stats) {
+                                                            const double* __restrict__ partial,
+                                                            const float2* __restrict__ part, int nseg,
+                                                            float* __restrict__ y, float* __restrict__ stats) {
   __shared__ float sm[2];
+  __shared__ double sd[2 * kThreads / 64];
   const int grp = blockIdx.x / sh.nsplit, sp = blockIdx.x % sh.nsplit;
-  if (threadIdx.x == 0) {
+  if (part) {
+    double s1, s2;
+    part_sums(part, nseg, shift, sh, grp, s1, s2);
+    block_sum2(s1, s2, sd);
+    if (threadIdx.x == 0) {
+      float mean, rstd;
+      moments_of(0.0 + s1, 0.0 + s2, sh, eps, mean, rstd);
+      sm[0] = mean;
+      sm[1] = rstd;
+      if (sp == 0 && stats) { stats[2 * grp] = mean; stats[2 * grp + 1] = rstd; }
+    }
+  } else if (threadIdx.x == 0) {
     float mean, rstd;
     group_moments(partial, grp, sh, eps, mean, rstd);
     sm[0] = mean;
@@ -341,6 +380,22 @@
   return B * G * sh.nsplit * 2;
 }
 
+namespace {
+void launch_apply(const float* x, const float* gamma, const float* beta, const float* shift, const GNShape& sh,
+                  float eps, int act, const double* partial, const float2* part, int nseg, float* y, float* stats,
+                  hipStream_t st) {
+  const bool vec = (sh.HW % 4 == 0) && ((reinterpret_cast<uintptr_t>(x) & 15) == 0) &&
+                   ((reinterpret_cast<uintptr_t>(y) & 15) == 0);
+  const dim3 grid(sh.B * sh.G * sh.nsplit);
+#define SKP_GN_APPLY(V, A) \
+  hipLaunchKernelGGL((gn_apply_kernel<V, A>), grid, dim3(kThreads), 0, st, x, gamma, beta, shift, sh, eps, partial, \
+                     part, nseg, y, stats)
+  if (vec) { if (act) SKP_GN_APPLY(true, true); else SKP_GN_APPLY(true, false); }
+  else { if (act) SKP_GN_APPLY(false, true); else SKP_GN_APPLY(false, false); }
+#undef SKP_GN_APPLY
+}
+}
+
 extern "C" int skp_groupnorm_fwd(const float* x, const float* gamma, const float* beta, const float* shift, int B,
                                  int C, long long HW, int G, float eps, int act, float* y, float* stats,
                                  double* partial, void* stream) {
@@ -351,15 +406,10 @@
                    ((reinterpret_cast<uintptr_t>(y) & 15) == 0);
   hipStream_t st = as_stream(stream);
   const dim3 grid(B * G * sh.nsplit);
-  if (vec) hipLaunchKernelGGL(gn_stats_kernel<true>, grid, dim3(kThreads), 0, st, x, shift, sh, partial);
-  else hipLaunchKernelGGL(gn_stats_kernel<false>, grid, dim3(kThreads), 0, st, x, shift, sh, partial);
-  SKP_LAUNCH_CHECK();
-#define SKP_GN_APPLY(V, A) \
-  hipLaunchKernelGGL((gn_apply_kernel<V, A>), grid, dim3(kThreads), 0, st, x, gamma, beta, shift, sh, eps, partial, y, \
-                     stats)
-  if (vec) { if (act) SKP_GN_APPLY(true, true); else SKP_GN_APPLY(true, false); }
-  else { if (act) SKP_GN_APPLY(false, true); else SKP_GN_APPLY(false, false); }
-#undef SKP_GN_APPLY
+  if (vec) hipLaunchKernelGGL(gn_stats_kernel<true>, grid, dim3(kThreads), 0, st, x, shift, sh, partial, eps, nullptr);
+  else hipLaunchKernelGGL(gn_stats_kernel<false>, grid, dim3(kThreads), 0, st, x, shift, sh, partial, eps, nullptr);
+  SKP_LAUNCH_CHECK();
+  launch_apply(x, gamma, beta, shift, sh, eps, act, partial, nullptr, 0, y, stats, st);
   SKP_LAUNCH_CHECK();
   return SKP_OK;
 }
@@ -372,19 +422,19 @@
   GNShape sh;
   SKP_CHECK_ARG(make_shape(B, C, HW, G, sh), "bad shape (C must be divisible by G)");
   SKP_CHECK_ARG((reinterpret_cast<uintptr_t>(part) & 7) == 0, "part must be 8-byte aligned");
-  const bool vec = (HW % 4 == 0) && ((reinterpret_cast<uintptr_t>(x) & 15) == 0) &&
-                   ((reinterpret_cast<uintptr_t>(y) & 15) == 0);
-  hipStream_t st = as_stream(stream);
-  hipLaunchKernelGGL(gn_part_combine_kernel, dim3(B * G), dim3(kThreads), 0, st, reinterpret_cast<const float2*>(part),
-                     nseg, shift, sh, partial);
-  SKP_LAUNCH_CHECK();
-  const dim3 grid(B * G * sh.nsplit);
-#define SKP_GN_APPLY(V, A) \
-  hipLaunchKernelGGL((gn_apply_kernel<V, A>), grid, dim3(kThreads), 0, st, x, gamma, beta, shift, sh, eps, partial, y, \
-                     stats)
-  if (vec) { if (act) SKP_GN_APPLY(true, true); else SKP_GN_APPLY(true, false); }
-  else { if (act) SKP_GN_APPLY(false, true); else SKP_GN_APPLY(false, false); }
-#undef SKP_GN_APPLY
+  launch_apply(x, gamma, beta, shift, sh, eps, act, partial, reinterpret_cast<const float2*>(part), nseg, y, stats,
+               as_stream(stream));
+  SKP_LAUNCH_CHECK();
+  return SKP_OK;
+}
+
+extern "C" int skp_groupnorm_apply(const float* x, const float* gamma, const float* beta, const float* shift, int B,
+                                   int C, long long HW, int G, float eps, int act, const double* partial, float* y,
+                                   float* stats, void* stream) {
+  SKP_CHECK_ARG(x && gamma && beta && y && partial, "null pointer");
+  GNShape sh;
+  SKP_CHECK_ARG(make_shape(B, C, HW, G, sh), "bad shape (C must be divisible by G)");
+  launch_apply(x, gamma, beta, shift, sh, eps, act, partial, nullptr, 0, y, stats, as_stream(stream));
   SKP_LAUNCH_CHECK();
   return SKP_OK;
 }
@@ -409,11 +459,13 @@
   const bool vec = (HW % 4 == 0) && ((reinterpret_cast<uintptr_t>(x) & 15) == 0);
   hipStream_t st = as_stream(stream);
   const dim3 grid(B * G * sh.nsplit);
-  if (vec) hipLaunchKernelGGL(gn_stats_kernel<true>, grid, dim3(kThreads), 0, st, x, shift, sh, partial);
-  else hipLaunchKernelGGL(gn_stats_kernel<false>, grid, dim3(kThreads), 0, st, x, shift, sh, partial);
-  SKP_LAUNCH_CHECK();
-  hipLaunchKernelGGL(gn_moments_kernel, dim3((B * G + kThreads - 1) / kThreads), dim3(kThreads), 0, st, partial, sh, eps,
-                     stats);
+  float* direct = sh.nsplit == 1 ? stats : nullptr;
+  if (vec) hipLaunchKernelGGL(gn_stats_kernel<true>, grid, dim3(kThreads), 0, st, x, shift, sh, partial, eps, direct);
+  else hipLaunchKernelGGL(gn_stats_kernel<false>, grid, dim3(kThreads), 0, st, x, shift, sh, partial, eps, direct);
+  SKP_LAUNCH_CHECK();
+  if (!direct)
+    hipLaunchKernelGGL(gn_moments_kernel, dim3((B * G + kThreads - 1) / kThreads), dim3(kThreads), 0, st, partial, sh,
+                       eps, stats);
   SKP_LAUNCH_CHECK();
   return SKP_OK;
 }
@@ -427,10 +479,7 @@
   SKP_CHECK_ARG((reinterpret_cast<uintptr_t>(part) & 7) == 0, "part must be 8-byte aligned");
   hipStream_t st = as_stream(stream);
   hipLaunchKernelGGL(gn_part_combine_kernel, dim3(B * G), dim3(kThreads), 0, st, reinterpret_cast<const float2*>(part),
-                     nseg, shift, sh, partial);
-  SKP_LAUNCH_CHECK();
-  hipLaunchKernelGGL(gn_moments_kernel, dim3((B * G + kThreads - 1) / kThreads), dim3(kThreads), 0, st, partial, sh, eps,
-                     stats);
+                     nseg, shift, sh, partial, eps, stats);
   SKP_LAUNCH_CHECK();
   return SKP_OK;
 }
diff --git a/stablekeypoints_amd/csrc/skp_softmax.hip b/stablekeypoints_amd/csrc/skp_softmax.hip
--- a/stablekeypoints_amd/csrc/skp_softmax.hip
+++ b/stablekeypoints_amd/csrc/skp_softmax.hip
@@ -559,7 +559,7 @@
 #pragma unroll
       for (int bj = 0; bj < 4; ++bj) {
         const float sv = alpha * (pc[bj][r] * (dp4[bj][r] - Dr));
-        if (!RC || k0 + 16 * bj + (lane & 15) < L) dSr[(size_t)r * L + 16 * bj] = sv;
+        if (dS && (!RC || k0 + 16 * bj + (lane & 15) < L)) dSr[(size_t)r * L + 16 * bj] = sv;
         s4[bj][r] = sv;
       }
     }
@@ -648,7 +648,7 @@
                           const float* dO, AttnLay lo, const float* stats, const float* D, float* dS, float* dV,
                           AttnLay ldv, float* dK, AttnLay ldk, int BH, int H, int S, int L, int d, float scale,
                           void* stream) {
-  SKP_CHECK_ARG(Q && K && V && dO && stats && D && dS && dV && dK, "null pointer");
+  SKP_CHECK_ARG(Q && K && V && dO && stats && D && dV && dK, "null pointer");
   SKP_CHECK_ARG(BH > 0 && H > 0 && BH % H == 0 && S > 0 && L > 0, "non-positive shape");
   SKP_CHECK_ARG(S % 64 == 0, "S must be a multiple of 64");
   SKP_CHECK_ARG(BH <= 65535, "grid too large");
diff --git a/stablekeypoints_amd/csrc/skp_wino_gemm.hip b/stablekeypoints_amd/csrc/skp_wino_gemm.hip
--- a/stablekeypoints_amd/csrc/skp_wino_gemm.hip
+++ b/stablekeypoints_amd/csrc/skp_wino_gemm.hip
@@ -1,4 +1,5 @@
 #include "skp_common.h"
+#include "skp_gn.h"
 
 using namespace skp;
 
@@ -12,7 +13,12 @@
                                         {0.f, 1.f, 1.f, 0.25f, 4.f, 0.f},
                                         {0.f, 1.f, -1.f, 0.125f, -8.f, 1.f}};
 
+template <int GN>
 __global__ __launch_bounds__(256) void wino_in_kernel(const float* __restrict__ x, int B, int C, int H, int W,
+                                                      const float* __restrict__ stats,
+                                                      const float* __restrict__ gamma,
+                                                      const float* __restrict__ beta,
+                                                      const float* __restrict__ shift, int G,
                                                       float* __restrict__ V) {
   const int tw = W >> 2, th = H >> 2, T = B * th * tw;
   const int t = blockIdx.x * blockDim.x + threadIdx.x;
@@ -21,6 +27,13 @@
   const int b = t / (th * tw), r = t - b * th * tw;
   const int ty = r / tw, tx = r - ty * tw;
   const float* xc = x + ((size_t)b * C + c) * H * W;
+  GNCoef k{1.0f, 0.0f};
+  float sft = 0.0f;
+  if (GN) {
+    const int grp = b * G + c / (C / G);
+    k = gn_coef(gamma[c], beta[c], stats[2 * grp], stats[2 * grp + 1]);
+    sft = shift ? shift[(size_t)b * C + c] : 0.0f;
+  }
   float d[6][6];
 #pragma unroll
   for (int a = 0; a < 6; ++a) {
@@ -28,7 +41,9 @@
 #pragma unroll
     for (int e = 0; e < 6; ++e) {
       const int xx = 4 * tx - 1 + e;
-      d[a][e] = (yy >= 0 && yy < H && xx >= 0 && xx < W) ? xc[(size_t)yy * W + xx] : 0.0f;
+      const bool in = yy >= 0 && yy < H && xx >= 0 && xx < W;
+      if (GN) d[a][e] = in ? gn_elem<GN == 2>(xc[(size_t)yy * W + xx], sft, k) : 0.0f;
+      else d[a][e] = in ? xc[(size_t)yy * W + xx] : 0.0f;
     }
   }
   float tmp[6][6];
@@ -189,15 +204,39 @@
 
 }
 
+namespace {
+const char* wino_in_args_error(const float* x, const float* V, int B, int C, int H, int W) {
+  if (!(x && V)) return "null pointer";
+  if (!(B > 0 && C > 0 && H > 0 && W > 0)) return "non-positive shape";
+  if (!(H % 4 == 0 && W % 4 == 0)) return "H and W must be multiples of 4";
+  if (C > 65535) return "C > 65535";
+  if ((long long)B * (H / 4) * (W / 4) * C * 36 >= (1LL << 40)) return "too large";
+  return nullptr;
+}
+}
+
 extern "C" int skp_wino_in_transform(const float* x, int B, int C, int H, int W, float* V, void* stream) {
-  SKP_CHECK_ARG(x && V, "null pointer");
-  SKP_CHECK_ARG(B > 0 && C > 0 && H > 0 && W > 0, "non-positive shape");
-  SKP_CHECK_ARG(H % 4 == 0 && W % 4 == 0, "H and W must be multiples of 4");
-  SKP_CHECK_ARG(C <= 65535, "C > 65535");
+  const char* err = wino_in_args_error(x, V, B, C, H, W);
+  SKP_CHECK_ARG(!err, err);
   const long long T = (long long)B * (H / 4) * (W / 4);
-  SKP_CHECK_ARG(T * C * 36 < (1LL << 40), "too large");
-  hipLaunchKernelGGL(wino_in_kernel, dim3((unsigned)((T + 255) / 256), C), dim3(256), 0, as_stream(stream), x, B, C, H, W,
-                     V);
+  hipLaunchKernelGGL(wino_in_kernel<0>, dim3((unsigned)((T + 255) / 256), C), dim3(256), 0, as_stream(stream), x, B, C,
+                     H, W, nullptr, nullptr, nullptr, nullptr, 1, V);
+  SKP_LAUNCH_CHECK();
+  return SKP_OK;
+}
+
+extern "C" int skp_wino_in_transform_gn(const float* x, const float* stats, const float* gamma, const float* beta,
+                                        const float* shift, int G, int act, float* V, int B, int C, int H, int W,
+                                        void* stream) {
+  const char* err = wino_in_args_error(x, V, B, C, H, W);
+  SKP_CHECK_ARG(!err, err);
+  SKP_CHECK_ARG(stats && gamma && beta, "null pointer (stats, gamma, beta)");
+  SKP_CHECK_ARG(G > 0 && C % G == 0, "C must be divisible by G");
+  const long long T = (long long)B * (H / 4) * (W / 4);
+  const dim3 grid((unsigned)((T + 255) / 256), C);
+  hipStream_t st = as_stream(stream);
+  if (act) hipLaunchKernelGGL(wino_in_kernel<2>, grid, dim3(256), 0, st, x, B, C, H, W, stats, gamma, beta, shift, G, V);
+  else hipLaunchKernelGGL(wino_in_kernel<1>, grid, dim3(256), 0, st, x, B, C, H, W, stats, gamma, beta, shift, G, V);
   SKP_LAUNCH_CHECK();
   return SKP_OK;
 }
diff --git a/stablekeypoints_amd/ops.py b/stablekeypoints_amd/ops.py
--- a/stablekeypoints_amd/ops.py
+++ b/stablekeypoints_amd/ops.py
@@ -867,6 +867,32 @@
     return y, stats, g, b, nws
 
 
+def _gn_stats(x, shift, groups, eps, pre):
+    B, C = x.shape[:2]
+    HW = x[0, 0].numel()
+    nws = _lib.lib().skp_groupnorm_workspace(B, C, HW, int(groups))
+    if nws < 0:
+        raise ValueError(f"groupnorm: bad shape {tuple(x.shape)} groups={groups}")
+    part = torch.empty(nws, device=x.device, dtype=torch.float64)
+    stats = torch.empty(B * groups * 2, device=x.device, dtype=F32)
+    if pre is not None:
+        call("skp_groupnorm_stats_part", ptr(pre[0]), pre[1], ptr(shift), B, C, HW, int(groups), float(eps),
+             ptr(stats), ptr(part), stream(x.device))
+    else:
+        call("skp_groupnorm_stats", ptr(x), ptr(shift), B, C, HW, int(groups), float(eps), ptr(stats), ptr(part),
+             stream(x.device))
+    return stats, nws
+
+
+def _gn_bwd(x, dy, g, b, shift, stats, meta, dres):
+    B, C, HW, G, act, nws = meta
+    dx = torch.empty_like(x)
+    part = torch.empty(nws, device=x.device, dtype=torch.float64)
+    call("skp_groupnorm_bwd_add", ptr(x), ptr(dy), ptr(g), ptr(b), ptr(shift), ptr(stats), B, C, HW, G, act,
+         ptr(dres), ptr(dx), ptr(part), stream(x.device))
+    return dx
+
+
 class GroupNormAct(torch.autograd.Function):
 
     @staticmethod
@@ -884,12 +910,7 @@
     @staticmethod
     def backward(ctx, dy):
         x, g, b, stats, shift = ctx.saved_tensors
-        B, C, HW, G, act, nws = ctx.meta
-        dy = _c(dy)
-        dx = torch.empty_like(x)
-        part = torch.empty(nws, device=x.device, dtype=torch.float64)
-        call("skp_groupnorm_bwd", ptr(x), ptr(dy), ptr(g), ptr(b), ptr(shift), ptr(stats), B, C, HW, G, act, ptr(dx),
-             ptr(part), stream(x.device))
+        dx = _gn_bwd(x, _c(dy), g, b, shift, stats, ctx.meta, None)
         return dx, None, None, None, None, None, None
 
 
@@ -910,13 +931,7 @@
     @staticmethod
     def backward(ctx, dy, dpass):
         x, g, b, stats, shift = ctx.saved_tensors
-        B, C, HW, G, act, nws = ctx.meta
-        dy = _c(dy)
-        dres = None if dpass is None else _c16(dpass)
-        dx = torch.empty_like(x)
-        part = torch.empty(nws, device=x.device, dtype=torch.float64)
-        call("skp_groupnorm_bwd_add", ptr(x), ptr(dy), ptr(g), ptr(b), ptr(shift), ptr(stats), B, C, HW, G, act,
-             ptr(dres), ptr(dx), ptr(part), stream(x.device))
+        dx = _gn_bwd(x, _c(dy), g, b, shift, stats, ctx.meta, None if dpass is None else _c16(dpass))
         return dx, None, None, None, None, None, None
 
 
@@ -1148,7 +1163,7 @@
         BH, S, d = q.shape
         L = k.shape[1]
         D = (dout * out).sum(-1)
-        ds = torch.empty(BH, S, L, device=q.device, dtype=F32)
+        ds = torch.empty(BH, S, L, device=q.device, dtype=F32) if ctx.needs_input_grad[0] else None
         dv, dk = torch.empty_like(v), torch.empty_like(k)
         call("skp_attn_bwd_flash", ptr(q), ptr(k), ptr(v), ptr(dout), ptr(stats), ptr(D), ptr(ds), ptr(dv), ptr(dk),
              BH, S, L, d, float(ctx.scale), stream(q.device))
@@ -1205,7 +1220,7 @@
         L = k.shape[1]
         d = C // H
         D = (dout.view(B, S, H, d) * out.view(B, S, H, d)).sum(-1).transpose(1, 2).contiguous()
-        ds = torch.empty(B * H, S, L, device=q.device, dtype=F32)
+        ds = torch.empty(B * H, S, L, device=q.device, dtype=F32) if ctx.needs_input_grad[0] else None
         dv = torch.empty(B, L, C, device=q.device, dtype=F32)
         dk = torch.empty(B, L, C, device=q.device, dtype=F32)
         call("skp_attn_bwd_flash_bshd", ptr(q), *_lay(q), ptr(k), *_lay(k), ptr(v), *_lay(v), ptr(dout), S * C, C,
@@ -1446,12 +1461,17 @@
     return _wino_u_cached(weight, flip, "gemm", build)
 
 
-def _wino_gemm_conv(x, weight, flip, bias, residual, K, gn=False):
+def _wino_gemm_conv(x, weight, flip, bias, residual, K, gn=False, norm=None):
     B, C, H, W = x.shape
     T = B * (H // 4) * (W // 4)
     U = _wino_u_gemm(weight, flip)
     V = torch.empty(36, C, T, device=x.device, dtype=F32)
-    call("skp_wino_in_transform", ptr(x), B, C, H, W, ptr(V), stream(x.device))
+    if norm is None:
+        call("skp_wino_in_transform", ptr(x), B, C, H, W, ptr(V), stream(x.device))
+    else:
+        stats, g, b, shift, groups, act = norm
+        call("skp_wino_in_transform_gn", ptr(x), ptr(stats), ptr(g), ptr(b), ptr(shift), int(groups), int(bool(act)),
+             ptr(V), B, C, H, W, stream(x.device))
     y = torch.empty(B, K, H, W, device=x.device, dtype=F32)
     bp, rp = ptr(bias) if bias is not None else None, ptr(residual) if residual is not None else None
     M = torch.bmm(U.transpose(1, 2), V)
@@ -1642,18 +1662,8 @@
     if shift is not None:
         shift = _c(shift.detach().reshape(-1, C).to(x.device, F32).expand(B, C))
     dev = x.device
-    nws = _lib.lib().skp_groupnorm_workspace(B, C, H * W, int(groups))
-    if nws < 0:
-        raise ValueError(f"gn_conv3x3: bad shape {tuple(x.shape)} groups={groups}")
-    part = torch.empty(nws, device=dev, dtype=torch.float64)
-    stats = torch.empty(B * groups * 2, device=dev, dtype=F32)
+    stats, _ = _gn_stats(x, shift, groups, eps, pre)
     g, b = _c(gamma.detach()), _c(beta.detach())
-    if pre is not None:
-        call("skp_groupnorm_stats_part", ptr(pre[0]), pre[1], ptr(shift), B, C, H * W, int(groups), float(eps),
-             ptr(stats), ptr(part), stream(dev))
-    else:
-        call("skp_groupnorm_stats", ptr(x), ptr(shift), B, C, H * W, int(groups), float(eps), ptr(stats), ptr(part),
-             stream(dev))
     V = torch.empty(B * C * (H // 4) * (W // 4) * 36, device=dev, dtype=F32)
     with _timed("skp_wino2_vtransform_gn", 0):
         call("skp_wino2_vtransform_gn", ptr(x), ptr(stats), ptr(g), ptr(b), ptr(shift), int(groups), int(bool(act)),
@@ -1670,6 +1680,68 @@
     if gnp is not None:
         y._skp_gn = (y._version, gnp, gnp.shape[2])
     return y
+
+
+GN_CONV_GEMM = True
+
+
+def gn_conv3x3_gemm_ok(B, C, K, H, W):
+    return bool(GN_CONV_GEMM and C % 4 == 0 and K % 32 == 0 and _wino_gemm_ok(B, C, K, H, W)
+                and wino_eligible(B, C, K, H, W))
+
+
+class GroupNormConv3x3(torch.autograd.Function):
+
+    @staticmethod
+    def forward(ctx, x, gamma, beta, groups, eps, act, shift, weight, bias, residual, pass_x):
+        pre = _gn_parts_of(x) if GN_EPI else None
+        xc = _c(x)
+        B, C, H, W = xc.shape
+        K = weight.shape[0]
+        if shift is not None:
+            shift = _c(shift.detach().expand(B, C))
+        stats, nws = _gn_stats(xc, shift, groups, eps, pre)
+        g, b = _c(gamma.detach()), _c(beta.detach())
+        y = _wino_gemm_conv(xc, weight, False, None if bias is None else _c(bias.detach()),
+                            None if residual is None else _c(residual), K, gn=True,
+                            norm=(stats, g, b, shift, groups, act))
+        ctx.save_for_backward(xc, g, b, stats, shift)
+        ctx.weight = weight
+        ctx.meta = (B, C, H * W, int(groups), int(act), nws)
+        ctx.has_res = residual is not None
+        return (y, x.view_as(x)) if pass_x else y
+
+    @staticmethod
+    def backward(ctx, dy, dpass=None):
+        x, g, b, stats, shift = ctx.saved_tensors
+        w = ctx.weight
+        B, C, H, W = x.shape
+        K = w.shape[0]
+        dx = None
+        dy = _c(dy)
+        if ctx.needs_input_grad[0]:
+            if wino_eligible(B, K, C, H, W):
+                dh = _wino_conv(dy, w, True, None, None, C)
+            else:
+                dh = torch.nn.grad.conv2d_input(x.shape, w.detach(), dy, padding=1)
+            dx = _gn_bwd(x, _c(dh), g, b, shift, stats, ctx.meta, None if dpass is None else _c16(dpass))
+        return dx, None, None, None, None, None, None, None, None, (dy if ctx.has_res else None), None
+
+
+def gn_conv3x3_gemm(x, gamma, beta, groups, eps, act, shift, weight, bias=None, residual=None, pass_x=False):
+    _lib.require_device(x)
+    if weight.requires_grad or gamma.requires_grad or beta.requires_grad:
+        raise ValueError("gn_conv3x3_gemm: the parameters must be frozen")
+    B, C, H, W = x.shape
+    K = weight.shape[0]
+    if x.dtype != F32 or tuple(weight.shape[1:]) != (C, 3, 3) or not gn_conv3x3_gemm_ok(B, C, K, H, W):
+        raise ValueError(f"gn_conv3x3_gemm: unsupported x {tuple(x.shape)} / weight {tuple(weight.shape)}")
+    if residual is not None and tuple(residual.shape) != (B, K, H, W):
+        raise ValueError(f"gn_conv3x3_gemm: residual {tuple(residual.shape)} is not ({B}, {K}, {H}, {W})")
+    if shift is not None:
+        shift = shift.reshape(-1, C).to(x.device, F32)
+    return GroupNormConv3x3.apply(x, gamma, beta, int(groups), float(eps), bool(act), shift, weight, bias, residual,
+                                  bool(pass_x))
 
 
 TAB10 = ((31, 119, 180), (255, 127, 14), (44, 160, 44), (214, 39, 40), (148, 103, 189), (140, 86, 75),
diff --git a/stablekeypoints_amd/sd/unet.py b/stablekeypoints_amd/sd/unet.py
--- a/stablekeypoints_amd/sd/unet.py
+++ b/stablekeypoints_amd/sd/unet.py
@@ -282,9 +282,17 @@
             vst = (not torch.is_grad_enabled() and x.dtype == torch.float32 and _fused(x, self.norm1)
                    and (self.dropout.p == 0 or not self.training))
             K = self.conv1.out_channels
+            gemm = (x.dtype == torch.float32 and _fused(x, self.norm1)
+                    and (self.dropout.p == 0 or not self.training))
+            n1, n2 = self.norm1, self.norm2
             if vst and ops.gn_conv3x3_wins(x.shape[0], x.shape[1], K, x.shape[2], x.shape[3]):
-                n1 = self.norm1
                 h = ops.gn_conv3x3(x, n1.weight, n1.bias, n1.num_groups, n1.eps, True, None, self.conv1.weight)
+            elif gemm and ops.gn_conv3x3_gemm_ok(x.shape[0], x.shape[1], K, x.shape[2], x.shape[3]):
+                res = NORM_RES and torch.is_grad_enabled() and x.requires_grad
+                h = ops.gn_conv3x3_gemm(x, n1.weight, n1.bias, n1.num_groups, n1.eps, True, None, self.conv1.weight,
+                                        pass_x=res)
+                if res:
+                    h, x = h
             else:
                 y, x = gn_act_res(self.norm1, x, True)
                 h = ops.conv3x3(y, self.conv1.weight)
@@ -299,9 +307,11 @@
                 else:
                     x = self.conv_shortcut(x)
             if vst and ops.gn_conv3x3_wins(h.shape[0], K, K, h.shape[2], h.shape[3]):
-                n2 = self.norm2
                 return ops.gn_conv3x3(h, n2.weight, n2.bias, n2.num_groups, n2.eps, True, shift, self.conv2.weight,
                                       bias, x)
+            if gemm and ops.gn_conv3x3_gemm_ok(h.shape[0], K, K, h.shape[2], h.shape[3]):
+                return ops.gn_conv3x3_gemm(h, n2.weight, n2.bias, n2.num_groups, n2.eps, True, shift,
+                                           self.conv2.weight, bias, x)
             return ops.conv3x3(self.dropout(gn_act(self.norm2, h, True, shift)), self.conv2.weight, bias, x)
         h = self.conv1(gn_act(self.norm1, x, True))
         if temb is not None and self.time_emb_proj is not None:
```

New measurement: 45.36, median of 6. Within noise of the previous version (+0.2%).
